# Eric-qi/NeuroQuant

Measured on AMD Instinct MI355X. Metric: calibration iters/sec (HNeRV Bunny 1280x640, 21k iters) + final PSNR vs ref, higher is better.
Workload: dtype f32 operands split into bf16 hi+lo, 3 BF16 MFMAs per product, fp32 accumulate (bf16x3); fp32 MFMA on small layers; 1 GPU; HNeRV Bunny_1280x640_3M, channel_wise, bits 6 5 4 5 5 6 6, phase-2 (AdaRound) iteration; per_gpu_batch=2, global_batch=2, frames=132, parallelism=dp1

## Files before the change

include/nq_hip.h:

```cpp
#ifndef NQ_HIP_H
#define NQ_HIP_H

#include <stdint.h>

#ifdef __cplusplus
extern "C" {
#endif

typedef void* nq_stream_t;

#define NQ_API __attribute__((visibility("default")))

#define NQ_OK 0
#define NQ_ERR_INVALID (-1)
#define NQ_ERR_UNSUPPORTED (-2)
#define NQ_ERR_LAUNCH (-3)

NQ_API int nq_abi_version(void);
NQ_API const char* nq_error_string(int code);


NQ_API int nq_scale_init_max(const float* x, int64_t rows, int64_t row_len, int n_levels, float* delta, float* zp,
                      nq_stream_t stream);

NQ_API int nq_uaq_forward(const float* x, const float* delta, const float* zp, float* y, int64_t rows, int64_t row_len,
                   int per_row, int n_levels, nq_stream_t stream);

NQ_API int nq_uaq_backward(const float* x, const float* gy, const float* delta, const float* zp, float* ddelta, float* dx,
                    int64_t rows, int64_t row_len, int per_row, int n_levels, nq_stream_t stream);

NQ_API int nq_adaround_init(const float* x, const float* delta_in, const float* zp_in, float* delta_out, float* zp_out,
                     float* alpha, int64_t rows, int64_t row_len, int per_row, nq_stream_t stream);

NQ_API int nq_adaround_forward(const float* x, const float* alpha, const float* delta, const float* zp, float* y, float* xq,
                        int64_t rows, int64_t row_len, int per_row, int n_levels, int soft, nq_stream_t stream);

NQ_API int nq_adaround_backward(const float* x, const float* gy, const float* alpha, const float* delta, const float* zp,
                         float* dalpha, int64_t rows, int64_t row_len, int per_row, int n_levels, float reg_weight,
                         float reg_b, nq_stream_t stream);

NQ_API int64_t nq_reduce_ws_floats(int64_t n);
NQ_API int nq_round_loss(const float* alpha, int64_t n, float b, float weight, float* ws, float* out, int accumulate,
                  nq_stream_t stream);

NQ_API int nq_round_loss_backward(const float* alpha, int64_t n, float b, float weight, const float* gscale, float* dalpha,
                           int accumulate, nq_stream_t stream);

NQ_API int nq_adam_step(float* p, const float* g, float* m, float* v, int64_t n, float step_size, float beta1, float beta2,
                 float eps, float bc2_sqrt, nq_stream_t stream);

typedef struct nq_ada_seg {
  const float* x;
  const float* gy;
  const float* alpha;
  const float* delta;
  const float* zp;
  float* out;
  int64_t rows, row_len;
  int per_row, n_levels, soft;
  float reg_weight;
} nq_ada_seg;
typedef struct nq_adam_seg {
  float* p;
  const float* g;
  float* m;
  float* v;
  int64_t n;
} nq_adam_seg;
typedef struct nq_ada_adam_seg {
  const float* x;
  const float* gy;
  float* alpha;
  const float* delta;
  const float* zp;
  float* m;
  float* v;
  int64_t rows, row_len;
  int per_row, n_levels;
  float reg_weight;
} nq_ada_adam_seg;
NQ_API int nq_adaround_adam_multi(const nq_ada_adam_seg* segs, int nseg, float reg_b, float step_size, float beta1, float beta2, float eps,
                           float bc2_sqrt, const float* dyn, nq_stream_t stream);
NQ_API int nq_adaround_forward_multi(const nq_ada_seg* segs, int nseg, nq_stream_t stream);
NQ_API int nq_uaq_forward_multi(const nq_ada_seg* segs, int nseg, nq_stream_t stream);
NQ_API int nq_uaq_backward_multi(const nq_ada_seg* segs, int nseg, nq_stream_t stream);
NQ_API int nq_adaround_backward_multi(const nq_ada_seg* segs, int nseg, float reg_b, nq_stream_t stream);
NQ_API int nq_adam_step_multi(const nq_adam_seg* segs, int nseg, float step_size, float beta1, float beta2, float eps,
                       float bc2_sqrt, nq_stream_t stream);

NQ_API int nq_step_prologue(const int64_t* order, const float* scal, int* step, int64_t* cur_idx, float* cur_scal, int B, int nscal,
                     nq_stream_t stream);
NQ_API int nq_step_prologue_gather(const int64_t* order, const float* scal, int* step, int64_t* cur_idx, float* cur_scal, int B, int nscal,
                            const float* table, int64_t table_rows, int64_t row_len, float* out, nq_stream_t stream);
NQ_API int nq_adaround_backward_multi_dyn(const nq_ada_seg* segs, int nseg, const float* dyn, nq_stream_t stream);
NQ_API int nq_adam_step_multi_dyn(const nq_adam_seg* segs, int nseg, const float* dyn, float beta1, float beta2, float eps,
                           nq_stream_t stream);

NQ_API int nq_fwht(const float* x, float* y, int64_t outer, int n, int64_t inner, int n_in, int n_out, nq_stream_t stream);

typedef struct nq_fwht_seg {
  const float* x;
  float* y;
  int64_t outer, inner;
  int n, n_in, n_out;
} nq_fwht_seg;
NQ_API int nq_fwht_multi(const nq_fwht_seg* segs, int nseg, nq_stream_t stream);

typedef struct nq_fq_fwht_seg {
  const float* x;
  float* alpha;
  const float* delta;
  const float* zp;
  float* m;
  float* v;
  const float* gy;
  float* y;
  int64_t outer, inner;
  int n, c_in, per_row, n_levels, soft;
  float reg_weight;
} nq_fq_fwht_seg;
NQ_API int nq_adaround_fwht_multi(const nq_fq_fwht_seg* segs, int nseg, nq_stream_t stream);
NQ_API int nq_fwht_adaround_adam_multi(const nq_fq_fwht_seg* segs, int nseg, float reg_b, float step_size, float beta1, float beta2,
                                float eps, float bc2_sqrt, const float* dyn, nq_stream_t stream);


NQ_API int nq_weight_layouts(const float* w, float* wt_fwd, float* wt_bwd, int Cout, int Cin, int k, int krows_fwd,
                      int ld_fwd, int krows_bwd, int ld_bwd, nq_stream_t stream);

typedef struct nq_wl_seg {
  const float* w;
  float* wt_fwd;
  float* wt_bwd;
  int Cout, Cin, k, krows_fwd, ld_fwd, krows_bwd, ld_bwd;
} nq_wl_seg;
NQ_API int nq_weight_layouts_multi(const nq_wl_seg* segs, int nseg, nq_stream_t stream);

NQ_API int nq_conv_operand_dims(int Cin, int Cout, int k, int* krows, int* ld);

#define NQ_EPI_PLAIN 0
#define NQ_EPI_PS_GELU 1
#define NQ_EPI_TANH 2
#define NQ_EPI_PS 3
#define NQ_EPI_DGRAD_GELU 4
#define NQ_EPI_X_SPLIT 0x100
#define NQ_EPI_Y_SPLIT 0x200
NQ_API int nq_split_words(const float* x, float* y, int64_t n, nq_stream_t stream);
NQ_API int64_t nq_conv_forward_ws_floats(int B, int Cin, int H, int W, int Cout, int k);
NQ_API int nq_conv_split_out(int B, int Cin, int H, int W, int Cout, int k, int r, int epilogue, int in_gelu, int has_bias);
NQ_API int nq_conv_forward(const float* x, const float* wt, const float* bias, float* y, float* z, float* ws, int B, int Cin, int H,
                    int W, int Cout, int k, int krows, int ld, int r, int epilogue, int in_gelu, const float* zprev,
                    nq_stream_t stream);

NQ_API int nq_conv3_supported(int B, int Cin, int H, int W, int Cout, int k);
NQ_API int nq_conv3_split_io(int B, int Cin, int H, int W, int Cout, int k);
NQ_API int64_t nq_conv_forward3_ws_floats(int B, int Cin, int H, int W, int Cout, int k);
NQ_API int64_t nq_conv3_weight_bytes(int Cin, int Cout, int k);
NQ_API int nq_weight_layout3(const float* w, void* wt3, int Cin, int Cout, int k, int transposed, nq_stream_t stream);
typedef struct nq_wl3_seg {
  const float* w;
  void* wt3;
  int Cin, Cout, k, transposed;
} nq_wl3_seg;
NQ_API int nq_weight_layout3_multi(const nq_wl3_seg* segs, int nseg, nq_stream_t stream);
NQ_API int nq_weight_layouts_all(const nq_wl3_seg* segs3, int n3, const nq_wl_seg* segsf, int nf, nq_stream_t stream);
NQ_API int nq_conv_forward3(const float* x, const void* wt3, const float* bias, float* y, float* z, const float* zprev, float* ws, int B,
                     int Cin, int H, int W, int Cout, int k, int r, int epilogue, nq_stream_t stream);

NQ_API int nq_conv_wgrad3_supported(int B, int Cin, int H, int W, int Cout, int k);
NQ_API int64_t nq_conv_wgrad3_ws_floats(int B, int Cin, int H, int W, int Cout, int k);
NQ_API int nq_conv_wgrad3_plan(int B, int Cin, int H, int W, int Cout, int k, int* mi, int* ni, int* nsplit, int* pc);
NQ_API int nq_conv_wgrad3(const float* x, const float* dy, float* dw, float* db, float* ws, int B, int Cin, int H, int W, int Cout,
                   int k, nq_stream_t stream);
NQ_API int nq_conv_wgrad3_split_io(int B, int Cin, int H, int W, int Cout, int k);
NQ_API int nq_conv_wgrad3_fmt(const float* x, const float* dy, float* dw, float* db, float* ws, int B, int Cin, int H, int W, int Cout,
                       int k, int fmt, nq_stream_t stream);
NQ_API int nq_conv_wgrad3_swapped(const float* x, const float* dy, float* dw, float* ws, int B, int Cin, int H, int W, int Cout, int k,
                           nq_stream_t stream);

NQ_API int64_t nq_conv_wgrad_ws_floats(int B, int Cin, int H, int W, int Cout, int k);
NQ_API int nq_conv_wgrad(const float* x, const float* dy, float* dw, float* db, float* ws, int B, int Cin, int H, int W, int Cout,
                  int k, int x_gelu, nq_stream_t stream);

typedef struct nq_wgr_seg {
  const float* slab;
  const float* slab_db;
  float* dw;
  float* db;
  int Cout, N, co_pad, n_pad, nsplit;
  int swap_kk;
  int sg;
} nq_wgr_seg;
NQ_API int nq_conv_wgrad3_slabs(const float* x, const float* dy, float* dw, float* db, float* ws, int B, int Cin, int H, int W, int Cout,
                         int k, nq_wgr_seg* seg, nq_stream_t stream);
NQ_API int nq_conv_wgrad3_slabs_fmt(const float* x, const float* dy, float* dw, float* db, float* ws, int B, int Cin, int H, int W,
                             int Cout, int k, nq_wgr_seg* seg, int fmt, nq_stream_t stream);
NQ_API int nq_conv_wgrad3_swapped_slabs(const float* x, const float* dy, float* dw, float* ws, int B, int Cin, int H, int W, int Cout,
                                 int k, nq_wgr_seg* seg, nq_stream_t stream);
NQ_API int nq_conv_wgrad_slabs(const float* x, const float* dy, float* dw, float* db, float* ws, int B, int Cin, int H, int W, int Cout,
                        int k, int x_gelu, nq_wgr_seg* seg, nq_stream_t stream);
NQ_API int nq_wgrad_reduce_multi(const nq_wgr_seg* segs, int nseg, nq_stream_t stream);

NQ_API int nq_ps_gelu_backward(const float* da, const float* z, float* dconv, int B, int C, int H, int W, int r,
                        nq_stream_t stream);

NQ_API int nq_tanh_out_backward(const float* dimg, const float* img, float* dconv, int64_t n, nq_stream_t stream);

NQ_API int nq_l2_loss(const float* pred, const float* tgt, float* loss, float* dpred, float* ws, int64_t n, int64_t mean_count,
               float gscale, nq_stream_t stream);

NQ_API int nq_channel_sum(const float* x, float* out, float* ws, int B, int C, int64_t HW, nq_stream_t stream);

NQ_API int nq_l2_loss_tanh_head(const float* pred, const float* tgt, const uint8_t* cache_u8, const int64_t* idx, float* loss,
                         float* dconv, float* db, float* ws, int B, int C, int64_t HW, int64_t mean_count, float gscale,
                         nq_stream_t stream);

NQ_API int64_t nq_head_forward_loss_ws_floats(int B, int H, int W);
NQ_API int nq_head_forward_loss(const float* x, const float* wt, int ld, const float* bias, float* y, const float* tgt,
                         const uint8_t* cache_u8, const int64_t* idx, float* loss, float* dconv, float* db, float* ws, int B,
                         int Cin, int H, int W, int64_t mean_count, float gscale, nq_stream_t stream);

NQ_API int nq_frame_sse(const float* out, const float* gt, float* sse, int64_t frames, int64_t frame_len, nq_stream_t stream);

NQ_API int64_t nq_ms_ssim_ws_floats(int64_t frames, int C, int H, int W);
NQ_API int nq_ms_ssim(const float* out, const float* gt, float* msssim, float* ws, int64_t frames, int C, int H, int W,
               nq_stream_t stream);

NQ_API int nq_gather_frames_u8(const uint8_t* src, const int64_t* idx, float* dst, int64_t n, int64_t frame_len,
                        nq_stream_t stream);

NQ_API int nq_act_dd(const float* x, const float* g, const float* g2, float* y, int64_t n, int mode, nq_stream_t stream);
NQ_API int nq_pixel_shuffle(const float* x, float* y, int B, int C, int H, int W, int r, int inverse, nq_stream_t stream);
NQ_API int nq_bias_add(const float* x, const float* bias, float* y, int B, int C, int64_t HW, nq_stream_t stream);

#ifdef __cplusplus
}
#endif
#endif
```

neuroquant_amd/_lib.py:

```python
import ctypes
import os
from ctypes import c_char_p, c_float, c_int, c_int64, c_void_p, POINTER, Structure

_HERE = os.path.dirname(os.path.abspath(__file__))
LIB_PATH = os.environ.get("NQ_LIB") or os.path.join(_HERE, "libnqhip.so")

NQ_OK = 0
ABI_VERSION = 5
EPI_PLAIN, EPI_PS_GELU, EPI_TANH, EPI_PS, EPI_DGRAD_GELU = 0, 1, 2, 3, 4


class NQLibraryError(RuntimeError):
    pass


class AdaSeg(Structure):
    _fields_ = [("x", c_void_p), ("gy", c_void_p), ("alpha", c_void_p), ("delta", c_void_p), ("zp", c_void_p),
                ("out", c_void_p), ("rows", c_int64), ("row_len", c_int64), ("per_row", c_int), ("n_levels", c_int),
                ("soft", c_int), ("reg_weight", c_float)]


class WL3Seg(Structure):
    _fields_ = [("w", c_void_p), ("wt3", c_void_p), ("Cin", c_int), ("Cout", c_int), ("k", c_int), ("transposed", c_int)]


class WLSeg(Structure):
    _fields_ = [("w", c_void_p), ("wt_fwd", c_void_p), ("wt_bwd", c_void_p), ("Cout", c_int), ("Cin", c_int), ("k", c_int),
                ("krows_fwd", c_int), ("ld_fwd", c_int), ("krows_bwd", c_int), ("ld_bwd", c_int)]


class FwhtSeg(Structure):
    _fields_ = [("x", c_void_p), ("y", c_void_p), ("outer", c_int64), ("inner", c_int64), ("n", c_int), ("n_in", c_int),
                ("n_out", c_int)]


class AdaAdamSeg(Structure):
    _fields_ = [("x", c_void_p), ("gy", c_void_p), ("alpha", c_void_p), ("delta", c_void_p), ("zp", c_void_p), ("m", c_void_p),
                ("v", c_void_p), ("rows", c_int64), ("row_len", c_int64), ("per_row", c_int), ("n_levels", c_int),
                ("reg_weight", c_float)]


class WgrSeg(Structure):
    _fields_ = [("slab", c_void_p), ("slab_db", c_void_p), ("dw", c_void_p), ("db", c_void_p), ("Cout", c_int), ("N", c_int),
                ("co_pad", c_int), ("n_pad", c_int), ("nsplit", c_int), ("swap_kk", c_int), ("sg", c_int)]


class FqFwhtSeg(Structure):
    _fields_ = [("x", c_void_p), ("alpha", c_void_p), ("delta", c_void_p), ("zp", c_void_p), ("m", c_void_p), ("v", c_void_p),
                ("gy", c_void_p), ("y", c_void_p), ("outer", c_int64), ("inner", c_int64), ("n", c_int), ("c_in", c_int),
                ("per_row", c_int), ("n_levels", c_int), ("soft", c_int), ("reg_weight", c_float)]


class AdamSeg(Structure):
    _fields_ = [("p", c_void_p), ("g", c_void_p), ("m", c_void_p), ("v", c_void_p), ("n", c_int64)]


def _load():
    if not os.path.exists(LIB_PATH):
        raise NQLibraryError(
            f"{LIB_PATH} not found: build it with `python -c 'import __graft_entry__ as g; g.build()'` "
            "(or `make -C neuroquant_amd/csrc`).  neuroquant_amd has no CPU/eager fallback.")
    import torch
    lib = ctypes.CDLL(LIB_PATH)
    P, I, L, F = c_void_p, c_int, c_int64, c_float

    def sig(name, res, *args):
        fn = getattr(lib, name)
        fn.restype = res
        fn.argtypes = list(args)

    sig("nq_abi_version", I)
    got = lib.nq_abi_version()
    if got != ABI_VERSION:
        raise NQLibraryError(f"{LIB_PATH} has ABI version {got}, this package binds version {ABI_VERSION}: rebuild it "
                             "(`make -C neuroquant_amd/csrc`)")
    sig("nq_error_string", c_char_p, I)
    sig("nq_scale_init_max", I, P, L, L, I, P, P, P)
    sig("nq_uaq_forward", I, P, P, P, P, L, L, I, I, P)
    sig("nq_uaq_backward", I, P, P, P, P, P, P, L, L, I, I, P)
    sig("nq_adaround_init", I, P, P, P, P, P, P, L, L, I, P)
    sig("nq_adaround_forward", I, P, P, P, P, P, P, L, L, I, I, I, P)
    sig("nq_adaround_backward", I, P, P, P, P, P, P, L, L, I, I, F, F, P)
    sig("nq_adaround_adam_multi", I, POINTER(AdaAdamSeg), I, F, F, F, F, F, F, P, P)
    sig("nq_adaround_forward_multi", I, POINTER(AdaSeg), I, P)
    sig("nq_uaq_forward_multi", I, POINTER(AdaSeg), I, P)
    sig("nq_uaq_backward_multi", I, POINTER(AdaSeg), I, P)
    sig("nq_adaround_backward_multi", I, POINTER(AdaSeg), I, F, P)
    sig("nq_adam_step_multi", I, POINTER(AdamSeg), I, F, F, F, F, F, P)
    sig("nq_step_prologue", I, P, P, P, P, P, I, I, P)
    sig("nq_step_prologue_gather", I, P, P, P, P, P, I, I, P, L, L, P, P)
    sig("nq_adaround_backward_multi_dyn", I, POINTER(AdaSeg), I, P, P)
    sig("nq_adam_step_multi_dyn", I, POINTER(AdamSeg), I, P, F, F, F, P)
    sig("nq_reduce_ws_floats", L, L)
    sig("nq_round_loss", I, P, L, F, F, P, P, I, P)
    sig("nq_round_loss_backward", I, P, L, F, F, P, P, I, P)
    sig("nq_adam_step", I, P, P, P, P, L, F, F, F, F, F, P)
    sig("nq_fwht", I, P, P, L, I, L, I, I, P)
    sig("nq_fwht_multi", I, POINTER(FwhtSeg), I, P)
    sig("nq_weight_layouts", I, P, P, P, I, I, I, I, I, I, I, P)
    sig("nq_conv_operand_dims", I, I, I, I, POINTER(c_int), POINTER(c_int))
    sig("nq_conv_forward_ws_floats", L, I, I, I, I, I, I)
    sig("nq_conv_forward", I, P, P, P, P, P, P, I, I, I, I, I, I, I, I, I, I, I, P, P)
    sig("nq_conv3_supported", I, I, I, I, I, I, I)
    sig("nq_conv3_split_io", I, I, I, I, I, I, I)
    sig("nq_conv_split_out", I, I, I, I, I, I, I, I, I, I, I)
    sig("nq_split_words", I, P, P, L, P)
    sig("nq_conv_wgrad3_split_io", I, I, I, I, I, I, I)
    sig("nq_conv_wgrad3_fmt", I, P, P, P, P, P, I, I, I, I, I, I, I, P)
    sig("nq_conv_wgrad3_slabs_fmt", I, P, P, P, P, P, I, I, I, I, I, I, POINTER(WgrSeg), I, P)
    sig("nq_conv3_weight_bytes", L, I, I, I)
    sig("nq_weight_layout3", I, P, P, I, I, I, I, P)
    sig("nq_weight_layout3_multi", I, POINTER(WL3Seg), I, P)
    sig("nq_weight_layouts_multi", I, POINTER(WLSeg), I, P)
    sig("nq_weight_layouts_all", I, POINTER(WL3Seg), I, POINTER(WLSeg), I, P)
    sig("nq_conv_forward3_ws_floats", L, I, I, I, I, I, I)
    sig("nq_conv_forward3", I, P, P, P, P, P, P, P, I, I, I, I, I, I, I, I, P)
    sig("nq_conv_wgrad3_supported", I, I, I, I, I, I, I)
    sig("nq_conv_wgrad3_ws_floats", L, I, I, I, I, I, I)
    sig("nq_conv_wgrad3_plan", I, I, I, I, I, I, I, POINTER(c_int), POINTER(c_int), POINTER(c_int), POINTER(c_int))
    sig("nq_conv_wgrad3", I, P, P, P, P, P, I, I, I, I, I, I, P)
    sig("nq_conv_wgrad3_swapped", I, P, P, P, P, I, I, I, I, I, I, P)
    sig("nq_conv_wgrad3_slabs", I, P, P, P, P, P, I, I, I, I, I, I, POINTER(WgrSeg), P)
    sig("nq_conv_wgrad3_swapped_slabs", I, P, P, P, P, I, I, I, I, I, I, POINTER(WgrSeg), P)
    sig("nq_conv_wgrad_slabs", I, P, P, P, P, P, I, I, I, I, I, I, I, POINTER(WgrSeg), P)
    sig("nq_wgrad_reduce_multi", I, POINTER(WgrSeg), I, P)
    sig("nq_conv_wgrad_ws_floats", L, I, I, I, I, I, I)
    sig("nq_conv_wgrad", I, P, P, P, P, P, I, I, I, I, I, I, I, P)
    sig("nq_ps_gelu_backward", I, P, P, P, I, I, I, I, I, P)
    sig("nq_tanh_out_backward", I, P, P, P, L, P)
    sig("nq_l2_loss", I, P, P, P, P, P, L, L, F, P)
    sig("nq_channel_sum", I, P, P, P, I, I, L, P)
    sig("nq_l2_loss_tanh_head", I, P, P, P, P, P, P, P, P, I, I, L, L, F, P)
    sig("nq_frame_sse", I, P, P, P, L, L, P)
    sig("nq_ms_ssim_ws_floats", L, L, I, I, I)
    sig("nq_ms_ssim", I, P, P, P, P, L, I, I, I, P)
    sig("nq_gather_frames_u8", I, P, P, P, L, L, P)
    sig("nq_adaround_fwht_multi", I, POINTER(FqFwhtSeg), I, P)
    sig("nq_fwht_adaround_adam_multi", I, POINTER(FqFwhtSeg), I, F, F, F, F, F, F, P, P)
    sig("nq_head_forward_loss_ws_floats", L, I, I, I)
    sig("nq_head_forward_loss", I, P, P, I, P, P, P, P, P, P, P, P, P, I, I, I, I, L, F, P)
    sig("nq_act_dd", I, P, P, P, P, L, I, P)
    sig("nq_pixel_shuffle", I, P, P, I, I, I, I, I, I, P)
    sig("nq_bias_add", I, P, P, P, I, I, L, P)
    return lib


EXPORTS = (
    "nq_abi_version", "nq_error_string", "nq_scale_init_max", "nq_uaq_forward", "nq_uaq_backward",
    "nq_adaround_init", "nq_adaround_forward", "nq_adaround_backward", "nq_reduce_ws_floats", "nq_round_loss", "nq_round_loss_backward",
    "nq_adam_step", "nq_adaround_adam_multi", "nq_adaround_forward_multi", "nq_uaq_forward_multi", "nq_uaq_backward_multi", "nq_adaround_backward_multi", "nq_adam_step_multi", "nq_step_prologue", "nq_step_prologue_gather", "nq_adaround_backward_multi_dyn", "nq_adam_step_multi_dyn", "nq_fwht", "nq_fwht_multi", "nq_weight_layouts", "nq_conv_operand_dims", "nq_conv_forward_ws_floats", "nq_conv_forward",
    "nq_conv3_supported", "nq_conv3_weight_bytes", "nq_weight_layout3", "nq_weight_layout3_multi", "nq_weight_layouts_multi", "nq_conv_forward3_ws_floats", "nq_conv_forward3",
    "nq_conv_wgrad3_supported", "nq_conv_wgrad3_ws_floats", "nq_conv_wgrad3_plan", "nq_conv_wgrad3", "nq_conv_wgrad3_swapped",
    "nq_conv_wgrad3_slabs", "nq_conv_wgrad3_swapped_slabs", "nq_conv_wgrad_slabs", "nq_wgrad_reduce_multi",
    "nq_conv_wgrad_ws_floats", "nq_conv_wgrad", "nq_ps_gelu_backward", "nq_tanh_out_backward", "nq_l2_loss",
    "nq_channel_sum", "nq_l2_loss_tanh_head", "nq_frame_sse", "nq_ms_ssim_ws_floats", "nq_ms_ssim", "nq_gather_frames_u8",
    "nq_act_dd", "nq_pixel_shuffle", "nq_bias_add", "nq_conv3_split_io", "nq_conv_split_out", "nq_split_words",
    "nq_conv_wgrad3_split_io", "nq_conv_wgrad3_fmt", "nq_conv_wgrad3_slabs_fmt", "nq_head_forward_loss_ws_floats", "nq_head_forward_loss",
    "nq_adaround_fwht_multi", "nq_fwht_adaround_adam_multi", "nq_weight_layouts_all",
)

_lib = None


def lib():
    global _lib
    if _lib is None:
        _lib = _load()
    return _lib


def check(rc, what=""):
    if rc != NQ_OK:
        msg = lib().nq_error_string(rc).decode()
        raise NQLibraryError(f"libnqhip {what}: {msg} ({rc})")
```

neuroquant_amd/csrc/conv3.hip:

```cpp
#include <cstdlib>
#include "nq_common.h"
#include "conv3_layout.h"

extern "C" {
int nq_conv_igemm3_k3(const float*, const void*, const float*, float*, float*, const float*, int, int, int, int, int, int, int,
                      int, int, int, float*, hipStream_t);
int nq_conv_igemm3_k5(const float*, const void*, const float*, float*, float*, const float*, int, int, int, int, int, int, int,
                      int, int, int, float*, hipStream_t);
int nq_conv_splitk_finish(const float*, const float*, float*, float*, const float*, int, int, int, int, int, int, int, hipStream_t);
int nq_conv3_nst_k3();
int nq_conv3_nst_k5();
int nq_conv3_nst8_k3();
int nq_conv3_nst8_k5();
int nq_conv3_nstk_k3(int);
int nq_conv3_nstk_k5(int);
int nq_conv_flat3_plan(int, int, int, int, int, int, int*, int*, int*, int*);
int nq_conv_flat3(const float*, const void*, const float*, float*, float*, const float*, float*, int, int, int, int, int, int, int, int,
                  int, int, int, int, hipStream_t);
int nq_conv_wgrad_flat3_ok(int, int, int, int, int, int);
int nq_conv_wgrad_flat3(const float*, const float*, float*, float*, int, int, int, int, int, int, hipStream_t);
int nq_conv_wgrad3_k3(const float*, const float*, float*, float*, int, int, int, int, int, int, int, int, int, int, int, int, hipStream_t);
int nq_conv_wgrad3_k5(const float*, const float*, float*, float*, int, int, int, int, int, int, int, int, int, int, int, int, hipStream_t);
}

namespace {

constexpr int CC = 16;

inline int pick_mi3(int Cout) {
  if (Cout <= 16) return 1;
  if (Cout <= 32) return 2;
  int best = 3, best_pad = 1 << 30;
  for (int mi = 5; mi >= 3; --mi) {
    int mt = 16 * mi, pad = (Cout + mt - 1) / mt * mt;
    if (pad < best_pad) {
      best_pad = pad;
      best = mi;
    }
  }
  if (Cout > 256 && (Cout + 63) / 64 * 64 <= best_pad + best_pad * 6 / 100) return 4;
  return best;
}
inline int nst_of(int k) { return k == 5 ? nq_conv3_nst_k5() : nq_conv3_nst_k3(); }
inline int nstk_of(int k, int kind) { return k == 5 ? nq_conv3_nstk_k5(kind) : nq_conv3_nstk_k3(kind); }
inline int tail_kind_of(int Cin, int mi) {
  const int r = Cin - CC * ((Cin + CC - 1) / CC - 1);
  return r <= 4 ? 1 : (r <= 8 ? 2 : (r <= 12 ? 3 : 0));
}
inline int64_t total_steps3(int Cin, int k, int mi) {
  const int nchunk = (Cin + CC - 1) / CC;
  return (int64_t)(nchunk - 1) * nst_of(k) + nstk_of(k, tail_kind_of(Cin, mi));
}

struct WL3 {
  const float* w;
  uint4* out;
  int Cin, Cout, KK, NST, NSTT, nchunk, tail, co_tiles, MT, transposed;
  int co16;
  int64_t slots;
};

constexpr int WL3_KKMAX = 25;
template <int KK>
__device__ __forceinline__ void wl3_tile(const WL3& p, int c, int g16, float* __restrict__ T ) {
  constexpr int RS = 16 * KK + 1;
  const int tid = threadIdx.x;
  const int nfull = p.nchunk - (p.tail ? 1 : 0);
  const int kind = (c == nfull) ? p.tail : 0;
  const int nst = kind ? p.NSTT : p.NST;
  const int64_t gs0 = (int64_t)c * p.NST;
  const int Ra = p.transposed ? p.Cin : p.Cout;
  const int Cb = p.transposed ? p.Cout : p.Cin;
  const int a0 = p.transposed ? c * 16 : g16 * 16, b0 = p.transposed ? g16 * 16 : c * 16;
  {
    float v[KK];
#pragma unroll
    for (int j = 0; j < KK; ++j) {
      const int e = tid + j * 256;
      const int a = e / (16 * KK), rem = e - a * (16 * KK);
      const int bb = rem / KK;
      const bool ok = a0 + a < Ra && b0 + bb < Cb;
      const float t = p.w[ok ? ((int64_t)(a0 + a) * Cb + b0) * KK + rem : 0];
      v[j] = ok ? t : 0.f;
    }
#pragma unroll
    for (int j = 0; j < KK; ++j) {
      const int e = tid + j * 256;
      const int a = e / (16 * KK), rem = e - a * (16 * KK);
      T[a * RS + rem] = v[j];
    }
  }
  __syncthreads();
  const int MT = p.MT;
  const int64_t plane_stride = (int64_t)p.co_tiles * 4 * MT;
  for (int sl = tid; sl < nst * 4 * 16; sl += 256) {
    const int col = sl & 15, kq = (sl >> 4) & 3, st = sl >> 6;
    const int co = g16 * 16 + col;
    if (co >= p.co_tiles * MT) continue;
    unsigned hi[4], lo[4];
#pragma unroll
    for (int j = 0; j < 4; ++j) {
      float v[2];
#pragma unroll
      for (int t = 0; t < 2; ++t) {
        int ch, tap;
        wl3_elem(kind, KK, st, kq, 2 * j + t, ch, tap);
        float x = 0.f;
        if (tap < KK) x = p.transposed ? T[ch * RS + col * KK + (KK - 1 - tap)] : T[col * RS + ch * KK + tap];
        v[t] = x;
      }
      __bf16 h0 = (__bf16)v[0], h1 = (__bf16)v[1];
      __bf16 l0 = (__bf16)(v[0] - (float)h0), l1 = (__bf16)(v[1] - (float)h1);
      hi[j] = (unsigned)__builtin_bit_cast(unsigned short, h0) | ((unsigned)__builtin_bit_cast(unsigned short, h1) << 16);
      lo[j] = (unsigned)__builtin_bit_cast(unsigned short, l0) | ((unsigned)__builtin_bit_cast(unsigned short, l1) << 16);
    }
    const int tile = co / MT, co_l = co - tile * MT;
    const int64_t base = (gs0 + st) * 2 * plane_stride + (int64_t)tile * 4 * MT + kq * MT + co_l;
    p.out[base] = make_uint4(hi[0], hi[1], hi[2], hi[3]);
    p.out[base + plane_stride] = make_uint4(lo[0], lo[1], lo[2], lo[3]);
  }
}

__global__ __launch_bounds__(256) void weight_layout3_kernel(WL3 p) {
  __shared__ float T[16 * (16 * WL3_KKMAX + 1)];
  if (p.KK == 25) wl3_tile<25>(p, (int)blockIdx.x / p.co16, (int)blockIdx.x % p.co16, T);
  else wl3_tile<9>(p, (int)blockIdx.x / p.co16, (int)blockIdx.x % p.co16, T);
}

constexpr int WL3_MAXSEG = 16;
struct WL3Multi {
  WL3 s[WL3_MAXSEG];
  int blk0[WL3_MAXSEG + 1];
  int nseg;
};
__global__ __launch_bounds__(256) void weight_layout3_multi_kernel(WL3Multi t) {
  __shared__ float T[16 * (16 * WL3_KKMAX + 1)];
  int k = 0;
  while (k + 1 < t.nseg && (int)blockIdx.x >= t.blk0[k + 1]) ++k;
  const int blk = (int)blockIdx.x - t.blk0[k];
  if (t.s[k].KK == 25) wl3_tile<25>(t.s[k], blk / t.s[k].co16, blk % t.s[k].co16, T);
  else wl3_tile<9>(t.s[k], blk / t.s[k].co16, blk % t.s[k].co16, T);
}

struct WLF {
  const float* w;
  float* wt;
  int Cout, Cin, KK, krows, ld, bwd;
};
struct WLAll {
  WL3 s3[WL3_MAXSEG];
  int blk3[WL3_MAXSEG + 1];
  int n3;
  WLF sf[WL3_MAXSEG];
  int blkf[WL3_MAXSEG + 1];
  int nf;
};
__global__ __launch_bounds__(256) void weight_layouts_all_kernel(WLAll t) {
  __shared__ float T[16 * (16 * WL3_KKMAX + 1)];
  const int nb3 = t.blk3[t.n3];
  if ((int)blockIdx.x < nb3) {
    int k = 0;
    while (k + 1 < t.n3 && (int)blockIdx.x >= t.blk3[k + 1]) ++k;
    const int blk = (int)blockIdx.x - t.blk3[k];
    if (t.s3[k].KK == 25) wl3_tile<25>(t.s3[k], blk / t.s3[k].co16, blk % t.s3[k].co16, T);
    else wl3_tile<9>(t.s3[k], blk / t.s3[k].co16, blk % t.s3[k].co16, T);
    return;
  }
  const int bf = (int)blockIdx.x - nb3;
  int k = 0;
  while (k + 1 < t.nf && bf >= t.blkf[k + 1]) ++k;
  const WLF& g = t.sf[k];
  const int64_t i = (int64_t)(bf - t.blkf[k]) * 256 + threadIdx.x;
  if (i >= (int64_t)g.krows * g.ld) return;
  const int row = (int)(i / g.ld), col = (int)(i - (int64_t)row * g.ld);
  float v = 0.f;
  if (g.bwd) {
    const int co = row / g.KK, tap = row - co * g.KK;
    if (co < g.Cout && col < g.Cin) v = g.w[((int64_t)co * g.Cin + col) * g.KK + (g.KK - 1 - tap)];
  } else {
    if (col < g.Cout && row < g.Cin * g.KK) v = g.w[(int64_t)col * (g.Cin * g.KK) + row];
  }
  g.wt[i] = v;
}

struct Fwd3Plan {
  int mi, nsplit, per;
  int64_t wgs;
};
inline Fwd3Plan plan_fwd3(int B, int Cin, int H, int W, int Cout) {
  Fwd3Plan p;
  p.mi = pick_mi3(Cout);
  p.wgs = (int64_t)((W + 31) / 32) * ((H + 7) / 8) * ((Cout + 16 * p.mi - 1) / (16 * p.mi)) * B;
  const int nchunk = (Cin + CC - 1) / CC;
  p.nsplit = 1;
  p.per = nchunk;
  static const int min_chunks = [] { const char* e = getenv("NQ_SPLITK_MIN_CHUNKS"); return e ? atoi(e) : 5; }();
  if (p.wgs < 256 && nchunk >= min_chunks) {
    int want = (int)(512 / p.wgs);
    if (want > nchunk) want = nchunk;
    p.per = (nchunk + want - 1) / want;
    p.nsplit = (nchunk + p.per - 1) / p.per;
  }
  return p;
}

inline bool use_flat3(int B, int Cin, int H, int W, int Cout, int k, int* fns) {
  int ns = 1;
  if (!nq_conv_flat3_plan(B, Cin, H, W, Cout, k, nullptr, nullptr, &ns, nullptr)) return false;
  if (fns) *fns = ns;
  if (ns == 1) return true;
  const Fwd3Plan p = plan_fwd3(B, Cin, H, W, Cout);
  return p.wgs * p.nsplit < 128;
}

struct Wg3Plan {
  int mi, ni, co_pad, n_pad, nsplit, pc;
};
inline bool wgrad3_ss1() {
  const char* e = std::getenv("NQ_WGRAD3_SS");
  return e && e[0] == '1';
}
inline bool wgrad3_pc_enabled() {
  const char* e = std::getenv("NQ_WGRAD3_PC");
  return !(e && e[0] == '0');
}
inline Wg3Plan plan_wgrad3(int B, int Cin, int H, int W, int Cout, int k) {
  Wg3Plan p;
  p.mi = pick_mi3(Cout);
  const int N = Cin * k * k;
  if (N <= 64) {
    p.ni = 1;
  } else {
    int best = 6, best_pad = 1 << 30;
    for (int ni = 5; ni <= (p.mi <= 4 ? 7 : 6); ++ni) {
      const int nt = 64 * ni, pad = (N + nt - 1) / nt * nt;
      if (pad <= best_pad) {
        best_pad = pad;
        best = ni;
      }
    }
    p.ni = best;
  }
  int mt = 16 * p.mi, nt = 64 * p.ni;
  p.co_pad = (Cout + mt - 1) / mt * mt;
  p.n_pad = (N + nt - 1) / nt * nt;
  int tiles = (p.co_pad / mt) * (p.n_pad / nt);
  if (tiles > 256 && p.mi < 5 && p.ni >= 5 && p.ni <= 6 ) {
    const int co5 = (Cout + 79) / 80 * 80, tiles5 = (co5 / 80) * (p.n_pad / nt);
    if (tiles5 <= 256 && co5 * 100 <= p.co_pad * 105) {
      p.mi = 5;
      mt = 80;
      p.co_pad = co5;
      tiles = tiles5;
    }
  }
  const int nseg = ((W + 31) / 32) * H * B;
  int ns = 512 / tiles;
  if (ns > nseg) ns = nseg;
  if (ns < 1) ns = 1;
  p.nsplit = ns;
  p.pc = 0;
  const bool pc_ok = wgrad3_pc_enabled() && (int64_t)B * Cin * H * W * 4 < (1ll << 31) && (int64_t)B * Cout * H * W * 4 < (1ll << 31);
  if (pc_ok && p.ni >= 5 && p.mi >= 3 && tiles <= 256) {
    int sy = 1;
    int ns_pc = 256 / tiles;
    const int segs_x = (W + 31) / 32;
    static const int minseg = [] { const char* e = std::getenv("NQ_WGRAD3_MINSEG"); return e ? atoi(e) : 6; }();
    if (!wgrad3_ss1() && ns_pc >= 1) {
      const bool sy4_fits = !(k == 3 && p.mi == 5 && p.ni == 6);
      if (sy4_fits && H % 4 == 0 && segs_x * (H / 4) * B / ns_pc >= minseg) sy = 4;
      else if (H % 2 == 0 && segs_x * (H / 2) * B / ns_pc >= minseg) sy = 2;
    }
    const int nseg_pc = segs_x * (H / sy) * B;
    const int need = minseg < 16 ? minseg : 16;
    static const int shrink = [] { const char* e = std::getenv("NQ_WGRAD3_SHRINK"); return e ? atoi(e) : 1; }();
    if (shrink && ns_pc >= 1 && nseg_pc / ns_pc < need && (nseg_pc / need) * tiles >= 192) ns_pc = nseg_pc / need;
    if (ns_pc >= 1 && nseg_pc / ns_pc >= need) {
      p.pc = sy == 1 ? 1 : 10 + sy;
      p.nsplit = ns_pc;
    }
  }
  if (pc_ok && p.ni == 1 && p.mi >= 2 && p.mi <= 5 && tiles == 1 && W % 128 == 0) {
    const int nseg_pc = (W / 128) * H * B;
    if (nseg_pc / 256 >= 8) {
      p.pc = 4;
      static const int hs = [] { const char* e = std::getenv("NQ_WGRAD3_HEAD_SPLITS"); return e ? atoi(e) : 512; }();
      p.nsplit = (p.mi <= 3 && nseg_pc / hs >= 8) ? hs : 256;
    }
  }
  return p;
}

template <int SG>
__global__ __launch_bounds__(256) void wgrad3_reduce_kernel(const float* __restrict__ slab, const float* __restrict__ slab_db,
                                                            float* __restrict__ dw, float* __restrict__ db, int Cout, int N,
                                                            int co_pad, int n_pad, int nsplit, int swap_kk) {
  constexpr int OG = 256 / SG;
  __shared__ float part[SG][OG];
  const int o = threadIdx.x % OG, g = threadIdx.x / OG;
  const int64_t i = (int64_t)blockIdx.x * OG + o;
  const int64_t total = (int64_t)Cout * N;
  float s = 0.f;
  if (i < total) {
    const int co = (int)(i / N), n = (int)(i - (int64_t)co * N);
    const float* p = slab + (int64_t)co * n_pad + n;
    const int64_t stride = (int64_t)co_pad * n_pad;
#pragma unroll 4
    for (int k = g; k < nsplit; k += SG) s += p[k * stride];
  } else if (db && i < total + Cout) {
    const int co = (int)(i - total);
#pragma unroll 4
    for (int k = g; k < nsplit; k += SG) s += slab_db[(int64_t)k * co_pad + co];
  }
  part[g][o] = s;
  __syncthreads();
  if (g == 0) {
    float t = part[0][o];
#pragma unroll
    for (int j = 1; j < SG; ++j) t += part[j][o];
    if (i < total) {
      if (swap_kk > 0) {
        const int co = (int)(i / N), n = (int)(i - (int64_t)co * N);
        const int ci = n / swap_kk, tap = n - ci * swap_kk;
        dw[((int64_t)ci * Cout + co) * swap_kk + (swap_kk - 1 - tap)] = t;
      } else {
        dw[i] = t;
      }
    } else if (db && i < total + Cout) {
      db[(int)(i - total)] = t;
    }
  }
}

constexpr int WGR_MAXSEG = 16;
struct WGRMulti {
  nq_wgr_seg s[WGR_MAXSEG];
  int blk0[WGR_MAXSEG + 1];
  int nseg;
};
__global__ __launch_bounds__(256) void wgrad_reduce_multi_kernel(WGRMulti t) {
  __shared__ float4 part[256];
  int k = 0;
  while (k + 1 < t.nseg && (int)blockIdx.x >= t.blk0[k + 1]) ++k;
  const nq_wgr_seg& q = t.s[k];
  const int SG = q.sg, OG = 256 / SG;
  const int o = threadIdx.x % OG, g = threadIdx.x / OG;
  const int N = q.N, Cout = q.Cout, nsplit = q.nsplit;
  const int NQ = (N + 3) >> 2;
  const int64_t i = (int64_t)((int)blockIdx.x - t.blk0[k]) * OG + o;
  const int64_t total = (int64_t)Cout * NQ;
  float4 s = make_float4(0.f, 0.f, 0.f, 0.f);
  int co = 0, n = 0;
  if (i < total) {
    co = (int)(i / NQ);
    n = 4 * (int)(i - (int64_t)co * NQ);
    const float* p = q.slab + (int64_t)co * q.n_pad + n;
    const int64_t stride = (int64_t)q.co_pad * q.n_pad;
#pragma unroll 8
    for (int j = g; j < nsplit; j += SG) {
      const float4 v = *reinterpret_cast<const float4*>(p + j * stride);
      s.x += v.x; s.y += v.y; s.z += v.z; s.w += v.w;
    }
  } else if (q.db && i < total + Cout) {
    const int cb = (int)(i - total);
#pragma unroll 8
    for (int j = g; j < nsplit; j += SG) s.x += q.slab_db[(int64_t)j * q.co_pad + cb];
  }
  if (SG > 1) {
    part[g * OG + o] = s;
    __syncthreads();
    if (g != 0) return;
    s = part[o];
    for (int j = 1; j < SG; ++j) {
      const float4 v = part[j * OG + o];
      s.x += v.x; s.y += v.y; s.z += v.z; s.w += v.w;
    }
  }
  if (i < total) {
    const float sv[4] = {s.x, s.y, s.z, s.w};
    if (q.swap_kk > 0) {
#pragma unroll
      for (int e = 0; e < 4; ++e) {
        if (n + e >= N) break;
        const int ci = (n + e) / q.swap_kk, tap = (n + e) - ci * q.swap_kk;
        q.dw[((int64_t)ci * Cout + co) * q.swap_kk + (q.swap_kk - 1 - tap)] = sv[e];
      }
    } else if ((N & 3) == 0) {
      *reinterpret_cast<float4*>(q.dw + (int64_t)co * N + n) = s;
    } else {
#pragma unroll
      for (int e = 0; e < 4; ++e)
        if (n + e < N) q.dw[(int64_t)co * N + n + e] = sv[e];
    }
  } else if (q.db && i < total + Cout) {
    q.db[(int)(i - total)] = s.x;
  }
}

}

extern "C" {

int nq_conv3_supported(int B, int Cin, int H, int W, int Cout, int k) {
  if (!(k == 3 || k == 5) || B <= 0 || Cin <= 0 || Cout <= 4 || Cin <= 4) return 0;
  if ((int64_t)B * Cin * H * W * 4 >= 0xFFFFFF00ll) return 0;
  if (use_flat3(B, Cin, H, W, Cout, k, nullptr) && (int64_t)Cin * k * k * Cout >= 65536) return 1;
  const Fwd3Plan p = plan_fwd3(B, Cin, H, W, Cout);
  return p.wgs * p.nsplit >= 128;
}

int64_t nq_conv_forward3_ws_floats(int B, int Cin, int H, int W, int Cout, int k) {
  if (!(k == 3 || k == 5) || B <= 0 || Cin <= 0 || H <= 0 || W <= 0 || Cout <= 0) return 0;
  int fns = 1;
  if (use_flat3(B, Cin, H, W, Cout, k, &fns)) return fns > 1 ? (int64_t)fns * B * Cout * H * W : 0;
  const Fwd3Plan p = plan_fwd3(B, Cin, H, W, Cout);
  return p.nsplit > 1 ? (int64_t)p.nsplit * B * Cout * H * W : 0;
}

int64_t nq_conv3_weight_bytes(int Cin, int Cout, int k) {
  if (!(k == 3 || k == 5)) return 0;
  const int mi = pick_mi3(Cout), mt = 16 * mi;
  const int64_t co_tiles = (Cout + mt - 1) / mt, nchunk = (Cin + CC - 1) / CC;
  (void)nchunk;
  return total_steps3(Cin, k, mi) * 2 * co_tiles * 4 * mt * 16;
}

static bool wl3_fill(WL3& p, const float* w, void* wt3, int Cin, int Cout, int k, int transposed) {
  if (!w || !wt3 || !(k == 3 || k == 5) || Cin <= 0 || Cout <= 0) return false;
  const int mi = pick_mi3(Cout);
  p.w = w; p.out = reinterpret_cast<uint4*>(wt3);
  p.Cin = Cin; p.Cout = Cout; p.KK = k * k; p.NST = nst_of(k); p.tail = tail_kind_of(Cin, mi); p.NSTT = nstk_of(k, p.tail);
  p.MT = 16 * mi; p.co_tiles = (Cout + p.MT - 1) / p.MT; p.nchunk = (Cin + CC - 1) / CC; p.transposed = transposed;
  p.slots = total_steps3(Cin, k, mi) * p.co_tiles * 4 * p.MT;
  p.co16 = (p.co_tiles * p.MT + 15) / 16;
  return true;
}

int nq_weight_layout3(const float* w, void* wt3, int Cin, int Cout, int k, int transposed, nq_stream_t stream) {
  WL3 p;
  if (!wl3_fill(p, w, wt3, Cin, Cout, k, transposed)) return NQ_ERR_INVALID;
  hipLaunchKernelGGL(weight_layout3_kernel, dim3((unsigned)(p.nchunk * p.co16)), dim3(256), 0, nq_s(stream), p);
  return nq_launch_status();
}

int nq_weight_layout3_multi(const nq_wl3_seg* segs, int nseg, nq_stream_t stream) {
  if (!segs || nseg <= 0) return NQ_ERR_INVALID;
  for (int base = 0; base < nseg; base += WL3_MAXSEG) {
    WL3Multi t;
    t.nseg = (nseg - base < WL3_MAXSEG) ? nseg - base : WL3_MAXSEG;
    int blocks = 0;
    for (int i = 0; i < t.nseg; ++i) {
      const nq_wl3_seg& h = segs[base + i];
      if (!wl3_fill(t.s[i], h.w, h.wt3, h.Cin, h.Cout, h.k, h.transposed)) return NQ_ERR_INVALID;
      t.blk0[i] = blocks;
      blocks += t.s[i].nchunk * t.s[i].co16;
    }
    t.blk0[t.nseg] = blocks;
    hipLaunchKernelGGL(weight_layout3_multi_kernel, dim3((unsigned)blocks), dim3(256), 0, nq_s(stream), t);
  }
  return nq_launch_status();
}

int nq_weight_layouts_all(const nq_wl3_seg* segs3, int n3, const nq_wl_seg* segsf, int nf, nq_stream_t stream) {
  if ((n3 > 0 && !segs3) || (nf > 0 && !segsf) || n3 < 0 || nf < 0 || n3 + nf == 0) return NQ_ERR_INVALID;
  int nfo = 0;
  for (int i = 0; i < nf; ++i) nfo += (segsf[i].wt_fwd ? 1 : 0) + (segsf[i].wt_bwd ? 1 : 0);
  if (n3 > WL3_MAXSEG || nfo > WL3_MAXSEG || n3 == 0 || nfo == 0) {
    if (n3 > 0)
      if (int rc = nq_weight_layout3_multi(segs3, n3, stream)) return rc;
    if (nf > 0) return nq_weight_layouts_multi(segsf, nf, stream);
    return NQ_OK;
  }
  WLAll t;
  t.n3 = n3;
  int blocks = 0;
  for (int i = 0; i < n3; ++i) {
    const nq_wl3_seg& h = segs3[i];
    if (!wl3_fill(t.s3[i], h.w, h.wt3, h.Cin, h.Cout, h.k, h.transposed)) return NQ_ERR_INVALID;
    t.blk3[i] = blocks;
    blocks += t.s3[i].nchunk * t.s3[i].co16;
  }
  t.blk3[n3] = blocks;
  t.nf = 0;
  int bf = 0;
  for (int i = 0; i < nf; ++i) {
    const nq_wl_seg& h = segsf[i];
    if (!h.w || h.Cout <= 0 || h.Cin <= 0 || h.k <= 0) return NQ_ERR_INVALID;
    const int KK = h.k * h.k;
    for (int bwd = 0; bwd < 2; ++bwd) {
      float* wt = bwd ? h.wt_bwd : h.wt_fwd;
      if (!wt) continue;
      const int krows = bwd ? h.krows_bwd : h.krows_fwd, ld = bwd ? h.ld_bwd : h.ld_fwd;
      if (bwd ? (krows < h.Cout * KK || ld < h.Cin) : (krows < h.Cin * KK || ld < h.Cout)) return NQ_ERR_INVALID;
      t.sf[t.nf] = WLF{h.w, wt, h.Cout, h.Cin, KK, krows, ld, bwd};
      t.blkf[t.nf] = bf;
      bf += (int)(((int64_t)krows * ld + 255) / 256);
      ++t.nf;
    }
  }
  t.blkf[t.nf] = bf;
  hipLaunchKernelGGL(weight_layouts_all_kernel, dim3((unsigned)(blocks + bf)), dim3(256), 0, nq_s(stream), t);
  return nq_launch_status();
}

int nq_conv3_split_io(int B, int Cin, int H, int W, int Cout, int k) {
  if (!nq_conv3_supported(B, Cin, H, W, Cout, k)) return 0;
  {
    int fns = 1;
    if (use_flat3(B, Cin, H, W, Cout, k, &fns)) return fns == 1 ? NQ_EPI_Y_SPLIT : 0;
  }
  const Fwd3Plan p = plan_fwd3(B, Cin, H, W, Cout);
  return (p.mi >= 2 ? NQ_EPI_X_SPLIT : 0) | (p.nsplit == 1 ? NQ_EPI_Y_SPLIT : 0);
}

int nq_conv_forward3(const float* x, const void* wt3, const float* bias, float* y, float* z, const float* zprev, float* ws, int B,
                     int Cin, int H, int W, int Cout, int k, int r, int epilogue, nq_stream_t stream) {
  if (!x || !wt3 || (!y && epilogue != NQ_EPI_PS) || B <= 0 || Cin <= 0 || H <= 0 || W <= 0 || Cout <= 0) return NQ_ERR_INVALID;
  if (!(k == 3 || k == 5)) return NQ_ERR_UNSUPPORTED;
  const int fmt = epilogue & (NQ_EPI_X_SPLIT | NQ_EPI_Y_SPLIT);
  epilogue &= ~(NQ_EPI_X_SPLIT | NQ_EPI_Y_SPLIT);
  if (fmt & ~nq_conv3_split_io(B, Cin, H, W, Cout, k)) return NQ_ERR_UNSUPPORTED;
  if (epilogue < 0 || epilogue > NQ_EPI_DGRAD_GELU) return NQ_ERR_INVALID;
  if ((epilogue == NQ_EPI_PS_GELU || epilogue == NQ_EPI_PS) && (!z || r <= 0 || Cout % (r * r) != 0)) return NQ_ERR_INVALID;
  if (epilogue == NQ_EPI_DGRAD_GELU && (!zprev || r <= 0 || H % r != 0 || W % r != 0)) return NQ_ERR_INVALID;
  if (B > 65535) return NQ_ERR_UNSUPPORTED;
  hipStream_t st = nq_s(stream);
  {
    int fns = 1;
    if (use_flat3(B, Cin, H, W, Cout, k, &fns)) {
      if (fns > 1 && !ws) return NQ_ERR_INVALID;
      const int mi = pick_mi3(Cout), kind = tail_kind_of(Cin, mi);
      int rc = nq_conv_flat3(x, wt3, bias, y, z, zprev, ws, B, Cin, H, W, Cout, k, r, epilogue | fmt, 16 * mi, kind, nst_of(k),
                             nstk_of(k, kind), st);
      if (rc != NQ_OK || fns == 1) return rc;
      return nq_conv_splitk_finish(ws, bias, y, z, zprev, B, H, W, Cout, r, epilogue, fns, st);
    }
  }
  const Fwd3Plan p = plan_fwd3(B, Cin, H, W, Cout);
  if (p.nsplit > 1 && !ws) return NQ_ERR_INVALID;
  int rc = (k == 3) ? nq_conv_igemm3_k3(x, wt3, bias, y, z, zprev, B, Cin, H, W, Cout, r, epilogue | fmt, p.mi, p.nsplit, p.per, ws, st)
                    : nq_conv_igemm3_k5(x, wt3, bias, y, z, zprev, B, Cin, H, W, Cout, r, epilogue | fmt, p.mi, p.nsplit, p.per, ws, st);
  if (rc != NQ_OK || p.nsplit == 1) return rc;
  return nq_conv_splitk_finish(ws, bias, y, z, zprev, B, H, W, Cout, r, epilogue, p.nsplit, st);
}

int nq_conv_wgrad3_supported(int B, int Cin, int H, int W, int Cout, int k) {
  if (!(k == 3 || k == 5) || B <= 0 || Cin <= 0 || Cout <= 4) return 0;
  if (nq_conv_wgrad_flat3_ok(B, Cin, H, W, Cout, k)) return 1;
  return (int64_t)((W + 31) / 32) * H * B >= 128;
}

int nq_conv_wgrad3_plan(int B, int Cin, int H, int W, int Cout, int k, int* mi, int* ni, int* nsplit, int* pc) {
  if (!(k == 3 || k == 5) || B <= 0 || Cin <= 0 || H <= 0 || W <= 0 || Cout <= 0 || !mi || !ni || !nsplit || !pc) return NQ_ERR_INVALID;
  const Wg3Plan p = plan_wgrad3(B, Cin, H, W, Cout, k);
  *mi = p.mi; *ni = p.ni; *nsplit = p.nsplit; *pc = p.pc;
  return NQ_OK;
}

int64_t nq_conv_wgrad3_ws_floats(int B, int Cin, int H, int W, int Cout, int k) {
  if (!(k == 3 || k == 5) || B <= 0 || Cin <= 0 || H <= 0 || W <= 0 || Cout <= 0) return 0;
  if (nq_conv_wgrad_flat3_ok(B, Cin, H, W, Cout, k)) return 4;
  Wg3Plan p = plan_wgrad3(B, Cin, H, W, Cout, k);
  return (int64_t)p.nsplit * p.co_pad * ((int64_t)p.n_pad + 1);
}

static int conv_wgrad3_impl(const float* x, const float* dy, float* dw, float* db, float* ws, int B, int Cin, int H, int W,
                            int Cout, int k, int swap_kk, nq_wgr_seg* seg, nq_stream_t stream, int fmt = 0);

int nq_conv_wgrad3(const float* x, const float* dy, float* dw, float* db, float* ws, int B, int Cin, int H, int W, int Cout,
                   int k, nq_stream_t stream) {
  return conv_wgrad3_impl(x, dy, dw, db, ws, B, Cin, H, W, Cout, k, 0, nullptr, stream);
}

int nq_conv_wgrad3_split_io(int B, int Cin, int H, int W, int Cout, int k) {
  if (!nq_conv_wgrad3_supported(B, Cin, H, W, Cout, k) || nq_conv_wgrad_flat3_ok(B, Cin, H, W, Cout, k)) return 0;
  const Wg3Plan p = plan_wgrad3(B, Cin, H, W, Cout, k);
  return (p.pc == 1 || p.pc == 12 || p.pc == 14) ? 3 : 0;
}
int nq_conv_wgrad3_fmt(const float* x, const float* dy, float* dw, float* db, float* ws, int B, int Cin, int H, int W, int Cout,
                       int k, int fmt, nq_stream_t stream) {
  if (fmt & ~nq_conv_wgrad3_split_io(B, Cin, H, W, Cout, k)) return NQ_ERR_UNSUPPORTED;
  return conv_wgrad3_impl(x, dy, dw, db, ws, B, Cin, H, W, Cout, k, 0, nullptr, stream, fmt);
}
int nq_conv_wgrad3_slabs_fmt(const float* x, const float* dy, float* dw, float* db, float* ws, int B, int Cin, int H, int W,
                             int Cout, int k, nq_wgr_seg* seg, int fmt, nq_stream_t stream) {
  if (!seg) return NQ_ERR_INVALID;
  if (fmt & ~nq_conv_wgrad3_split_io(B, Cin, H, W, Cout, k)) return NQ_ERR_UNSUPPORTED;
  return conv_wgrad3_impl(x, dy, dw, db, ws, B, Cin, H, W, Cout, k, 0, seg, stream, fmt);
}

int nq_conv_wgrad3_swapped(const float* x, const float* dy, float* dw, float* ws, int B, int Cin, int H, int W, int Cout, int k,
                           nq_stream_t stream) {
  return conv_wgrad3_impl(dy, x, dw, nullptr, ws, B, Cout, H, W, Cin, k, k * k, nullptr, stream);
}

int nq_conv_wgrad3_slabs(const float* x, const float* dy, float* dw, float* db, float* ws, int B, int Cin, int H, int W, int Cout,
                         int k, nq_wgr_seg* seg, nq_stream_t stream) {
  if (!seg) return NQ_ERR_INVALID;
  return conv_wgrad3_impl(x, dy, dw, db, ws, B, Cin, H, W, Cout, k, 0, seg, stream);
}

int nq_conv_wgrad3_swapped_slabs(const float* x, const float* dy, float* dw, float* ws, int B, int Cin, int H, int W, int Cout,
                                 int k, nq_wgr_seg* seg, nq_stream_t stream) {
  if (!seg) return NQ_ERR_INVALID;
  return conv_wgrad3_impl(dy, x, dw, nullptr, ws, B, Cout, H, W, Cin, k, k * k, seg, stream);
}

int nq_wgrad_reduce_multi(const nq_wgr_seg* segs, int nseg, nq_stream_t stream) {
  if (!segs || nseg < 0) return NQ_ERR_INVALID;
  WGRMulti t;
  t.nseg = 0;
  int blocks = 0;
  auto flush = [&]() {
    if (t.nseg == 0) return;
    t.blk0[t.nseg] = blocks;
    hipLaunchKernelGGL(wgrad_reduce_multi_kernel, dim3((unsigned)blocks), dim3(256), 0, nq_s(stream), t);
    t.nseg = 0;
    blocks = 0;
  };
  for (int i = 0; i < nseg; ++i) {
    const nq_wgr_seg& h = segs[i];
    if (h.nsplit == 0) continue;
    if (!h.slab || !h.dw || h.Cout <= 0 || h.N <= 0 || h.nsplit < 0 || !(h.sg == 1 || h.sg == 4 || h.sg == 16) ||
        (h.db && !h.slab_db))
      return NQ_ERR_INVALID;
    if (t.nseg == WGR_MAXSEG) flush();
    t.s[t.nseg] = h;
    t.blk0[t.nseg] = blocks;
    const int og = 256 / h.sg;
    blocks += (int)(((int64_t)h.Cout * ((h.N + 3) / 4) + h.Cout + og - 1) / og);
    ++t.nseg;
  }
  flush();
  return nq_launch_status();
}

static int conv_wgrad3_impl(const float* x, const float* dy, float* dw, float* db, float* ws, int B, int Cin, int H, int W,
                            int Cout, int k, int swap_kk, nq_wgr_seg* seg, nq_stream_t stream, int fmt) {
  if (!x || !dy || !dw || !ws || B <= 0 || Cin <= 0 || H <= 0 || W <= 0 || Cout <= 0) return NQ_ERR_INVALID;
  if (!(k == 3 || k == 5)) return NQ_ERR_UNSUPPORTED;
  if ((int64_t)Cout * H * W >= (1ll << 31) || (int64_t)Cin * H * W >= (1ll << 31)) return NQ_ERR_UNSUPPORTED;
  if (swap_kk == 0 && nq_conv_wgrad_flat3_ok(B, Cin, H, W, Cout, k)) {
    if (fmt) return NQ_ERR_UNSUPPORTED;
    if (seg) *seg = nq_wgr_seg{nullptr, nullptr, dw, db, Cout, Cin * k * k, 0, 0, 0, 0, 1};
    return nq_conv_wgrad_flat3(x, dy, dw, db, B, Cin, H, W, Cout, k, nq_s(stream));
  }
  if (swap_kk != 0 && nq_conv_wgrad_flat3_ok(B, Cin, H, W, Cout, k)) return NQ_ERR_UNSUPPORTED;
  Wg3Plan p = plan_wgrad3(B, Cin, H, W, Cout, k);
  float* slab = ws;
  float* slab_db = ws + (int64_t)p.nsplit * p.co_pad * p.n_pad;
  hipStream_t st = nq_s(stream);
  int rc = (k == 3) ? nq_conv_wgrad3_k3(x, dy, slab, slab_db, B, Cin, H, W, Cout, p.co_pad, p.n_pad, p.nsplit, p.mi, p.ni, p.pc, fmt, st)
                    : nq_conv_wgrad3_k5(x, dy, slab, slab_db, B, Cin, H, W, Cout, p.co_pad, p.n_pad, p.nsplit, p.mi, p.ni, p.pc, fmt, st);
  if (rc != NQ_OK) return rc;
  const int N = Cin * k * k;
  int64_t total = (int64_t)Cout * N + Cout;
  if (seg) {
    *seg = nq_wgr_seg{slab, db ? slab_db : nullptr, dw, db, Cout, N, p.co_pad, p.n_pad, p.nsplit, swap_kk,
                      (total < 65536 && p.nsplit >= 16) ? 16 : 4};
    return NQ_OK;
  }
  if (total < 65536 && p.nsplit >= 16) {
    hipLaunchKernelGGL(wgrad3_reduce_kernel<16>, dim3((unsigned)((total + 15) / 16)), dim3(256), 0, st, slab, slab_db, dw, db,
                       Cout, N, p.co_pad, p.n_pad, p.nsplit, swap_kk);
  } else {
    hipLaunchKernelGGL(wgrad3_reduce_kernel<4>, dim3((unsigned)((total + 63) / 64)), dim3(256), 0, st, slab, slab_db, dw, db,
                       Cout, N, p.co_pad, p.n_pad, p.nsplit, swap_kk);
  }
  return nq_launch_status();
}

}
```

neuroquant_amd/csrc/quant.hip:

```cpp
#include "nq_common.h"
#include "quant_elem.h"

namespace {

constexpr int TPB = 256;
constexpr int EPT = 4;

__global__ __launch_bounds__(TPB) void scale_init_kernel(const float* __restrict__ x, int64_t row_len, int n_levels,
                                                         float* __restrict__ delta, float* __restrict__ zp) {
  __shared__ float smin[4], smax[4];
  const float* xr = x + (int64_t)blockIdx.x * row_len;
  float mn = 0.f, mx = 0.f;
  for (int64_t i = threadIdx.x; i < row_len; i += TPB) {
    float v = xr[i];
    mn = fminf(mn, v);
    mx = fmaxf(mx, v);
  }
  mn = nq_wave_min(mn);
  mx = nq_wave_max(mx);
  if ((threadIdx.x & 63) == 0) {
    smin[threadIdx.x >> 6] = mn;
    smax[threadIdx.x >> 6] = mx;
  }
  __syncthreads();
// ... 83 lines not shown
                                                           const float* __restrict__ delta,
                                                           const float* __restrict__ zp, float* __restrict__ y,
                                                           float* __restrict__ xq_out, int64_t row_len, int per_row,
                                                           float qmax, int soft, unsigned bpr) {
  const int64_t row = blockIdx.x / bpr;
  const float d = per_row ? delta[row] : delta[0];
  const float z = per_row ? zp[row] : zp[0];
  const int64_t base = row * row_len;
  int64_t i = (int64_t)(blockIdx.x - row * bpr) * (TPB * EPT) + threadIdx.x;
#pragma unroll
  for (int e = 0; e < EPT; ++e, i += TPB) {
    if (i < row_len) {
      float xq;
      y[base + i] = ada_fwd_elem(x[base + i], alpha[base + i], d, z, qmax, soft, xq);
      if (xq_out) xq_out[base + i] = xq;
    }
  }
}

__global__ __launch_bounds__(TPB) void adaround_bwd_kernel(const float* __restrict__ x, const float* __restrict__ gy,
                                                           const float* __restrict__ alpha,
                                                           const float* __restrict__ delta,
                                                           const float* __restrict__ zp, float* __restrict__ dalpha,
                                                           int64_t row_len, int per_row, float qmax, float reg_weight,
                                                           float reg_b, unsigned bpr) {
  const int64_t row = blockIdx.x / bpr;
  const float d = per_row ? delta[row] : delta[0];
  const float z = per_row ? zp[row] : zp[0];
  const int64_t base = row * row_len;
  int64_t i = (int64_t)(blockIdx.x - row * bpr) * (TPB * EPT) + threadIdx.x;
#pragma unroll
  for (int e = 0; e < EPT; ++e, i += TPB) {
    if (i < row_len) {
      float g = ada_bwd_elem(x[base + i], gy[base + i], alpha[base + i], d, z, qmax, reg_weight, reg_b);
      dalpha[base + i] = g;
    }
  }
}

constexpr int RED_CHUNK = NQ_RED_CHUNK;

__global__ __launch_bounds__(TPB) void round_loss_stage1(const float* __restrict__ alpha, int64_t n, float b,
                                                         float* __restrict__ ws) {
  __shared__ float red[16];
  int64_t i0 = (int64_t)blockIdx.x * RED_CHUNK;
  float acc = 0.f;
  for (int k = 0; k < 16; ++k) {
    int64_t i = i0 + k * TPB + threadIdx.x;
    if (i < n) {
      float h = fminf(fmaxf(soft_target_lin(alpha[i]), 0.f), 1.f);
      acc += 1.f - powf(fabsf(h - 0.5f) * 2.f, b);
    }
  }
  float s = nq_block_sum(acc, red);
  if (threadIdx.x == 0) ws[blockIdx.x] = s;
}

__global__ __launch_bounds__(TPB) void round_loss_bwd_kernel(const float* __restrict__ alpha, int64_t n, float b,
                                                             float weight, const float* __restrict__ gscale,
                                                             float* __restrict__ dalpha, int accumulate) {
  int64_t i = (int64_t)blockIdx.x * TPB + threadIdx.x;
  if (i >= n) return;
  float s = nq_sigmoid(alpha[i]);
  float lin = s * (NQ_ZETA - NQ_GAMMA) + NQ_GAMMA;
  float h = fminf(fmaxf(lin, 0.f), 1.f);
  float hp = (lin >= 0.f && lin <= 1.f) ? (NQ_ZETA - NQ_GAMMA) * (s * (1.f - s)) : 0.f;
  float c = h - 0.5f;
  float sg = (c > 0.f) ? 1.f : ((c < 0.f) ? -1.f : 0.f);
  float g = -(weight * (gscale ? gscale[0] : 1.f)) * (b * powf(fabsf(c) * 2.f, b - 1.f)) * 2.f * sg * hp;
  dalpha[i] = accumulate ? dalpha[i] + g : g;
}

__device__ __forceinline__ void adam_elem(float* __restrict__ p, const float* __restrict__ g, float* __restrict__ m,
                                          float* __restrict__ v, int64_t i, float step_size, float beta1, float beta2,
                                          float eps, float bc2_sqrt) {
  float gi = g[i];
  float mi = m[i];
  mi = mi + (1.f - beta1) * (gi - mi);
  float vi = v[i] * beta2 + (1.f - beta2) * (gi * gi);
  m[i] = mi;
  v[i] = vi;
  float denom = sqrtf(vi) / bc2_sqrt + eps;
  p[i] = p[i] - step_size * (mi / denom);
}

__global__ __launch_bounds__(TPB) void adam_kernel(float* __restrict__ p, const float* __restrict__ g,
                                                   float* __restrict__ m, float* __restrict__ v, int64_t n,
                                                   float step_size, float beta1, float beta2, float eps,
                                                   float bc2_sqrt) {
  int64_t i = (int64_t)blockIdx.x * TPB + threadIdx.x;
  if (i >= n) return;
  adam_elem(p, g, m, v, i, step_size, beta1, beta2, eps, bc2_sqrt);
}


constexpr int MAXSEG = 16;
struct AdaSegD {
  const float* x;
  const float* gy;
  const float* alpha;
  const float* delta;
  const float* zp;
  float* out;
  int64_t n;
  int row_len, per_row, soft;
  float qmax, reg_weight;
  int vec;
};
struct AdaMulti {
  AdaSegD s[MAXSEG];
  int blk0[MAXSEG + 1];
  int nseg;
  float reg_b;
  const float* dyn;
};
struct AdamSegD {
  float* p;
  const float* g;
  float* m;
  float* v;
  int64_t n;
  int vec;
};
struct AdamMulti {
  AdamSegD s[MAXSEG];
  int blk0[MAXSEG + 1];
  int nseg;
};

template <class T>
__device__ __forceinline__ int find_seg(const T& t, int blk) {
  int k = 0;
  while (k + 1 < t.nseg && blk >= t.blk0[k + 1]) ++k;
  return k;
}

template <bool BWD>
__global__ __launch_bounds__(TPB) void adaround_multi_kernel(AdaMulti t) {
  const int k = find_seg(t, blockIdx.x);
  const AdaSegD& sg = t.s[k];
  const int64_t i0 = (int64_t)(blockIdx.x - t.blk0[k]) * (TPB * EPT) + 4 * threadIdx.x;
  if (i0 >= sg.n) return;
  const bool vec = sg.vec && (i0 + 3 < sg.n);
  float xv[4], av[4], gv[4] = {0.f, 0.f, 0.f, 0.f}, ov[4];
  if (vec) {
    const float4 x4 = *reinterpret_cast<const float4*>(sg.x + i0), a4 = *reinterpret_cast<const float4*>(sg.alpha + i0);
    xv[0] = x4.x; xv[1] = x4.y; xv[2] = x4.z; xv[3] = x4.w;
    av[0] = a4.x; av[1] = a4.y; av[2] = a4.z; av[3] = a4.w;
    if (BWD) {
      const float4 g4 = *reinterpret_cast<const float4*>(sg.gy + i0);
      gv[0] = g4.x; gv[1] = g4.y; gv[2] = g4.z; gv[3] = g4.w;
    }
  } else {
#pragma unroll
    for (int j = 0; j < 4; ++j) {
      const bool in = i0 + j < sg.n;
      xv[j] = in ? sg.x[i0 + j] : 0.f;
      av[j] = in ? sg.alpha[i0 + j] : 0.f;
      if (BWD) gv[j] = in ? sg.gy[i0 + j] : 0.f;
    }
  }
  const int64_t row0 = sg.per_row ? i0 / sg.row_len : 0;
  const int rem0 = sg.per_row ? (int)(i0 - row0 * sg.row_len) : 0;
  const float rb = (BWD && t.dyn) ? t.dyn[0] : t.reg_b;
  const float rw = (BWD && t.dyn) ? sg.reg_weight * t.dyn[1] : sg.reg_weight;
#pragma unroll
  for (int j = 0; j < 4; ++j) {
    int64_t row = 0;
    if (sg.per_row) row = (sg.row_len >= 4) ? row0 + ((rem0 + j >= sg.row_len) ? 1 : 0) : (i0 + j) / sg.row_len;
    if (i0 + j >= sg.n) row = 0;
    const float d = sg.delta[row], z = sg.zp[row];
    if (BWD) {
      ov[j] = ada_bwd_elem(xv[j], gv[j], av[j], d, z, sg.qmax, rw, rb);
    } else {
      float xq;
      ov[j] = ada_fwd_elem(xv[j], av[j], d, z, sg.qmax, sg.soft, xq);
    }
  }
  if (vec) {
    *reinterpret_cast<float4*>(sg.out + i0) = make_float4(ov[0], ov[1], ov[2], ov[3]);
  } else {
#pragma unroll
    for (int j = 0; j < 4; ++j)
      if (i0 + j < sg.n) sg.out[i0 + j] = ov[j];
  }
}

__global__ __launch_bounds__(TPB) void adam_multi_kernel(AdamMulti t, float step_size, float beta1, float beta2, float eps,
                                                         float bc2_sqrt, const float* __restrict__ dyn) {
  if (dyn) {
    step_size = dyn[2];
    bc2_sqrt = dyn[3];
  }
  const int k = find_seg(t, blockIdx.x);
  const AdamSegD& sg = t.s[k];
  const int64_t i0 = (int64_t)(blockIdx.x - t.blk0[k]) * (TPB * EPT) + 4 * threadIdx.x;
  if (i0 >= sg.n) return;
  if (sg.vec && i0 + 3 < sg.n) {
    const float4 g4 = *reinterpret_cast<const float4*>(sg.g + i0);
    float4 m4 = *reinterpret_cast<const float4*>(sg.m + i0), v4 = *reinterpret_cast<const float4*>(sg.v + i0);
    float4 p4 = *reinterpret_cast<const float4*>(sg.p + i0);
    const float g[4] = {g4.x, g4.y, g4.z, g4.w};
    float m[4] = {m4.x, m4.y, m4.z, m4.w}, v[4] = {v4.x, v4.y, v4.z, v4.w}, p[4] = {p4.x, p4.y, p4.z, p4.w};
#pragma unroll
    for (int j = 0; j < 4; ++j) {
      m[j] = m[j] + (1.f - beta1) * (g[j] - m[j]);
      v[j] = v[j] * beta2 + (1.f - beta2) * (g[j] * g[j]);
      const float denom = sqrtf(v[j]) / bc2_sqrt + eps;
      p[j] = p[j] - step_size * (m[j] / denom);
    }
    *reinterpret_cast<float4*>(sg.m + i0) = make_float4(m[0], m[1], m[2], m[3]);
    *reinterpret_cast<float4*>(sg.v + i0) = make_float4(v[0], v[1], v[2], v[3]);
    *reinterpret_cast<float4*>(sg.p + i0) = make_float4(p[0], p[1], p[2], p[3]);
  } else {
#pragma unroll
    for (int j = 0; j < 4; ++j)
      if (i0 + j < sg.n) adam_elem(sg.p, sg.g, sg.m, sg.v, i0 + j, step_size, beta1, beta2, eps, bc2_sqrt);
  }
}

struct AdaAdamSegD {
  const float* x;
  const float* gy;
  float* alpha;
  const float* delta;
  const float* zp;
  float* m;
  float* v;
  int64_t n;
  int row_len, per_row;
  float qmax, reg_weight;
  int vec;
};
struct AdaAdamMulti {
  AdaAdamSegD s[MAXSEG];
  int blk0[MAXSEG + 1];
  int nseg;
};
__global__ __launch_bounds__(TPB) void adaround_adam_multi_kernel(AdaAdamMulti t, float reg_b, float step_size, float beta1,
                                                                  float beta2, float eps, float bc2_sqrt,
                                                                  const float* __restrict__ dyn) {
  float gate = 1.f;
  if (dyn) {
    reg_b = dyn[0];
    gate = dyn[1];
    step_size = dyn[2];
    bc2_sqrt = dyn[3];
  }
  const int k = find_seg(t, blockIdx.x);
  const AdaAdamSegD& sg = t.s[k];
  const int64_t i0 = (int64_t)(blockIdx.x - t.blk0[k]) * (TPB * EPT) + 4 * threadIdx.x;
  if (i0 >= sg.n) return;
  const bool vec = sg.vec && (i0 + 3 < sg.n);
  float xv[4], av[4], gv[4], mv[4], vv[4];
  if (vec) {
    const float4 x4 = *reinterpret_cast<const float4*>(sg.x + i0), a4 = *reinterpret_cast<const float4*>(sg.alpha + i0);
    const float4 g4 = *reinterpret_cast<const float4*>(sg.gy + i0);
    const float4 m4 = *reinterpret_cast<const float4*>(sg.m + i0), v4 = *reinterpret_cast<const float4*>(sg.v + i0);
    xv[0] = x4.x; xv[1] = x4.y; xv[2] = x4.z; xv[3] = x4.w;
    av[0] = a4.x; av[1] = a4.y; av[2] = a4.z; av[3] = a4.w;
    gv[0] = g4.x; gv[1] = g4.y; gv[2] = g4.z; gv[3] = g4.w;
    mv[0] = m4.x; mv[1] = m4.y; mv[2] = m4.z; mv[3] = m4.w;
    vv[0] = v4.x; vv[1] = v4.y; vv[2] = v4.z; vv[3] = v4.w;
  } else {
#pragma unroll
    for (int j = 0; j < 4; ++j) {
      const bool in = i0 + j < sg.n;
      xv[j] = in ? sg.x[i0 + j] : 0.f;
      av[j] = in ? sg.alpha[i0 + j] : 0.f;
      gv[j] = in ? sg.gy[i0 + j] : 0.f;
      mv[j] = in ? sg.m[i0 + j] : 0.f;
      vv[j] = in ? sg.v[i0 + j] : 0.f;
    }
  }
  const int64_t row0 = sg.per_row ? i0 / sg.row_len : 0;
  const int rem0 = sg.per_row ? (int)(i0 - row0 * sg.row_len) : 0;
  const float rw = dyn ? sg.reg_weight * gate : sg.reg_weight;
#pragma unroll
  for (int j = 0; j < 4; ++j) {
    int64_t row = 0;
    if (sg.per_row) row = (sg.row_len >= 4) ? row0 + ((rem0 + j >= sg.row_len) ? 1 : 0) : (i0 + j) / sg.row_len;
    if (i0 + j >= sg.n) row = 0;
    const float g = ada_bwd_elem(xv[j], gv[j], av[j], sg.delta[row], sg.zp[row], sg.qmax, rw, reg_b);
    mv[j] = mv[j] + (1.f - beta1) * (g - mv[j]);
    vv[j] = vv[j] * beta2 + (1.f - beta2) * (g * g);
    const float denom = sqrtf(vv[j]) / bc2_sqrt + eps;
    av[j] = av[j] - step_size * (mv[j] / denom);
  }
  if (vec) {
    *reinterpret_cast<float4*>(sg.m + i0) = make_float4(mv[0], mv[1], mv[2], mv[3]);
    *reinterpret_cast<float4*>(sg.v + i0) = make_float4(vv[0], vv[1], vv[2], vv[3]);
    *reinterpret_cast<float4*>(sg.alpha + i0) = make_float4(av[0], av[1], av[2], av[3]);
  } else {
#pragma unroll
    for (int j = 0; j < 4; ++j)
      if (i0 + j < sg.n) {
        sg.m[i0 + j] = mv[j];
        sg.v[i0 + j] = vv[j];
        sg.alpha[i0 + j] = av[j];
      }
  }
}

struct UaqSegD {
  const float* x;
  const float* gy;
  const float* delta;
  const float* zp;
  float* out;
  int64_t n;
  int64_t rows;
  int row_len, per_row;
  float qmax;
};
struct UaqMulti {
  UaqSegD s[MAXSEG];
  int blk0[MAXSEG + 1];
  int nseg;
};
__global__ __launch_bounds__(TPB) void uaq_fwd_multi_kernel(UaqMulti t) {
  const int k = find_seg(t, blockIdx.x);
  const UaqSegD& sg = t.s[k];
  int64_t i = (int64_t)(blockIdx.x - t.blk0[k]) * (TPB * EPT) + threadIdx.x;
#pragma unroll
  for (int e = 0; e < EPT; ++e, i += TPB) {
    if (i < sg.n) {
      const int64_t row = sg.per_row ? i / sg.row_len : 0;
      const float d = sg.delta[row], z = sg.zp[row];
      float xi = rintf(sg.x[i] / d) + z;
      float xq = fminf(fmaxf(xi, 0.f), sg.qmax);
      sg.out[i] = (xq - z) * d;
    }
  }
}
__global__ __launch_bounds__(TPB) void uaq_bwd_multi_kernel(UaqMulti t) {
  __shared__ float red[16];
  const int k = find_seg(t, blockIdx.x);
  const UaqSegD& sg = t.s[k];
  const int64_t row = blockIdx.x - t.blk0[k];
  const float d = sg.delta[row], z = sg.zp[row];
  const int64_t base = row * sg.row_len;
  float acc = 0.f;
  for (int64_t i = threadIdx.x; i < sg.row_len; i += TPB) {
    float u = sg.x[base + i] / d;
    float xi = rintf(u) + z;
    float xq = fminf(fmaxf(xi, 0.f), sg.qmax);
    float inside = (xi >= 0.f && xi <= sg.qmax) ? 1.f : 0.f;
    acc += sg.gy[base + i] * ((xq - z) - inside * u);
  }
  float s = nq_block_sum(acc, red);
  if (threadIdx.x == 0) sg.out[row] = s;
}

inline unsigned blocks_per_row(int64_t row_len) { return (unsigned)((row_len + TPB * EPT - 1) / (TPB * EPT)); }
inline dim3 row_grid(int64_t rows, int64_t row_len) { return dim3((unsigned)(rows * blocks_per_row(row_len)), 1, 1); }
inline bool bad_rows(int64_t rows, int64_t row_len) {
  return rows <= 0 || row_len <= 0 || rows * (int64_t)blocks_per_row(row_len) > 0x7fffffffLL;
}

}

extern "C" {

int nq_abi_version(void) { return 5; }

const char* nq_error_string(int code) {
  switch (code) {
    case NQ_OK: return "ok";
    case NQ_ERR_INVALID: return "invalid argument";
    case NQ_ERR_UNSUPPORTED: return "unsupported shape";
    case NQ_ERR_LAUNCH: return "HIP launch error";
    default: return "unknown error";
  }
}

int nq_scale_init_max(const float* x, int64_t rows, int64_t row_len, int n_levels, float* delta, float* zp,
                      nq_stream_t stream) {
  if (!x || !delta || !zp || rows <= 0 || row_len <= 0 || n_levels < 2) return NQ_ERR_INVALID;
  hipLaunchKernelGGL(scale_init_kernel, dim3((unsigned)rows), dim3(TPB), 0, nq_s(stream), x, row_len, n_levels, delta,
                     zp);
  return nq_launch_status();
}

int nq_uaq_forward(const float* x, const float* delta, const float* zp, float* y, int64_t rows, int64_t row_len,
                   int per_row, int n_levels, nq_stream_t stream) {
  if (!x || !delta || !zp || !y || bad_rows(rows, row_len)) return NQ_ERR_INVALID;
  hipLaunchKernelGGL(uaq_fwd_kernel, row_grid(rows, row_len), dim3(TPB), 0, nq_s(stream), x, delta, zp, y, row_len,
                     per_row, (float)(n_levels - 1), blocks_per_row(row_len));
  return nq_launch_status();
}

int nq_uaq_backward(const float* x, const float* gy, const float* delta, const float* zp, float* ddelta, float* dx,
                    int64_t rows, int64_t row_len, int per_row, int n_levels, nq_stream_t stream) {
  if (!x || !gy || !delta || !zp || !ddelta || rows <= 0 || row_len <= 0) return NQ_ERR_INVALID;
  int64_t r = per_row ? rows : 1, len = per_row ? row_len : rows * row_len;
  hipLaunchKernelGGL(uaq_bwd_kernel, dim3((unsigned)r), dim3(TPB), 0, nq_s(stream), x, gy, delta, zp, ddelta, dx, len,
                     per_row, (float)(n_levels - 1));
  return nq_launch_status();
}

static int uaq_multi(const nq_ada_seg* segs, int nseg, bool bwd, nq_stream_t stream) {
  if (!segs || nseg <= 0) return NQ_ERR_INVALID;
  for (int base = 0; base < nseg; base += MAXSEG) {
    UaqMulti t;
    t.nseg = (nseg - base < MAXSEG) ? nseg - base : MAXSEG;
    int64_t blocks = 0;
    for (int k = 0; k < t.nseg; ++k) {
      const nq_ada_seg& h = segs[base + k];
      if (!h.x || !h.delta || !h.zp || !h.out || (bwd && !h.gy) || h.rows <= 0 || h.row_len <= 0) return NQ_ERR_INVALID;
      UaqSegD& d = t.s[k];
      d.x = h.x; d.gy = h.gy; d.delta = h.delta; d.zp = h.zp; d.out = h.out;
      d.n = h.rows * h.row_len;
      d.rows = h.per_row ? h.rows : 1;
      const int64_t rl = h.per_row ? h.row_len : h.rows * h.row_len;
      if (rl > 0x7fffffffLL) return NQ_ERR_INVALID;
      d.row_len = (int)rl; d.per_row = h.per_row; d.qmax = (float)(h.n_levels - 1);
      t.blk0[k] = (int)blocks;
      blocks += bwd ? d.rows : (d.n + TPB * EPT - 1) / (TPB * EPT);
      if (blocks > 0x7fffffffLL) return NQ_ERR_INVALID;
    }
    t.blk0[t.nseg] = (int)blocks;
    if (bwd)
      hipLaunchKernelGGL(uaq_bwd_multi_kernel, dim3((unsigned)blocks), dim3(TPB), 0, nq_s(stream), t);
    else
      hipLaunchKernelGGL(uaq_fwd_multi_kernel, dim3((unsigned)blocks), dim3(TPB), 0, nq_s(stream), t);
  }
  return nq_launch_status();
}

int nq_uaq_forward_multi(const nq_ada_seg* segs, int nseg, nq_stream_t stream) { return uaq_multi(segs, nseg, false, stream); }
int nq_uaq_backward_multi(const nq_ada_seg* segs, int nseg, nq_stream_t stream) { return uaq_multi(segs, nseg, true, stream); }

int nq_adaround_init(const float* x, const float* delta_in, const float* zp_in, float* delta_out, float* zp_out,
                     float* alpha, int64_t rows, int64_t row_len, int per_row, nq_stream_t stream) {
  if (!x || !delta_in || !zp_in || !delta_out || !zp_out || !alpha || bad_rows(rows, row_len)) return NQ_ERR_INVALID;
  int64_t ns = per_row ? rows : 1;
  hipLaunchKernelGGL(adaround_scale_kernel, dim3((unsigned)((ns + 255) / 256)), dim3(256), 0, nq_s(stream), delta_in,
                     zp_in, delta_out, zp_out, ns);
  hipLaunchKernelGGL(adaround_alpha_init_kernel, row_grid(rows, row_len), dim3(TPB), 0, nq_s(stream), x, delta_out,
                     alpha, row_len, per_row, blocks_per_row(row_len));
  return nq_launch_status();
}

int nq_adaround_forward(const float* x, const float* alpha, const float* delta, const float* zp, float* y, float* xq,
                        int64_t rows, int64_t row_len, int per_row, int n_levels, int soft, nq_stream_t stream) {
  if (!x || !alpha || !delta || !zp || !y || bad_rows(rows, row_len)) return NQ_ERR_INVALID;
  hipLaunchKernelGGL(adaround_fwd_kernel, row_grid(rows, row_len), dim3(TPB), 0, nq_s(stream), x, alpha, delta, zp, y,
                     xq, row_len, per_row, (float)(n_levels - 1), soft, blocks_per_row(row_len));
  return nq_launch_status();
}

int nq_adaround_backward(const float* x, const float* gy, const float* alpha, const float* delta, const float* zp,
                         float* dalpha, int64_t rows, int64_t row_len, int per_row, int n_levels, float reg_weight,
                         float reg_b, nq_stream_t stream) {
  if (!x || !gy || !alpha || !delta || !zp || !dalpha || bad_rows(rows, row_len)) return NQ_ERR_INVALID;
  hipLaunchKernelGGL(adaround_bwd_kernel, row_grid(rows, row_len), dim3(TPB), 0, nq_s(stream), x, gy, alpha, delta, zp,
                     dalpha, row_len, per_row, (float)(n_levels - 1), reg_weight, reg_b, blocks_per_row(row_len));
  return nq_launch_status();
}

int64_t nq_reduce_ws_floats(int64_t n) { return n <= 0 ? 1 : (n + RED_CHUNK - 1) / RED_CHUNK; }

int nq_round_loss(const float* alpha, int64_t n, float b, float weight, float* ws, float* out, int accumulate,
                  nq_stream_t stream) {
  if (!alpha || !ws || !out || n <= 0) return NQ_ERR_INVALID;
  int64_t parts = nq_reduce_ws_floats(n);
  hipLaunchKernelGGL(round_loss_stage1, dim3((unsigned)parts), dim3(TPB), 0, nq_s(stream), alpha, n, b, ws);
  hipLaunchKernelGGL(nq_sum_stage2, dim3(1), dim3(TPB), 0, nq_s(stream), ws, parts, weight, out, accumulate);
  return nq_launch_status();
}

int nq_round_loss_backward(const float* alpha, int64_t n, float b, float weight, const float* gscale, float* dalpha,
                           int accumulate, nq_stream_t stream) {
  if (!alpha || !dalpha || n <= 0) return NQ_ERR_INVALID;
  hipLaunchKernelGGL(round_loss_bwd_kernel, dim3((unsigned)((n + TPB - 1) / TPB)), dim3(TPB), 0, nq_s(stream), alpha, n,
                     b, weight, gscale, dalpha, accumulate);
  return nq_launch_status();
}

int nq_adam_step(float* p, const float* g, float* m, float* v, int64_t n, float step_size, float beta1, float beta2,
                 float eps, float bc2_sqrt, nq_stream_t stream) {
  if (!p || !g || !m || !v || n <= 0) return NQ_ERR_INVALID;
  hipLaunchKernelGGL(adam_kernel, dim3((unsigned)((n + TPB - 1) / TPB)), dim3(TPB), 0, nq_s(stream), p, g, m, v, n,
                     step_size, beta1, beta2, eps, bc2_sqrt);
  return nq_launch_status();
}

__global__ __launch_bounds__(256) void step_prologue_kernel(const int64_t* __restrict__ order, const float* __restrict__ scal,
                                                            int* __restrict__ step, int64_t* __restrict__ cur_idx,
                                                            float* __restrict__ cur_scal, int B, int nscal) {
  const int s = *step;
  const int t = threadIdx.x;
  int64_t vi = 0;
  float vs = 0.f;
  if (t < B) vi = order[(int64_t)s * B + t];
  if (t < nscal) vs = scal[(int64_t)s * nscal + t];
  __syncthreads();
  if (t < B) cur_idx[t] = vi;
  if (t < nscal) cur_scal[t] = vs;
  if (t == 0) *step = s + 1;
}

__global__ __launch_bounds__(256) void step_prologue_gather_kernel(const int64_t* __restrict__ order, const float* __restrict__ scal,
                                                                   int* __restrict__ step, int64_t* __restrict__ cur_idx,
                                                                   float* __restrict__ cur_scal, int B, int nscal,
                                                                   const float* __restrict__ table, int64_t table_rows,
                                                                   int64_t row_len, float* __restrict__ out) {
  __shared__ int last;
  const int s = __hip_atomic_load(step, __ATOMIC_RELAXED, __HIP_MEMORY_SCOPE_AGENT);
  const int t = threadIdx.x;
  if (blockIdx.x == 0) {
    if (t < B) cur_idx[t] = order[(int64_t)s * B + t];
    if (t < nscal) cur_scal[t] = scal[(int64_t)s * nscal + t];
  } else {
    const int64_t per = ((int64_t)B * row_len + (gridDim.x - 2)) / (gridDim.x - 1);
    const int64_t lo = (int64_t)(blockIdx.x - 1) * per, hi = min(lo + per, (int64_t)B * row_len);
    for (int64_t e = lo + t; e < hi; e += 256) {
      const int64_t f = e / row_len, j = e - f * row_len;
      int64_t idx = order[(int64_t)s * B + f];
      idx = idx < 0 ? 0 : (idx >= table_rows ? table_rows - 1 : idx);
      out[e] = table[idx * row_len + j];
    }
  }
  __syncthreads();
  if (t == 0) last = (atomicAdd(step + 1, 1) == (int)gridDim.x - 1);
  __syncthreads();
  if (last && t == 0) {
    step[1] = 0;
    __hip_atomic_store(step, s + 1, __ATOMIC_RELAXED, __HIP_MEMORY_SCOPE_AGENT);
  }
}

static int ada_multi(const nq_ada_seg* segs, int nseg, float reg_b, const float* dyn, bool bwd, nq_stream_t stream) {
  if (!segs || nseg <= 0) return NQ_ERR_INVALID;
  for (int base = 0; base < nseg; base += MAXSEG) {
    AdaMulti t;
    t.nseg = (nseg - base < MAXSEG) ? nseg - base : MAXSEG;
    t.reg_b = reg_b;
    t.dyn = dyn;
    int blocks = 0;
    for (int k = 0; k < t.nseg; ++k) {
      const nq_ada_seg& h = segs[base + k];
      if (!h.x || !h.alpha || !h.delta || !h.zp || !h.out || (bwd && !h.gy) || h.rows <= 0 || h.row_len <= 0 ||
          h.row_len > 0x7fffffffLL)
        return NQ_ERR_INVALID;
      AdaSegD& d = t.s[k];
      d.x = h.x; d.gy = h.gy; d.alpha = h.alpha; d.delta = h.delta; d.zp = h.zp; d.out = h.out;
      d.n = h.rows * h.row_len; d.row_len = (int)h.row_len; d.per_row = h.per_row; d.soft = h.soft;
      d.qmax = (float)(h.n_levels - 1); d.reg_weight = h.reg_weight;
      d.vec = (((uintptr_t)h.x | (uintptr_t)h.alpha | (uintptr_t)h.out | (uintptr_t)(bwd ? h.gy : h.x)) & 15) == 0;
      t.blk0[k] = blocks;
      blocks += (int)((d.n + TPB * EPT - 1) / (TPB * EPT));
    }
    t.blk0[t.nseg] = blocks;
    if (bwd)
      hipLaunchKernelGGL(adaround_multi_kernel<true>, dim3((unsigned)blocks), dim3(TPB), 0, nq_s(stream), t);
    else
      hipLaunchKernelGGL(adaround_multi_kernel<false>, dim3((unsigned)blocks), dim3(TPB), 0, nq_s(stream), t);
  }
  return nq_launch_status();
}

int nq_adaround_forward_multi(const nq_ada_seg* segs, int nseg, nq_stream_t stream) {
  return ada_multi(segs, nseg, 0.f, nullptr, false, stream);
}

int nq_adaround_backward_multi(const nq_ada_seg* segs, int nseg, float reg_b, nq_stream_t stream) {
  return ada_multi(segs, nseg, reg_b, nullptr, true, stream);
}

int nq_adaround_backward_multi_dyn(const nq_ada_seg* segs, int nseg, const float* dyn, nq_stream_t stream) {
  if (!dyn) return NQ_ERR_INVALID;
  return ada_multi(segs, nseg, 0.f, dyn, true, stream);
}

int nq_step_prologue(const int64_t* order, const float* scal, int* step, int64_t* cur_idx, float* cur_scal, int B, int nscal,
                     nq_stream_t stream) {
  if (!order || !scal || !step || !cur_idx || !cur_scal || B <= 0 || B > 256 || nscal <= 0 || nscal > 256) return NQ_ERR_INVALID;
  hipLaunchKernelGGL(step_prologue_kernel, dim3(1), dim3(256), 0, nq_s(stream), order, scal, step, cur_idx, cur_scal, B, nscal);
  return nq_launch_status();
}

int nq_step_prologue_gather(const int64_t* order, const float* scal, int* step, int64_t* cur_idx, float* cur_scal, int B, int nscal,
                            const float* table, int64_t table_rows, int64_t row_len, float* out, nq_stream_t stream) {
  if (!order || !scal || !step || !cur_idx || !cur_scal || B <= 0 || B > 256 || nscal <= 0 || nscal > 256 || !table || !out ||
      table_rows <= 0 || row_len <= 0)
    return NQ_ERR_INVALID;
  const int64_t total = (int64_t)B * row_len;
  int gb = (int)((total + 4095) / 4096);
  if (gb < 1) gb = 1;
  if (gb > 64) gb = 64;
  hipLaunchKernelGGL(step_prologue_gather_kernel, dim3(1 + gb), dim3(256), 0, nq_s(stream), order, scal, step, cur_idx, cur_scal, B,
                     nscal, table, table_rows, row_len, out);
  return nq_launch_status();
}

static int adam_multi(const nq_adam_seg* segs, int nseg, float step_size, float beta1, float beta2, float eps, float bc2_sqrt,
                      const float* dyn, nq_stream_t stream);

int nq_adaround_adam_multi(const nq_ada_adam_seg* segs, int nseg, float reg_b, float step_size, float beta1, float beta2, float eps,
                           float bc2_sqrt, const float* dyn, nq_stream_t stream) {
  if (!segs || nseg <= 0) return NQ_ERR_INVALID;
  for (int base = 0; base < nseg; base += MAXSEG) {
    AdaAdamMulti t;
    t.nseg = (nseg - base < MAXSEG) ? nseg - base : MAXSEG;
    int blocks = 0;
    for (int k = 0; k < t.nseg; ++k) {
      const nq_ada_adam_seg& h = segs[base + k];
      if (!h.x || !h.gy || !h.alpha || !h.delta || !h.zp || !h.m || !h.v || h.rows <= 0 || h.row_len <= 0 ||
          h.row_len > 0x7fffffffLL)
        return NQ_ERR_INVALID;
      AdaAdamSegD& d = t.s[k];
      d.x = h.x; d.gy = h.gy; d.alpha = h.alpha; d.delta = h.delta; d.zp = h.zp; d.m = h.m; d.v = h.v;
      d.n = h.rows * h.row_len; d.row_len = (int)h.row_len; d.per_row = h.per_row;
      d.qmax = (float)(h.n_levels - 1); d.reg_weight = h.reg_weight;
      d.vec = (((uintptr_t)h.x | (uintptr_t)h.gy | (uintptr_t)h.alpha | (uintptr_t)h.m | (uintptr_t)h.v) & 15) == 0;
      t.blk0[k] = blocks;
      blocks += (int)((d.n + TPB * EPT - 1) / (TPB * EPT));
    }
    t.blk0[t.nseg] = blocks;
    hipLaunchKernelGGL(adaround_adam_multi_kernel, dim3((unsigned)blocks), dim3(TPB), 0, nq_s(stream), t, reg_b, step_size,
                       beta1, beta2, eps, bc2_sqrt, dyn);
  }
  return nq_launch_status();
}

int nq_adam_step_multi(const nq_adam_seg* segs, int nseg, float step_size, float beta1, float beta2, float eps,
                       float bc2_sqrt, nq_stream_t stream) {
  return adam_multi(segs, nseg, step_size, beta1, beta2, eps, bc2_sqrt, nullptr, stream);
}

int nq_adam_step_multi_dyn(const nq_adam_seg* segs, int nseg, const float* dyn, float beta1, float beta2, float eps,
                           nq_stream_t stream) {
  if (!dyn) return NQ_ERR_INVALID;
  return adam_multi(segs, nseg, 0.f, beta1, beta2, eps, 1.f, dyn, stream);
}

static int adam_multi(const nq_adam_seg* segs, int nseg, float step_size, float beta1, float beta2, float eps, float bc2_sqrt,
                      const float* dyn, nq_stream_t stream) {
  if (!segs || nseg <= 0) return NQ_ERR_INVALID;
  for (int base = 0; base < nseg; base += MAXSEG) {
    AdamMulti t;
    t.nseg = (nseg - base < MAXSEG) ? nseg - base : MAXSEG;
    int blocks = 0;
    for (int k = 0; k < t.nseg; ++k) {
      const nq_adam_seg& h = segs[base + k];
      if (!h.p || !h.g || !h.m || !h.v || h.n <= 0) return NQ_ERR_INVALID;
      t.s[k].p = h.p; t.s[k].g = h.g; t.s[k].m = h.m; t.s[k].v = h.v; t.s[k].n = h.n;
      t.s[k].vec = (((uintptr_t)h.p | (uintptr_t)h.g | (uintptr_t)h.m | (uintptr_t)h.v) & 15) == 0;
      t.blk0[k] = blocks;
      blocks += (int)((h.n + TPB * EPT - 1) / (TPB * EPT));
    }
    t.blk0[t.nseg] = blocks;
    hipLaunchKernelGGL(adam_multi_kernel, dim3((unsigned)blocks), dim3(TPB), 0, nq_s(stream), t, step_size, beta1, beta2,
                       eps, bc2_sqrt, dyn);
  }
  return nq_launch_status();
}

}
```

neuroquant_amd/ops.py:

```python
import contextlib
import ctypes
import functools
import math
import os
import threading

import torch
from torch.autograd import Function

from . import _lib as L

_QCACHE = {}


def _q(name, *args):
    key = (name, args, os.environ.get("NQ_WGRAD3_PC"), os.environ.get("NQ_WGRAD3_SS"))
    v = _QCACHE.get(key)
    if v is None:
        v = _QCACHE[key] = getattr(L.lib(), name)(*args)
    return v

EPI_PLAIN, EPI_PS_GELU, EPI_TANH, EPI_PS, EPI_DGRAD_GELU = (L.EPI_PLAIN, L.EPI_PS_GELU, L.EPI_TANH, L.EPI_PS,
                                                                L.EPI_DGRAD_GELU)
EPI_X_SPLIT, EPI_Y_SPLIT = 0x100, 0x200


def _stream():
    return torch.cuda.current_stream().cuda_stream


_PROF = None
_PROF_ON = True


def profile_start():
    global _PROF, _PROF_ON
    _PROF, _PROF_ON = {}, True


def profile_sample(on: bool):
    global _PROF_ON
    _PROF_ON = bool(on)


def profile_stop():
    global _PROF
    prof, _PROF = _PROF, None
    torch.cuda.synchronize()
    return {k: (len(v), sum(s.elapsed_time(e) for s, e in v)) for k, v in (prof or {}).items()}


def profiling_active():
    return _PROF is not None and _PROF_ON


def _timed(key, fn):
    if _PROF is None or not _PROF_ON:
        return fn()
    s, e = torch.cuda.Event(enable_timing=True), torch.cuda.Event(enable_timing=True)
    s.record()
    out = fn()
    e.record()
    _PROF.setdefault(key, []).append((s, e))
    return out


def _dev(t: torch.Tensor, name="tensor") -> torch.Tensor:
    if not isinstance(t, torch.Tensor) or not t.is_cuda:
        raise RuntimeError(f"neuroquant_amd: {name} must live on the GPU (no CPU fallback exists)")
    if t.dtype != torch.float32:
        raise RuntimeError(f"neuroquant_amd: {name} must be float32, got {t.dtype}")
    return t if t.is_contiguous() else t.contiguous()


def _p(t):
    return None if t is None else ctypes.c_void_p(t.data_ptr())


def _rows(x: torch.Tensor, scale: torch.Tensor):
    if scale.numel() > 1:
        rows = x.shape[0]
        if scale.numel() != rows:
            raise RuntimeError("delta/zero_point must hold one value per output channel or a single value")
        return rows, x.numel() // rows, 1
    return 1, x.numel(), 0


def scale_init_max(x: torch.Tensor, n_levels: int, channel_wise: bool):
    x = _dev(x.detach(), "x")
    if channel_wise:
        if x.dim() == 4:
            rows, shape = x.shape[0], (-1, 1, 1, 1)
        elif x.dim() == 1:
            rows, shape = 1, (-1,)
        else:
            raise ValueError
    else:
        rows, shape = 1, ()
    delta = torch.empty(rows, device=x.device, dtype=torch.float32)
    zp = torch.empty_like(delta)
    L.check(L.lib().nq_scale_init_max(_p(x), rows, x.numel() // rows, n_levels, _p(delta), _p(zp), _stream()), "scale_init")
    return delta.view(shape), zp.view(shape)


def uaq_forward(x, delta, zp, n_levels, out=None):
    x, delta, zp = _dev(x), _dev(delta), _dev(zp)
    rows, rl, per_row = _rows(x, delta)
    y = torch.empty_like(x) if out is None else out
    L.check(L.lib().nq_uaq_forward(_p(x), _p(delta), _p(zp), _p(y), rows, rl, per_row, n_levels, _stream()), "uaq_forward")
    return y


def uaq_backward(x, gy, delta, zp, n_levels, want_dx=False):
    x, gy, delta, zp = _dev(x), _dev(gy), _dev(delta), _dev(zp)
    rows, rl, per_row = _rows(x, delta)
    dd = torch.empty_like(delta)
    dx = torch.empty_like(x) if want_dx else None
    L.check(L.lib().nq_uaq_backward(_p(x), _p(gy), _p(delta), _p(zp), _p(dd), _p(dx), rows, rl, per_row, n_levels, _stream()),
            "uaq_backward")
    return (dd, dx) if want_dx else dd


def adaround_init(x, delta_uaq, zp_uaq):
    x, d0, z0 = _dev(x.detach()), _dev(delta_uaq.detach()), _dev(zp_uaq.detach())
    rows, rl, per_row = _rows(x, d0)
    d, z, a = torch.empty_like(d0), torch.empty_like(z0), torch.empty_like(x)
    L.check(L.lib().nq_adaround_init(_p(x), _p(d0), _p(z0), _p(d), _p(z), _p(a), rows, rl, per_row, _stream()),
            "adaround_init")
    return d, z, a


def adaround_forward(x, alpha, delta, zp, n_levels, soft, want_xq=False, out=None):
    x, alpha, delta, zp = _dev(x), _dev(alpha), _dev(delta), _dev(zp)
    rows, rl, per_row = _rows(x, delta)
    y = torch.empty_like(x) if out is None else out
    xq = torch.empty_like(x) if want_xq else None
    L.check(L.lib().nq_adaround_forward(_p(x), _p(alpha), _p(delta), _p(zp), _p(y), _p(xq), rows, rl, per_row, n_levels,
                                        1 if soft else 0, _stream()), "adaround_forward")
    return (y, xq) if want_xq else y


def adaround_backward(x, gy, alpha, delta, zp, n_levels, reg_weight=0.0, reg_b=0.0, out=None):
    x, gy, alpha, delta, zp = _dev(x), _dev(gy), _dev(alpha), _dev(delta), _dev(zp)
    rows, rl, per_row = _rows(x, delta)
    da = torch.empty_like(alpha) if out is None else out
    L.check(L.lib().nq_adaround_backward(_p(x), _p(gy), _p(alpha), _p(delta), _p(zp), _p(da), rows, rl, per_row, n_levels,
                                         float(reg_weight), float(reg_b), _stream()), "adaround_backward")
    return da


def round_loss(alpha, b, weight, out=None, accumulate=False):
    alpha = _dev(alpha)
    n = alpha.numel()
    ws = torch.empty(_q("nq_reduce_ws_floats", n), device=alpha.device, dtype=torch.float32)
    if out is None:
        out = torch.zeros((), device=alpha.device, dtype=torch.float32)
    L.check(L.lib().nq_round_loss(_p(alpha), n, float(b), float(weight), _p(ws), _p(out), 1 if accumulate else 0, _stream()),
            "round_loss")
    return out


def adam_step(p, g, m, v, lr, step, beta1=0.9, beta2=0.999, eps=1e-8):
    bc1 = 1 - beta1 ** step
    bc2 = 1 - beta2 ** step
    L.check(L.lib().nq_adam_step(_p(p), _p(_dev(g)), _p(m), _p(v), p.numel(), lr / bc1, beta1, beta2, eps, bc2 ** 0.5,
                                 _stream()), "adam_step")


def _ada_segs(items, out_like=None, opt=None, absent=()):
    segs = ((L.AdaSeg if opt is None else L.AdaAdamSeg) * len(items))()
    outs, keep = [], []
    for i, (sg, (x, gy, alpha, delta, zp, n_levels, reg_weight, soft)) in enumerate(zip(segs, items)):
        t = {"x": x, "gy": gy, "alpha": alpha, "delta": delta, "zp": zp}
        t = {name: None if name in absent else _dev(a, name) for name, a in t.items()}
        for name, a in t.items():
            setattr(sg, name, _p(a))
        sg.rows, sg.row_len, sg.per_row = _rows(t["x"], t["delta"])
        sg.n_levels, sg.reg_weight = n_levels, float(reg_weight)
        if opt is None:
            outs.append(torch.empty_like(t[out_like]))
            sg.out, sg.soft = _p(outs[-1]), int(bool(soft))
        else:
            sg.m, sg.v = _p(opt.m[i]), _p(opt.v[i])
        keep.append(t)
    return segs, outs, keep


def adaround_forward_multi(items):
    segs, outs, keep = _ada_segs([(x, None, alpha, delta, zp, n_levels, 0.0, soft)
                                  for x, alpha, delta, zp, n_levels, soft in items], "x", absent=("gy",))
    L.check(L.lib().nq_adaround_forward_multi(segs, len(items), _stream()), "adaround_forward_multi")
    return outs


def uaq_forward_multi(items):
    segs, outs, keep = _ada_segs([(x, None, None, delta, zp, n_levels, 0.0, 0) for x, delta, zp, n_levels in items], "x",
                                 absent=("gy", "alpha"))
    L.check(L.lib().nq_uaq_forward_multi(segs, len(items), _stream()), "uaq_forward_multi")
    return outs


def uaq_backward_multi(items):
    segs, outs, keep = _ada_segs([(x, gy, None, delta, zp, n_levels, 0.0, 0) for x, gy, delta, zp, n_levels in items], "delta",
                                 absent=("alpha",))
    L.check(L.lib().nq_uaq_backward_multi(segs, len(items), _stream()), "uaq_backward_multi")
    return outs


def step_prologue(order_tab, scal_tab, step_ctr, cur_idx, cur_scal):
    L.check(L.lib().nq_step_prologue(_p(order_tab), _p(scal_tab), _p(step_ctr), _p(cur_idx), _p(cur_scal), cur_idx.numel(),
                                     cur_scal.numel(), _stream()), "step_prologue")


def step_prologue_gather(order_tab, scal_tab, step_ctr, cur_idx, cur_scal, table, out):
    table = _dev(table)
    if step_ctr.numel() < 2 or out.shape[0] != cur_idx.numel() or out[0].numel() != table[0].numel() or not out.is_contiguous():
        raise RuntimeError("step_prologue_gather: step_ctr needs two ints, out must be (B,) + table.shape[1:], contiguous")
    L.check(L.lib().nq_step_prologue_gather(_p(order_tab), _p(scal_tab), _p(step_ctr), _p(cur_idx), _p(cur_scal), cur_idx.numel(),
                                            cur_scal.numel(), _p(table), table.shape[0], table[0].numel(), _p(out), _stream()),
            "step_prologue_gather")


def adaround_backward_multi(items, reg_b=0.0, dyn=None):
    segs, outs, keep = _ada_segs([tuple(it) + (1,) for it in items], "alpha")
    if dyn is not None:
        L.check(L.lib().nq_adaround_backward_multi_dyn(segs, len(items), _p(dyn), _stream()), "adaround_backward_multi_dyn")
    else:
        L.check(L.lib().nq_adaround_backward_multi(segs, len(items), float(reg_b), _stream()), "adaround_backward_multi")
    return outs


def adaround_adam_multi(items, opt, reg_b=0.0, dyn=None, beta1=0.9, beta2=0.999, eps=1e-8):
    assert len(items) == len(opt.params)
    opt.t += 1
    segs, _, keep = _ada_segs([tuple(it) + (1,) for it in items], opt=opt)
    if any(t["alpha"].data_ptr() != p.data_ptr() for t, p in zip(keep, opt.params)):
        raise RuntimeError("adaround_adam_multi: items must be in the optimiser's parameter order")
    step_size, bc2_sqrt = opt.scalars(opt.t, beta1, beta2)
    L.check(L.lib().nq_adaround_adam_multi(segs, len(items), float(reg_b), step_size, beta1, beta2, eps, bc2_sqrt, _p(dyn),
                                           _stream()), "adaround_adam_multi")


class FusedAdam:

    def __init__(self, params, lr):
        self.params = [p for p in params]
        self.lr = lr
        self.t = 0
        self.m = [torch.zeros_like(p) for p in self.params]
        self.v = [torch.zeros_like(p) for p in self.params]

    def zero_grad(self):
        for p in self.params:
            p.grad = None

    def scalars(self, t, beta1=0.9, beta2=0.999):
        return self.lr / (1 - beta1 ** t), (1 - beta2 ** t) ** 0.5

    def step(self, grads=None, beta1=0.9, beta2=0.999, eps=1e-8, dyn=None):
        self.t += 1
        todo = [(p, (p.grad if grads is None else grads[i]), self.m[i], self.v[i]) for i, p in enumerate(self.params)]
        todo = [t for t in todo if t[1] is not None]
        if not todo:
            return
        segs = (L.AdamSeg * len(todo))()
        keep = []
        for sg, (p, g, m, v) in zip(segs, todo):
            g = _dev(g).contiguous()
            keep.append(g)
            sg.p, sg.g, sg.m, sg.v, sg.n = _p(p.data), _p(g), _p(m), _p(v), p.numel()
        if dyn is not None:
            L.check(L.lib().nq_adam_step_multi_dyn(segs, len(todo), _p(dyn), beta1, beta2, eps, _stream()), "adam_step_multi_dyn")
            return
        bc1, bc2 = 1 - beta1 ** self.t, 1 - beta2 ** self.t
        L.check(L.lib().nq_adam_step_multi(segs, len(todo), self.lr / bc1, beta1, beta2, eps, bc2 ** 0.5, _stream()),
                "adam_step_multi")


class _UAQFn(Function):
    @staticmethod
    def forward(ctx, x, delta, zp, n_levels):
        ctx.save_for_backward(x, delta, zp)
        ctx.n_levels = n_levels
        return uaq_forward(x, delta, zp, n_levels)

    @staticmethod
    def backward(ctx, gy):
        x, delta, zp = ctx.saved_tensors
        if ctx.needs_input_grad[0]:
            dd, dx = uaq_backward(x, gy, delta, zp, ctx.n_levels, want_dx=True)
            return dx, dd.view_as(delta), None, None
        return None, uaq_backward(x, gy, delta, zp, ctx.n_levels).view_as(delta), None, None


class _AdaRoundFn(Function):
    @staticmethod
    def forward(ctx, x, alpha, delta, zp, n_levels, soft):
        y, xq = adaround_forward(x, alpha, delta, zp, n_levels, soft, want_xq=True)
        ctx.save_for_backward(x, alpha, delta, zp)
        ctx.n_levels, ctx.soft = n_levels, soft
        ctx.mark_non_differentiable(xq)
        return y, xq

    @staticmethod
    def backward(ctx, gy, _gxq):
        x, alpha, delta, zp = ctx.saved_tensors
        if ctx.needs_input_grad[2] and os.environ.get("NQ_STRICT_GRADS"):
            raise NotImplementedError("d(delta) of the AdaRound fake-quant is not built (never stepped by the reference)")
        da = adaround_backward(x, gy, alpha, delta, zp, ctx.n_levels) if ctx.soft else None
        return None, da, None, None, None, None


class _RoundLossFn(Function):
    @staticmethod
    def forward(ctx, alpha, b, weight):
        ctx.save_for_backward(alpha)
        ctx.b, ctx.weight = float(b), float(weight)
        return round_loss(alpha, b, weight)

    @staticmethod
    def backward(ctx, g):
        (alpha,) = ctx.saved_tensors
        da = torch.empty_like(alpha)
        L.check(L.lib().nq_round_loss_backward(_p(alpha), alpha.numel(), ctx.b, ctx.weight, _p(_dev(g)), _p(da), 0, _stream()),
                "round_loss_backward")
        return da, None, None


def uaq_fake_quant(x, delta, zp, n_levels):
    return _UAQFn.apply(x, delta, zp, n_levels)


def adaround_fake_quant(x, alpha, delta, zp, n_levels, soft):
    return _AdaRoundFn.apply(x, alpha, delta, zp, n_levels, soft)


def round_regulariser(alpha, b, weight):
    return _RoundLossFn.apply(alpha, b, weight)


def next_pow2(n: int) -> int:
    return 1 if n == 0 else 2 ** math.ceil(math.log2(n))


def fwht_channels(w: torch.Tensor, n: int, n_out: int) -> torch.Tensor:
    w = _dev(w)
    co, c, kh, kw = w.shape
    y = torch.empty((co, n_out, kh, kw), device=w.device, dtype=torch.float32)
    L.check(L.lib().nq_fwht(_p(w), _p(y), co, n, kh * kw, c, n_out, _stream()), "fwht")
    return y


def fwht_channels_multi(items):
    segs = (L.FwhtSeg * len(items))()
    outs = []
    for sg, (w, n, n_out) in zip(segs, items):
        w = _dev(w)
        co, c, kh, kw = w.shape
        y = torch.empty((co, n_out, kh, kw), device=w.device, dtype=torch.float32)
        sg.x, sg.y, sg.outer, sg.inner, sg.n, sg.n_in, sg.n_out = _p(w), _p(y), co, kh * kw, n, c, n_out
        outs.append(y)
    if items:
        L.check(L.lib().nq_fwht_multi(segs, len(items), _stream()), "fwht_multi")
    return outs


def _fq_fwht_segs(items, bwd):
    segs = (L.FqFwhtSeg * len(items))()
    outs, keep = [], []
    for sg, (x, alpha, delta, zp, n_levels, soft, n, c_in, reg_weight, gy, m, v) in zip(segs, items):
        x, alpha, delta, zp = _dev(x), _dev(alpha), _dev(delta), _dev(zp)
        sg.x, sg.alpha, sg.delta, sg.zp = _p(x), _p(alpha), _p(delta), _p(zp)
        sg.n_levels, sg.soft, sg.reg_weight = n_levels, int(bool(soft)), float(reg_weight)
        if n:
            co, npad, kh, kw = x.shape
            if npad != n or delta.numel() not in (1, co):
                raise RuntimeError("fused fake-quant + FWHT: x must be (C_out, n, kh, kw) with per-channel or scalar delta")
            sg.outer, sg.inner, sg.n, sg.c_in, sg.per_row = co, kh * kw, n, c_in, int(delta.numel() > 1)
            spatial = (co, c_in, kh, kw)
        else:
            if delta.numel() != 1:
                raise RuntimeError("fused fake-quant + FWHT: a plain tensor takes one scalar delta / zero point")
            sg.outer, sg.inner, sg.n, sg.c_in, sg.per_row = x.numel(), 1, 0, 0, 0
            spatial = tuple(x.shape)
        if bwd:
            gy = _dev(gy)
            if tuple(gy.shape) != spatial:
                raise RuntimeError(f"fused FWHT + d(alpha) + Adam: gradient shape {tuple(gy.shape)} != {spatial}")
            sg.gy, sg.m, sg.v = _p(gy), _p(m), _p(v)
            keep.append((x, gy))
        else:
            y = torch.empty(spatial, device=x.device, dtype=torch.float32)
            sg.y = _p(y)
            outs.append(y)
            keep.append(x)
    return segs, outs, keep


def adaround_fwht_multi(items):
    segs, outs, keep = _fq_fwht_segs([it + (0.0, None, None, None) for it in items], bwd=False)
    L.check(L.lib().nq_adaround_fwht_multi(segs, len(items), _stream()), "adaround_fwht_multi")
    return outs


def fwht_adaround_adam_multi(items, opt, reg_b=0.0, dyn=None, beta1=0.9, beta2=0.999, eps=1e-8):
    assert len(items) == len(opt.params)
    opt.t += 1
    full = []
    for i, (x, gy, alpha, delta, zp, n_levels, reg_weight, n, c_in) in enumerate(items):
        if alpha.data_ptr() != opt.params[i].data_ptr():
            raise RuntimeError("fwht_adaround_adam_multi: items must be in the optimiser's parameter order")
        full.append((x, alpha, delta, zp, n_levels, True, n, c_in, reg_weight, gy, opt.m[i], opt.v[i]))
    segs, _, keep = _fq_fwht_segs(full, bwd=True)
    step_size, bc2_sqrt = opt.scalars(opt.t, beta1, beta2)
    L.check(L.lib().nq_fwht_adaround_adam_multi(segs, len(items), float(reg_b), step_size, beta1, beta2, eps, bc2_sqrt, _p(dyn),
                                                _stream()), "fwht_adaround_adam_multi")


def fq_fwht_fusable(n, inner):
    return n * inner <= 8192 and n <= 1024


class _HadamardFn(Function):
    @staticmethod
    def forward(ctx, w, n, n_out):
        ctx.n, ctx.c_in = n, w.shape[1]
        return fwht_channels(w, n, n_out)

    @staticmethod
    def backward(ctx, g):
        return fwht_channels(g, ctx.n, ctx.c_in), None, None


def hadamard_along_channel_weight(x: torch.Tensor, n_out=None) -> torch.Tensor:
    n = next_pow2(x.shape[1])
    if n != x.shape[1] and n_out is None:
        raise ValueError("channel count must be a power of two (pad first, quant_layer.py:45-49)")
    return _HadamardFn.apply(x, n, x.shape[1] if n_out is None else n_out)


def hadamard_weight_of(w: torch.Tensor) -> torch.Tensor:
    n = next_pow2(w.shape[1])
    return fwht_channels(w.detach(), n, n)


@functools.lru_cache(maxsize=None)
def conv_operand_dims(cin, cout, k):
    kr, ld = ctypes.c_int(0), ctypes.c_int(0)
    L.check(L.lib().nq_conv_operand_dims(cin, cout, k, ctypes.byref(kr), ctypes.byref(ld)), "conv_operand_dims")
    return kr.value, ld.value


def _wl_segs(items):
    segs = (L.WLSeg * len(items))()
    outs, keep = [], []
    for sg, (w, need_fwd, need_bwd) in zip(segs, items):
        w = _dev(w)
        cout, cin, k, _ = w.shape
        wt = wb = None
        kf = lf = kb = lb = 0
        if need_fwd:
            kf, lf = conv_operand_dims(cin, cout, k)
            wt = torch.empty(kf * lf, device=w.device, dtype=torch.float32)
        if need_bwd:
            kb, lb = conv_operand_dims(cout, cin, k)
            wb = torch.empty(kb * lb, device=w.device, dtype=torch.float32)
        sg.w, sg.wt_fwd, sg.wt_bwd, sg.Cout, sg.Cin, sg.k = _p(w), _p(wt), _p(wb), cout, cin, k
        sg.krows_fwd, sg.ld_fwd, sg.krows_bwd, sg.ld_bwd = kf, lf, kb, lb
        outs.append((wt, (kf, lf), wb, (kb, lb)))
        keep.append(w)
    return segs, outs, keep


def _wl3_segs(items):
    segs = (L.WL3Seg * len(items))()
    outs, keep = [], []
    for sg, (w, transposed) in zip(segs, items):
        w = _dev(w)
        cw_out, cw_in, k, _ = w.shape
        cin, cout = (cw_out, cw_in) if transposed else (cw_in, cw_out)
        outs.append(torch.empty(_q("nq_conv3_weight_bytes", cin, cout, k), device=w.device, dtype=torch.uint8))
        sg.w, sg.wt3, sg.Cin, sg.Cout, sg.k, sg.transposed = _p(w), _p(outs[-1]), cin, cout, k, int(bool(transposed))
        keep.append(w)
    return segs, outs, keep


def weight_layouts(w, need_bwd):
    (sg,), (out,), (w,) = _wl_segs([(w, True, need_bwd)])
    L.check(L.lib().nq_weight_layouts(_p(w), _p(out[0]), _p(out[2]), sg.Cout, sg.Cin, sg.k, sg.krows_fwd, sg.ld_fwd, sg.krows_bwd,
                                      sg.ld_bwd, _stream()), "weight_layouts")
    return out


def weight_layouts_multi(items):
    segs, outs, keep = _wl_segs(items)
    if items:
        L.check(L.lib().nq_weight_layouts_multi(segs, len(items), _stream()), "weight_layouts_multi")
    return outs


def weight_layouts_all(items3, items_f):
    if not items3 or not items_f or os.environ.get("NQ_LAYOUTS_ALL", "1") == "0":
        return weight_layout3_multi(items3), weight_layouts_multi(items_f)
    segs3, outs3, keep3 = _wl3_segs(items3)
    segsf, outsf, keepf = _wl_segs(items_f)
    L.check(L.lib().nq_weight_layouts_all(segs3, len(items3), segsf, len(items_f), _stream()), "weight_layouts_all")
    return outs3, outsf


def _conv_outputs(x, cout, epilogue, r):
    B, _, H, W = x.shape
    y = z = None
    if epilogue in (EPI_PS_GELU, EPI_PS):
        z = torch.empty((B, cout // (r * r), H * r, W * r), device=x.device, dtype=torch.float32)
        if epilogue == EPI_PS_GELU:
            y = torch.empty_like(z)
    elif epilogue == EPI_DGRAD_GELU:
        y = torch.empty((B, cout * r * r, H // r, W // r), device=x.device, dtype=torch.float32)
    else:
        y = torch.empty((B, cout, H, W), device=x.device, dtype=torch.float32)
    return y, z


def conv_forward_raw(x, wt, dims, bias, cout, k, epilogue, r, zprev=None, fmt=0):
    B, cin, H, W = x.shape
    y, z = _conv_outputs(x, cout, epilogue, r)
    nws = _q("nq_conv_forward_ws_floats", B, cin, H, W, cout, k)
    ws = torch.empty(nws, device=x.device, dtype=torch.float32) if nws else None
    _timed(("conv_igemm", k, cin, cout, H, W, B, epilogue),
           lambda: L.check(L.lib().nq_conv_forward(_p(x), _p(wt), _p(bias), _p(y), _p(z), _p(ws), B, cin, H, W, cout, k,
                                                   dims[0], dims[1], r, epilogue | fmt, 0, _p(zprev), _stream()), "conv_forward"))
    return y, z


def conv3_supported(B, cin, H, W, cout, k):
    return bool(_q("nq_conv3_supported", B, cin, H, W, cout, k))


def conv3_split_io(B, cin, H, W, cout, k):
    return int(_q("nq_conv3_split_io", B, cin, H, W, cout, k))


def conv_wgrad3_split_io(B, cin, H, W, cout, k):
    return int(_q("nq_conv_wgrad3_split_io", B, cin, H, W, cout, k))


def conv_split_out(B, cin, H, W, cout, k, r, epilogue, has_bias=False):
    return bool(_q("nq_conv_split_out", B, cin, H, W, cout, k, r, epilogue, 0, 1 if has_bias else 0))


def split_words(x):
    x = _dev(x).contiguous()
    y = torch.empty_like(x)
    L.check(L.lib().nq_split_words(_p(x), _p(y), x.numel(), _stream()), "split_words")
    return y


def weight_layout3(w, transposed=False):
    (sg,), (buf,), (w,) = _wl3_segs([(w, transposed)])
    L.check(L.lib().nq_weight_layout3(_p(w), _p(buf), sg.Cin, sg.Cout, sg.k, sg.transposed, _stream()), "weight_layout3")
    return buf


def weight_layout3_multi(items):
    segs, outs, keep = _wl3_segs(items)
    if items:
        L.check(L.lib().nq_weight_layout3_multi(segs, len(items), _stream()), "weight_layout3_multi")
    return outs


def conv3_forward_raw(x, wt3, bias, cout, k, epilogue, r, zprev=None, fmt=0):
    B, cin, H, W = x.shape
    y, z = _conv_outputs(x, cout, epilogue, r)
    nws = _q("nq_conv_forward3_ws_floats", B, cin, H, W, cout, k)
    ws = torch.empty(nws, device=x.device, dtype=torch.float32) if nws else None
    _timed(("conv_igemm3", k, cin, cout, H, W, B, epilogue),
           lambda: L.check(L.lib().nq_conv_forward3(_p(x), _p(wt3), _p(bias), _p(y), _p(z), _p(zprev), _p(ws), B, cin, H, W,
                                                    cout, k, r, epilogue | fmt, _stream()), "conv_forward3"))
    return y, z


def conv_wgrad3_supported(B, cin, H, W, cout, k):
    return bool(_q("nq_conv_wgrad3_supported", B, cin, H, W, cout, k))


class PendingReductions:

    def __init__(self):
        self.segs, self.keep = [], []

    def add(self, seg, *tensors):
        self.segs.append(seg)
        self.keep.append(tensors)

    def flush(self):
        if self.segs:
            arr = (L.WgrSeg * len(self.segs))(*self.segs)
            L.check(L.lib().nq_wgrad_reduce_multi(arr, len(self.segs), _stream()), "wgrad_reduce_multi")
        self.segs, self.keep = [], []


def conv_wgrad3_raw(x, dy, cout, k, want_db, out=None, defer=None, fmt=0):
    B, cin, H, W = x.shape
    ws = torch.empty(_q("nq_conv_wgrad3_ws_floats", B, cin, H, W, cout, k), device=x.device, dtype=torch.float32)
    dw = torch.empty((cout, cin, k, k), device=x.device, dtype=torch.float32) if out is None else out[0]
    db = (torch.empty(cout, device=x.device, dtype=torch.float32) if out is None else out[1]) if want_db else None
    if defer is not None:
        seg = L.WgrSeg()
        _timed(("conv_wgrad3", k, cin, cout, H, W, B, 0),
               lambda: L.check(L.lib().nq_conv_wgrad3_slabs_fmt(_p(x), _p(dy), _p(dw), _p(db), _p(ws), B, cin, H, W, cout, k,
                                                                ctypes.byref(seg), fmt, _stream()), "conv_wgrad3_slabs"))
        defer.add(seg, ws, dw, db)
        return dw, db
    _timed(("conv_wgrad3", k, cin, cout, H, W, B, 0),
           lambda: L.check(L.lib().nq_conv_wgrad3_fmt(_p(x), _p(dy), _p(dw), _p(db), _p(ws), B, cin, H, W, cout, k, fmt,
                                                      _stream()), "conv_wgrad3"))
    return dw, db


def channel_sum(x):
    x = _dev(x)
    B, C = x.shape[0], x.shape[1]
    out = torch.empty(C, device=x.device, dtype=torch.float32)
    ws = torch.empty(512 * C, device=x.device, dtype=torch.float32)
    L.check(L.lib().nq_channel_sum(_p(x), _p(out), _p(ws), B, C, x.numel() // (B * C), _stream()), "channel_sum")
    return out


def conv_wgrad_swapped3_supported(B, cin, H, W, cout, k):
    return (cout <= 4 and cin > 4 and cout * k * k <= 64 and conv_wgrad3_supported(B, cout, H, W, cin, k)
            and _q("nq_conv_wgrad3_ws_floats", B, cout, H, W, cin, k) > 4)


def conv_wgrad_swapped3(x, dy, cout, k, want_db, out=None, defer=None):
    B, cin, H, W = x.shape
    ws = torch.empty(_q("nq_conv_wgrad3_ws_floats", B, cout, H, W, cin, k), device=x.device, dtype=torch.float32)
    dw = torch.empty((cout, cin, k, k), device=x.device, dtype=torch.float32) if out is None else out[0]
    if defer is not None:
        seg = L.WgrSeg()
        _timed(("conv_wgrad3", k, cout, cin, H, W, B, 0),
               lambda: L.check(L.lib().nq_conv_wgrad3_swapped_slabs(_p(x), _p(dy), _p(dw), _p(ws), B, cin, H, W, cout, k,
                                                                    ctypes.byref(seg), _stream()), "conv_wgrad3_swapped_slabs"))
        defer.add(seg, ws, dw)
    else:
        _timed(("conv_wgrad3", k, cout, cin, H, W, B, 0),
               lambda: L.check(L.lib().nq_conv_wgrad3_swapped(_p(x), _p(dy), _p(dw), _p(ws), B, cin, H, W, cout, k, _stream()),
                               "conv_wgrad3_swapped"))
    db = None
    if want_db:
        db = channel_sum(dy)
        if out is not None:
            out[1].copy_(db)
            db = out[1]
    return dw, db


def conv_wgrad_raw(x, dy, cout, k, want_db, out=None, defer=None):
    B, cin, H, W = x.shape
    ws = torch.empty(_q("nq_conv_wgrad_ws_floats", B, cin, H, W, cout, k), device=x.device, dtype=torch.float32)
    dw = torch.empty((cout, cin, k, k), device=x.device, dtype=torch.float32) if out is None else out[0]
    db = (torch.empty(cout, device=x.device, dtype=torch.float32) if out is None else out[1]) if want_db else None
    if defer is not None:
        seg = L.WgrSeg()
        _timed(("conv_wgrad", k, cin, cout, H, W, B, 0),
               lambda: L.check(L.lib().nq_conv_wgrad_slabs(_p(x), _p(dy), _p(dw), _p(db), _p(ws), B, cin, H, W, cout, k,
                                                           0, ctypes.byref(seg), _stream()), "conv_wgrad_slabs"))
        defer.add(seg, ws, dw, db)
        return dw, db
    _timed(("conv_wgrad", k, cin, cout, H, W, B, 0),
           lambda: L.check(L.lib().nq_conv_wgrad(_p(x), _p(dy), _p(dw), _p(db), _p(ws), B, cin, H, W, cout, k,
                                                 0, _stream()), "conv_wgrad"))
    return dw, db


class _ConvFn(Function):

    @staticmethod
    def forward(ctx, x, w, b, epilogue, r):
        x, w = _dev(x, "x"), _dev(w, "weight")
        b = _dev(b, "bias") if b is not None else None
        cout, cin, k, k2 = w.shape
        if k != k2 or x.shape[1] != cin:
            raise ValueError(f"conv shape mismatch: x {tuple(x.shape)} w {tuple(w.shape)}")
        need_dx = ctx.needs_input_grad[0]
        wt, dims, wb, dims_b = weight_layouts(w, need_dx)
        y, z = conv_forward_raw(x, wt, dims, b, cout, k, epilogue, r)
        ctx.save_for_backward(x, wb, z if epilogue == EPI_PS_GELU else (y if epilogue == EPI_TANH else None))
        ctx.meta = (cout, cin, k, epilogue, r, dims_b, b is not None)
        return y

    @staticmethod
    def backward(ctx, gy):
        x, wb, aux = ctx.saved_tensors
        cout, cin, k, epilogue, r, dims_b, has_b = ctx.meta
        B, _, H, W = x.shape
        gy = _dev(gy, "grad")
        if epilogue == EPI_PS_GELU:
            dconv = torch.empty((B, cout, H, W), device=x.device, dtype=torch.float32)
            L.check(L.lib().nq_ps_gelu_backward(_p(gy), _p(aux), _p(dconv), B, cout // (r * r), H, W, r, _stream()),
                    "ps_gelu_backward")
        elif epilogue == EPI_TANH:
            dconv = torch.empty_like(gy)
            L.check(L.lib().nq_tanh_out_backward(_p(gy), _p(aux), _p(dconv), gy.numel(), _stream()), "tanh_backward")
        else:
            dconv = gy
        dx = dw = db = None
        if ctx.needs_input_grad[0]:
            dx, _ = conv_forward_raw(dconv, wb, dims_b, None, cin, k, EPI_PLAIN, 1)
        if ctx.needs_input_grad[1] or (has_b and ctx.needs_input_grad[2]):
            dw, db = conv_wgrad_raw(x, dconv, cout, k, has_b)
        return dx, dw, db, None, None


_PRECISION = None


def set_conv_precision(precision):
    global _PRECISION
    if precision not in (None, "fp32", "bf16x3"):
        raise ValueError(f"unknown conv precision {precision!r}")
    _PRECISION = precision


def get_conv_precision():
    return _PRECISION or os.environ.get("NQ_CONV_PRECISION", "bf16x3")


def _use3(precision):
    return (precision or get_conv_precision()) == "bf16x3"


def _conv_plain(x, w, precision=None):
    cout, cin, k, _ = w.shape
    B, _, H, W = x.shape
    if _use3(precision) and conv3_supported(B, cin, H, W, cout, k):
        return conv3_forward_raw(x, weight_layout3(w), None, cout, k, EPI_PLAIN, 1)[0]
    wt, dims, _, _ = weight_layouts(w, need_bwd=False)
    return conv_forward_raw(x, wt, dims, None, cout, k, EPI_PLAIN, 1)[0]


def _dgrad_plain(gy, w, precision=None):
    cout, cin, k, _ = w.shape
    B, _, H, W = gy.shape
    if _use3(precision) and conv3_supported(B, cout, H, W, cin, k):
        return conv3_forward_raw(gy, weight_layout3(w, transposed=True), None, cin, k, EPI_PLAIN, 1)[0]
    _, _, wb, dims_b = weight_layouts(w, need_bwd=True)
    return conv_forward_raw(gy, wb, dims_b, None, cin, k, EPI_PLAIN, 1)[0]


def _wgrad_plain(x, gy, k, precision=None):
    B, cin, H, W = x.shape
    cout = gy.shape[1]
    if _use3(precision) and conv_wgrad3_supported(B, cin, H, W, cout, k):
        return conv_wgrad3_raw(x, gy, cout, k, False)[0]
    if _use3(precision) and conv_wgrad_swapped3_supported(B, cin, H, W, cout, k):
        return conv_wgrad_swapped3(x, gy, cout, k, False)[0]
    return conv_wgrad_raw(x, gy, cout, k, False)[0]


class _ConvF(Function):
    @staticmethod
    def forward(ctx, x, w):
        x, w = _dev(x, "x").contiguous(), _dev(w, "weight").contiguous()
        ctx.save_for_backward(x, w)
        return _conv_plain(x, w)

    @staticmethod
    def backward(ctx, gy):
        x, w = ctx.saved_tensors
        gy = gy.contiguous()
        return (_ConvD.apply(gy, w) if ctx.needs_input_grad[0] else None,
                _ConvWg.apply(x, gy, w.shape[-1]) if ctx.needs_input_grad[1] else None)


class _ConvD(Function):
    @staticmethod
    def forward(ctx, gy, w):
        gy, w = _dev(gy, "gy").contiguous(), _dev(w, "weight").contiguous()
        ctx.save_for_backward(gy, w)
        return _dgrad_plain(gy, w)

    @staticmethod
    def backward(ctx, g):
        gy, w = ctx.saved_tensors
        g = g.contiguous()
        return (_ConvF.apply(g, w) if ctx.needs_input_grad[0] else None,
                _ConvWg.apply(g, gy, w.shape[-1]) if ctx.needs_input_grad[1] else None)


class _ConvWg(Function):
    @staticmethod
    def forward(ctx, x, gy, k):
        x, gy = _dev(x, "x").contiguous(), _dev(gy, "gy").contiguous()
        ctx.save_for_backward(x, gy)
        return _wgrad_plain(x, gy, k)

    @staticmethod
    def backward(ctx, G):
        x, gy = ctx.saved_tensors
        G = G.contiguous()
        return (_ConvD.apply(gy, G) if ctx.needs_input_grad[0] else None,
                _ConvF.apply(x, G) if ctx.needs_input_grad[1] else None, None)


_ACT_BASE = {"gelu": 0, "tanh": 3}


def act_dd_raw(x, kind, order, g=None, g2=None):
    x = _dev(x, "x")
    g = _dev(g, "g") if g is not None else None
    g2 = _dev(g2, "g2") if g2 is not None else None
    y = torch.empty_like(x)
    L.check(L.lib().nq_act_dd(_p(x), _p(g), _p(g2), _p(y), x.numel(), _ACT_BASE[kind] + order, _stream()), "act_dd")
    return y


class _ActDD(Function):

    @staticmethod
    def forward(ctx, x, g, kind, order):
        ctx.save_for_backward(x, g)
        ctx.kind, ctx.order = kind, order
        return act_dd_raw(x, kind, order, g)

    @staticmethod
    def backward(ctx, gy):
        x, g = ctx.saved_tensors
        gy = gy.contiguous()
        dx = dg = None
        if ctx.needs_input_grad[0]:
            if ctx.order >= 2:
                raise NotImplementedError("third derivative of the activation is not built (Hessian-vector products need two)")
            dx = _ActDD2.apply(x, gy, g, ctx.kind, ctx.order + 1)
        if g is not None and ctx.needs_input_grad[1]:
            dg = _ActDD.apply(x, gy, ctx.kind, ctx.order)
        return dx, dg, None, None


class _ActDD2(Function):

    @staticmethod
    def forward(ctx, x, g, h, kind, order):
        ctx.save_for_backward(x, g, h)
        ctx.kind, ctx.order = kind, order
        return act_dd_raw(x, kind, order, g, h)

    @staticmethod
    def backward(ctx, gy):
        x, g, h = ctx.saved_tensors
        gy = gy.contiguous()
        dx = dg = dh = None
        if ctx.needs_input_grad[0]:
            if ctx.order >= 2 or h is not None:
                raise NotImplementedError("third derivative of the activation is not built (Hessian-vector products need two)")
            dx = _ActDD2.apply(x, gy, g, ctx.kind, ctx.order + 1)
        if ctx.needs_input_grad[1]:
            dg = _ActDD2.apply(x, gy, h, ctx.kind, ctx.order) if h is not None else _ActDD.apply(x, gy, ctx.kind, ctx.order)
        if h is not None and ctx.needs_input_grad[2]:
            dh = _ActDD2.apply(x, gy, g, ctx.kind, ctx.order)
        return dx, dg, dh, None, None


def gelu_dd(x):
    return _ActDD.apply(x.contiguous(), None, "gelu", 0)


def tanh_out_dd(x):
    return _ActDD.apply(x.contiguous(), None, "tanh", 0)


def pixel_shuffle_raw(x, r, inverse=False):
    x = _dev(x, "x")
    B, Cx, Hx, Wx = x.shape
    if inverse:
        if Hx % r or Wx % r:
            raise ValueError("pixel_unshuffle: spatial size not divisible by r")
        C, H, W = Cx, Hx // r, Wx // r
        y = torch.empty((B, C * r * r, H, W), device=x.device, dtype=torch.float32)
    else:
        if Cx % (r * r):
            raise ValueError("pixel_shuffle: channels not divisible by r*r")
        C, H, W = Cx // (r * r), Hx, Wx
        y = torch.empty((B, C, H * r, W * r), device=x.device, dtype=torch.float32)
    L.check(L.lib().nq_pixel_shuffle(_p(x), _p(y), B, C, H, W, r, 1 if inverse else 0, _stream()), "pixel_shuffle")
    return y


class _PixelShuffleDD(Function):

    @staticmethod
    def forward(ctx, x, r, inverse):
        ctx.r, ctx.inverse = r, inverse
        return pixel_shuffle_raw(x.contiguous(), r, inverse)

    @staticmethod
    def backward(ctx, gy):
        return _PixelShuffleDD.apply(gy.contiguous(), ctx.r, not ctx.inverse), None, None


def pixel_shuffle_dd(x, r):
    return _PixelShuffleDD.apply(x, r, False)


class _BiasAddDD(Function):

    @staticmethod
    def forward(ctx, x, bias):
        x, bias = _dev(x, "x").contiguous(), _dev(bias, "bias").contiguous()
        y = torch.empty_like(x)
        B, C = x.shape[0], x.shape[1]
        L.check(L.lib().nq_bias_add(_p(x), _p(bias), _p(y), B, C, x.numel() // (B * C), _stream()), "bias_add")
        return y

    @staticmethod
    def backward(ctx, gy):
        gy = gy.contiguous()
        return (gy if ctx.needs_input_grad[0] else None), (_ChannelSumDD.apply(gy) if ctx.needs_input_grad[1] else None)


class _ChannelSumDD(Function):
    @staticmethod
    def forward(ctx, x):
        ctx.shape = tuple(x.shape)
        return channel_sum(x.contiguous())

    @staticmethod
    def backward(ctx, g):
        g = _dev(g, "g").contiguous()
        B, C = ctx.shape[0], ctx.shape[1]
        y = torch.empty(ctx.shape, device=g.device, dtype=torch.float32)
        L.check(L.lib().nq_bias_add(None, _p(g), _p(y), B, C, y.numel() // (B * C), _stream()), "bias_add")
        return y


def conv2d_dd(x, w, b=None):
    y = _ConvF.apply(x, w)
    return y if b is None else _BiasAddDD.apply(y, b)


def decoder_stack_dd(emb, spec, weights):
    x = emb
    for l, ((k, r, act), (W, b)) in enumerate(zip(spec.layers, weights)):
        x = conv2d_dd(x, W, b)
        if l == 0 and spec.fc_hw != (1, 1):
            x = _space_from_channels(x, *spec.fc_hw)
        if r > 1:
            x = pixel_shuffle_dd(x, r)
        if act:
            x = gelu_dd(x)
    return tanh_out_dd(x) if spec.tanh_out else x


def conv2d_fused(x, w, b, epilogue=EPI_PLAIN, r=1):
    if not torch.is_grad_enabled() or not (x.requires_grad or w.requires_grad or (b is not None and b.requires_grad)):
        x, w = _dev(x, "x"), _dev(w, "weight")
        b = _dev(b, "bias") if b is not None else None
        cout, cin, k, k2 = w.shape
        if k != k2 or x.shape[1] != cin:
            raise ValueError(f"conv shape mismatch: x {tuple(x.shape)} w {tuple(w.shape)}")
        B, _, H, W = x.shape
        if _use3(None) and conv3_supported(B, cin, H, W, cout, k):
            return conv3_forward_raw(x, weight_layout3(w), b, cout, k, epilogue, r)[0]
        wt, dims, _, _ = weight_layouts(w, False)
        return conv_forward_raw(x, wt, dims, b, cout, k, epilogue, r)[0]
    return _ConvFn.apply(x, w, b, epilogue, r)


class DecoderSpec:

    def __init__(self, layers, fc_hw=(1, 1), tanh_out=True, precision=None):
        self.layers = [tuple(l) for l in layers]
        self.fc_hw = tuple(fc_hw)
        self.tanh_out = tanh_out
        self.precision = precision or get_conv_precision()
        if self.precision not in ("fp32", "bf16x3"):
            raise ValueError(f"unknown conv precision {self.precision!r}")
        self.overlap_wgrad = os.environ.get("NQ_WGRAD_STREAM", "0") == "1"


def _space_from_channels(x, fh, fw):
    n, c, h, w = x.shape
    return x.view(n, -1, fh, fw, h, w).permute(0, 1, 4, 2, 5, 3).reshape(n, -1, fh * h, fw * w)


def _channels_from_space(g, fh, fw):
    n, c, hh, ww = g.shape
    return g.view(n, c, hh // fh, fh, ww // fw, fw).permute(0, 1, 3, 5, 2, 4).reshape(n, c * fh * fw, hh // fh, ww // fw)


_ARENA_TLS = threading.local()


def _arena_state():
    return getattr(_ARENA_TLS, "state", (None, False))


def set_grad_arena_hook(fn, two_phase=False):
    _ARENA_TLS.state = (fn, bool(two_phase) and fn is not None)


@contextlib.contextmanager
def grad_arena_hook(fn, two_phase=False):
    prev = _arena_state()
    set_grad_arena_hook(fn, two_phase)
    try:
        yield
    finally:
        _ARENA_TLS.state = prev


def arena_reduced(img):
    return bool(getattr(getattr(img, "grad_fn", None), "nq_arena_reduced", False))


_LOSS_TLS = threading.local()


@contextlib.contextmanager
def fused_head_loss(tgt=None, cache_u8=None, idx=None):
    prev = getattr(_LOSS_TLS, "req", None)
    _LOSS_TLS.req = None if os.environ.get("NQ_FUSED_HEAD_LOSS", "1") == "0" else (tgt, cache_u8, idx)
    try:
        yield
    finally:
        _LOSS_TLS.req = prev


def head_forward_loss_raw(x, wt, dims, bias, cout, k, tgt=None, cache_u8=None, idx=None):
    B, cin, H, W = x.shape
    if cout != 3 or k != 3 or (W & 3) or (dims[1] & 3) or os.environ.get("NQ_HEAD_FWD") == "1":
        return None
    if cache_u8 is not None:
        if not cache_u8.is_cuda or cache_u8.dtype != torch.uint8 or not cache_u8.is_contiguous() \
                or tuple(cache_u8.shape[1:]) != (cout, H, W) or idx is None or idx.numel() != B:
            return None
        idx = idx.to(device=x.device, dtype=torch.int64).contiguous()
        tgt = None
    elif tgt is not None:
        if not tgt.is_cuda or tgt.dtype != torch.float32 or tuple(tgt.shape) != (B, cout, H, W):
            return None
        tgt = tgt.contiguous()
    else:
        return None
    y = torch.empty((B, cout, H, W), device=x.device, dtype=torch.float32)
    dconv = torch.empty_like(y)
    loss = torch.empty((), device=x.device, dtype=torch.float32)
    db = torch.empty(cout, device=x.device, dtype=torch.float32)
    ws = torch.empty(_q("nq_head_forward_loss_ws_floats", B, H, W), device=x.device, dtype=torch.float32)
    rc = _timed(("conv_igemm", k, cin, cout, H, W, B, EPI_TANH),
                lambda: L.lib().nq_head_forward_loss(_p(x), _p(wt), dims[1], _p(bias), _p(y), _p(tgt), _p(cache_u8), _p(idx), _p(loss),
                                                     _p(dconv), _p(db), _p(ws), B, cin, H, W, B * H * W, 1.0, _stream()))
    if rc == -2:
        return None
    L.check(rc, "head_forward_loss")
    return y, loss, dconv, db


_SIDE_STREAMS = {}


def _side_stream(device):
    key = torch.device(device).index
    if key not in _SIDE_STREAMS:
        _SIDE_STREAMS[key] = torch.cuda.Stream(device=device)
    return _SIDE_STREAMS[key]


class LayerPlan:
    __slots__ = ("k", "r", "act", "cin", "cout", "has_bias", "H", "W", "epi", "fwd", "dgrad", "wgrad", "x_split", "g_split",
                 "fwd_fmt", "dgrad_epi", "dgrad_r", "dgrad_fmt", "wgrad_fmt")


def plan_decoder(spec, wshapes, has_bias, B, H, W, want_emb_grad):
    n = len(spec.layers)
    use3 = spec.precision == "bf16x3"
    plan = []
    fio, bio, wio = [0] * n, [0] * n, [0] * n
    for l, (k, r, act) in enumerate(spec.layers):
        p = LayerPlan()
        p.k, p.r, p.act, (p.cout, p.cin), p.has_bias, p.H, p.W = k, r, act, wshapes[l], bool(has_bias[l]), H, W
        cout, cin = p.cout, p.cin
        if l == n - 1:
            p.epi = EPI_TANH if spec.tanh_out else EPI_PLAIN
        else:
            p.epi = EPI_PS_GELU if act else EPI_PS if r > 1 else EPI_PLAIN
        p.fwd = "bf16x3" if use3 and conv3_supported(B, cin, H, W, cout, k) else "fp32"
        if l == 0:
            p.dgrad = "fp32" if want_emb_grad else None
        else:
            p.dgrad = "bf16x3" if use3 and conv3_supported(B, cout, H, W, cin, k) else "fp32"
        if use3 and conv_wgrad3_supported(B, cin, H, W, cout, k):
            p.wgrad = "bf16x3"
        elif use3 and conv_wgrad_swapped3_supported(B, cin, H, W, cout, k):
            p.wgrad = "swapped3"
        else:
            p.wgrad = "fp32"
        if p.fwd == "bf16x3":
            fio[l] = conv3_split_io(B, cin, H, W, cout, k)
        if p.dgrad == "bf16x3":
            bio[l] = conv3_split_io(B, cout, H, W, cin, k)
        if p.wgrad == "bf16x3":
            wio[l] = conv_wgrad3_split_io(B, cin, H, W, cout, k)
        below_act = l > 0 and spec.layers[l - 1][2]
        p.dgrad_epi, p.dgrad_r = (EPI_DGRAD_GELU, spec.layers[l - 1][1]) if below_act else (EPI_PLAIN, 1)
        if l == n - 1 and l > 0 and p.dgrad == "fp32" and below_act \
                and conv_split_out(B, cout, H, W, cin, k, p.dgrad_r, EPI_DGRAD_GELU):
            bio[l] = EPI_Y_SPLIT
        plan.append(p)
        if l == 0:
            H, W = H * spec.fc_hw[0], W * spec.fc_hw[1]
        H, W = H * r, W * r
    split_on = use3 and os.environ.get("NQ_SPLIT_IO", "1") != "0"
    for l, p in enumerate(plan):
        below_act = l > 0 and plan[l - 1].act
        p.x_split = bool(split_on and l >= 2 and below_act and (fio[l - 1] & EPI_Y_SPLIT) and (fio[l] & EPI_X_SPLIT)
                         and (wio[l] & 1))
        p.g_split = bool(split_on and 1 <= l < n - 1 and (bio[l + 1] & EPI_Y_SPLIT) and (bio[l] & EPI_X_SPLIT) and (wio[l] & 2)
                         and below_act and not (l == 1 and spec.fc_hw != (1, 1)))
    for l, p in enumerate(plan):
        p.fwd_fmt = (EPI_X_SPLIT if p.x_split else 0) | (EPI_Y_SPLIT if l + 1 < n and plan[l + 1].x_split else 0)
        p.dgrad_fmt = (EPI_X_SPLIT if p.g_split else 0) | (EPI_Y_SPLIT if l > 0 and plan[l - 1].g_split else 0)
        p.wgrad_fmt = (1 if p.x_split else 0) | (2 if p.g_split else 0)
    return plan


class _DecoderStackFn(Function):

    @staticmethod
    def forward(ctx, emb, spec, *wb):
        x = _dev(emb, "embedding")
        n = len(spec.layers)
        Ws = [_dev(w, "weight") for w in wb[0::2]]
        bs = [_dev(b, "bias") if b is not None else None for b in wb[1::2]]
        plan = plan_decoder(spec, [tuple(W.shape[:2]) for W in Ws], [b is not None for b in bs], x.shape[0], x.shape[2],
                            x.shape[3], ctx.needs_input_grad[0])
        keys3 = [(l, t) for l, p in enumerate(plan) for t, route in ((False, p.fwd), (True, p.dgrad)) if route == "bf16x3"]
        keys32 = [l for l, p in enumerate(plan) if "fp32" in (p.fwd, p.dgrad)]
        ops3, ops32 = weight_layouts_all([(Ws[l], t) for l, t in keys3],
                                         [(Ws[l], plan[l].fwd == "fp32", plan[l].dgrad == "fp32") for l in keys32])
        ops3, ops32 = dict(zip(keys3, ops3)), dict(zip(keys32, ops32))
        saved_in, saved_z = [], []
        ctx.wbk, ctx.dims_b, ctx.w3t = [None] * n, [None] * n, [None] * n
        zprev = None
        fused_loss = None
        for l, p in enumerate(plan):
            wt, dims, wbk, dims_b = ops32.get(l, (None,) * 4)
            if p.dgrad == "fp32":
                ctx.wbk[l], ctx.dims_b[l] = wbk, dims_b
            ctx.w3t[l] = ops3.get((l, True))
            if l == n - 1 and p.epi == EPI_TANH and p.fwd == "fp32" and getattr(_LOSS_TLS, "req", None) is not None:
                fused_loss = head_forward_loss_raw(x, wt, dims, bs[l], p.cout, p.k, *_LOSS_TLS.req)
            if fused_loss is not None:
                y, z = fused_loss[0], None
            elif p.fwd == "bf16x3":
                y, z = conv3_forward_raw(x, ops3[l, False], bs[l], p.cout, p.k, p.epi, p.r, fmt=p.fwd_fmt)
            else:
                y, z = conv_forward_raw(x, wt, dims, bs[l], p.cout, p.k, p.epi, p.r)
            saved_in.append(x)
            saved_z.append(zprev)
            x, zprev = (y, z) if p.epi == EPI_PS_GELU else (z, None) if p.epi == EPI_PS else (y, None)
            if l == 0 and spec.fc_hw != (1, 1):
                x = _space_from_channels(x, *spec.fc_hw).contiguous()
        ctx.spec, ctx.plan, ctx.n = spec, plan, n
        ctx.save_for_backward(x, *saved_in, *saved_z)
        ctx.nq_arena, ctx.nq_arena_reduced = _arena_state(), False
        ctx.nq_head = _HeadHandoff() if spec.tanh_out else None
        if fused_loss is not None:
            ctx.nq_head.loss, ctx.nq_head.dconv, ctx.nq_head.db = fused_loss[1], fused_loss[2], fused_loss[3]
            ctx.nq_head.version = fused_loss[2]._version
        return x

    @staticmethod
    def backward(ctx, g_img):
        hook = ctx.nq_arena[0]
        steps = _decoder_backward_steps(ctx, g_img)
        while True:
            try:
                part, last = next(steps)
            except StopIteration as done:
                return done.value
            if last is None:
                hook(part)
            else:
                hook(part, last)


def _decoder_backward_steps(ctx, g_img):
    spec, plan, n = ctx.spec, ctx.plan, ctx.n
    saved = ctx.saved_tensors
    img, xs, zs = saved[0], saved[1:1 + n], saved[1 + n:]
    d_emb = None
    g = _dev(g_img, "grad")
    head_db = None
    head = ctx.nq_head
    if head is not None and head.loss is not None:
        head.dconv = head.db = head.loss = None
    if head is not None and head.dconv is not None:
        if head.dconv.data_ptr() != g.data_ptr() or g.shape != head.dconv.shape:
            raise RuntimeError("neuroquant_amd: the gradient returned by ops.l2_loss_head_grad must be passed to "
                               "backward() as it is (it already contains the tanh backward of this decoder)")
        dconv = g
        head_db = head.db if g._version == head.version else None
        head.dconv = head.db = None
    elif spec.tanh_out:
        dconv = torch.empty_like(g)
        L.check(L.lib().nq_tanh_out_backward(_p(g), _p(img), _p(dconv), g.numel(), _stream()), "tanh_backward")
    else:
        dconv = g
    grads = [None] * (2 * n)
    main = torch.cuda.current_stream()
    side = _side_stream(g.device) if spec.overlap_wgrad else None
    keep = []

    arena = views = None
    arena_hook, arena_two_phase = ctx.nq_arena
    if arena_hook is not None:
        sizes = []
        for p in plan:
            sizes += [p.cout * p.cin * p.k * p.k, p.cout if p.has_bias else 0]
        arena = torch.empty(sum(sizes), device=g.device, dtype=torch.float32)
        views, off = [], 0
        for l, p in enumerate(plan):
            wv = arena[off:off + sizes[2 * l]].view(p.cout, p.cin, p.k, p.k)
            off += sizes[2 * l]
            bv = arena[off:off + sizes[2 * l + 1]] if sizes[2 * l + 1] else None
            off += sizes[2 * l + 1]
            views.append((wv, bv))

    pending = PendingReductions() if side is None and os.environ.get("NQ_DEFER_REDUCE", "1") != "0" else None

    def wgrad(l, dconv):
        p = plan[l]
        out = views[l] if views is not None else None
        if p.wgrad == "bf16x3":
            return conv_wgrad3_raw(xs[l], dconv, p.cout, p.k, p.has_bias, out=out, defer=pending, fmt=p.wgrad_fmt)
        if p.wgrad == "swapped3":
            if l == n - 1 and p.has_bias and head_db is not None:
                dw, _ = conv_wgrad_swapped3(xs[l], dconv, p.cout, p.k, False, out=out, defer=pending)
                if out is not None:
                    out[1].copy_(head_db)
                    return dw, out[1]
                return dw, head_db
            return conv_wgrad_swapped3(xs[l], dconv, p.cout, p.k, p.has_bias, out=out, defer=pending)
        return conv_wgrad_raw(xs[l], dconv, p.cout, p.k, p.has_bias, out=out, defer=pending)

    def dgrad(l, dconv):
        p = plan[l]
        if not plan[l - 1].act and plan[l - 1].r != 1:
            raise NotImplementedError("PixelShuffle without activation between decoder layers")
        zp = zs[l] if p.dgrad_epi == EPI_DGRAD_GELU else None
        if p.dgrad == "bf16x3":
            d, _ = conv3_forward_raw(dconv, ctx.w3t[l], None, p.cin, p.k, p.dgrad_epi, p.dgrad_r, zprev=zp, fmt=p.dgrad_fmt)
        else:
            d, _ = conv_forward_raw(dconv, ctx.wbk[l], ctx.dims_b[l], None, p.cin, p.k, p.dgrad_epi, p.dgrad_r, zprev=zp,
                                    fmt=p.dgrad_fmt)
        if not plan[l - 1].act and l == 1 and spec.fc_hw != (1, 1):
            d = _channels_from_space(d, *spec.fc_hw).contiguous()
        return d

    def emb_grad(dconv):
        return conv_forward_raw(dconv, ctx.wbk[0], ctx.dims_b[0], None, plan[0].cin, plan[0].k, EPI_PLAIN, 1)[0]

    if arena is not None and arena_two_phase and n > 1:
        dcs = [None] * n
        dcs[n - 1] = dconv
        for l in range(n - 1, 0, -1):
            dcs[l - 1] = dgrad(l, dcs[l])
        if plan[0].dgrad is not None:
            d_emb = emb_grad(dcs[0])
        flops = [p.cout * p.cin * p.k ** 2 * p.H * p.W for p in plan]
        split, late = n - 1, flops[n - 1]
        while split > 1 and late < 0.8 * sum(flops):
            split -= 1
            late += flops[split]
        for l in range(split):
            grads[2 * l], grads[2 * l + 1] = wgrad(l, dcs[l])
            dcs[l] = None
        off = sum(sizes[:2 * split])
        if pending is not None:
            pending.flush()
        yield arena[:off], False
        for l in range(split, n):
            grads[2 * l], grads[2 * l + 1] = wgrad(l, dcs[l])
            dcs[l] = None
        if pending is not None:
            pending.flush()
        yield arena[off:], True
        ctx.nq_arena_reduced = True
        return (d_emb, None) + tuple(grads)

    for l in range(n - 1, -1, -1):
        if side is not None:
            keep.append(dconv)
            side.wait_stream(main)
            with torch.cuda.stream(side):
                dw, db = wgrad(l, dconv)
            for t in (dw, db):
                if t is not None:
                    t.record_stream(main)
        else:
            dw, db = wgrad(l, dconv)
        grads[2 * l], grads[2 * l + 1] = dw, db
        if l == 0:
            if plan[0].dgrad is not None:
                d_emb = emb_grad(dconv)
            break
        dconv = dgrad(l, dconv)
    if side is not None:
        main.wait_stream(side)
        keep.clear()
    if pending is not None:
        pending.flush()
    if arena is not None:
        yield arena, None
        ctx.nq_arena_reduced = True
    return (d_emb, None) + tuple(grads)


class _ManualNode:

    def __init__(self, n_inputs, want_emb_grad=False):
        self.needs_input_grad = (bool(want_emb_grad), False) + (True,) * n_inputs
        self.saved_tensors = ()

    def save_for_backward(self, *tensors):
        self.saved_tensors = tensors


def decoder_forward_manual(emb, spec: DecoderSpec, weights, two_phase=True):
    flat = []
    for W, b in weights:
        flat += [W, b]
    node = _ManualNode(len(flat))
    with torch.no_grad():
        img = _DecoderStackFn.forward(node, emb, spec, *flat)
    node.nq_arena = ("manual", bool(two_phase))
    return img, node


def decoder_backward_steps(node, g_img):
    return _decoder_backward_steps(node, g_img)


def decoder_stack(emb, spec: DecoderSpec, weights):
    flat = []
    for W, b in weights:
        flat += [W, b]
    return _DecoderStackFn.apply(emb, spec, *flat)


class _L2LossFn(Function):

    @staticmethod
    def forward(ctx, pred, tgt):
        pred, tgt = _dev(pred, "pred"), _dev(tgt, "tgt")
        n = pred.numel()
        mean_count = n // pred.shape[1]
        loss = torch.empty((), device=pred.device, dtype=torch.float32)
        dpred = torch.empty_like(pred) if ctx.needs_input_grad[0] else None
        ws = torch.empty(_q("nq_reduce_ws_floats", n), device=pred.device, dtype=torch.float32)
        L.check(L.lib().nq_l2_loss(_p(pred), _p(tgt), _p(loss), _p(dpred), _p(ws), n, mean_count, 1.0, _stream()), "l2_loss")
        ctx.save_for_backward(dpred)
        return loss

    @staticmethod
    def backward(ctx, g):
        (dpred,) = ctx.saved_tensors
        return dpred * g, None


def l2_loss(pred, tgt):
    return _L2LossFn.apply(pred, tgt)


def l2_loss_and_grad(pred, tgt):
    pred_d, tgt = _dev(pred.detach(), "pred"), _dev(tgt, "tgt")
    n = pred_d.numel()
    loss = torch.empty((), device=pred_d.device, dtype=torch.float32)
    dpred = torch.empty_like(pred_d)
    ws = torch.empty(_q("nq_reduce_ws_floats", n), device=pred_d.device, dtype=torch.float32)
    L.check(L.lib().nq_l2_loss(_p(pred_d), _p(tgt), _p(loss), _p(dpred), _p(ws), n, n // pred_d.shape[1], 1.0, _stream()),
            "l2_loss")
    return loss, dpred


class _HeadHandoff:
    __slots__ = ("dconv", "db", "version", "loss")

    def __init__(self):
        self.dconv = self.db = self.version = self.loss = None


def l2_loss_tanh_head_raw(pred, tgt=None, cache_u8=None, idx=None):
    pred_d = _dev(pred.detach(), "pred")
    if pred_d.dim() != 4:
        return None
    B, C, H, W = pred_d.shape
    if (H * W) % 4096 != 0 or C > 1024:
        return None
    if cache_u8 is not None:
        if not cache_u8.is_cuda or cache_u8.dtype != torch.uint8 or not cache_u8.is_contiguous() \
                or tuple(cache_u8.shape[1:]) != (C, H, W) or idx.numel() != B:
            raise RuntimeError("frame cache must be a contiguous uint8 GPU tensor of the image's shape")
        idx = idx.to(device=pred_d.device, dtype=torch.int64).contiguous()
    else:
        tgt = _dev(tgt, "tgt")
    n = pred_d.numel()
    loss = torch.empty((), device=pred_d.device, dtype=torch.float32)
    dconv = torch.empty_like(pred_d)
    db = torch.empty(C, device=pred_d.device, dtype=torch.float32)
    ws = torch.empty(2 * _q("nq_reduce_ws_floats", n), device=pred_d.device, dtype=torch.float32)
    L.check(L.lib().nq_l2_loss_tanh_head(_p(pred_d), _p(tgt) if cache_u8 is None else None,
                                         _p(cache_u8) if cache_u8 is not None else None,
                                         _p(idx) if cache_u8 is not None else None, _p(loss), _p(dconv), _p(db), _p(ws),
                                         B, C, H * W, n // C, 1.0, _stream()), "l2_loss_tanh_head")
    return loss, dconv, db


def l2_loss_head_grad(pred, tgt=None, cache_u8=None, idx=None, node=None):
    head = getattr(node if node is not None else pred.grad_fn, "nq_head", None)
    if not isinstance(head, _HeadHandoff) or os.environ.get("NQ_FUSED_LOSS", "1") == "0":
        return None
    if head.loss is not None:
        loss, head.loss = head.loss, None
        return loss, head.dconv
    out = l2_loss_tanh_head_raw(pred, tgt, cache_u8, idx)
    if out is None:
        return None
    loss, head.dconv, head.db = out
    head.version = head.dconv._version
    return loss, head.dconv


def frame_psnr(out, gt):
    out, gt = _dev(out.detach()), _dev(gt.detach())
    frames = out.shape[0]
    flen = out.numel() // frames
    sse = torch.empty(frames, device=out.device, dtype=torch.float32)
    L.check(L.lib().nq_frame_sse(_p(out), _p(gt), _p(sse), frames, flen, _stream()), "frame_sse")
    return -10 * torch.log10(sse / flen + 1e-9)


def ms_ssim(out, gt):
    out, gt = _dev(out.detach(), "out"), _dev(gt.detach(), "gt")
    if out.dim() != 4 or out.shape != gt.shape:
        raise RuntimeError(f"neuroquant_amd: ms_ssim takes two (F, C, H, W) tensors of one shape, got {tuple(out.shape)} and "
                           f"{tuple(gt.shape)}")
    F_, C, H, W = out.shape
    if min(H, W) <= 160:
        raise ValueError(f"ms_ssim: the smaller side of the image must exceed (11 - 1) * 2**4 = 160, got {H} x {W}")
    res = torch.empty(F_, device=out.device, dtype=torch.float32)
    ws = torch.empty(_q("nq_ms_ssim_ws_floats", F_, C, H, W), device=out.device, dtype=torch.float32)
    L.check(L.lib().nq_ms_ssim(_p(out), _p(gt), _p(res), _p(ws), F_, C, H, W, _stream()), "ms_ssim")
    return res


def gather_frames_u8(frames_u8: torch.Tensor, idx: torch.Tensor) -> torch.Tensor:
    if not frames_u8.is_cuda or frames_u8.dtype != torch.uint8 or not frames_u8.is_contiguous():
        raise RuntimeError("frame cache must be a contiguous uint8 GPU tensor")
    idx = idx.to(device=frames_u8.device, dtype=torch.int64).contiguous()
    n = idx.numel()
    flen = frames_u8[0].numel()
    out = torch.empty((n,) + tuple(frames_u8.shape[1:]), device=frames_u8.device, dtype=torch.float32)
    L.check(L.lib().nq_gather_frames_u8(_p(frames_u8), _p(idx), _p(out), n, flen, _stream()), "gather_frames")
    return out
```

neuroquant_amd/quantization/calib_model.py:

```python
import contextlib
import logging
import os

import torch
import torch.nn as nn

from .. import ops
from ..utils import allreduce_mean_
from .data_utils import LinearTempDecay
from .quant_layer import QuantModule
from .quant_model import QuantModel
from .quantizer import AdaRoundQuantizer, lp_loss


def _quant_modules(module: nn.Module, out=None):
    out = [] if out is None else out
    for name, child in module.named_children():
        if 'encoder' in name:
            continue
        if isinstance(child, QuantModule):
            out.append(child)
        else:
            _quant_modules(child, out)
    return out


class LossFunction:

    def __init__(self, model: nn.Module, round_loss: str = 'relaxation', weight: float = 1., rec_loss: str = 'mse',
                 max_count: int = 2000, b_range: tuple = (10, 2), decay_start: float = 0.0, warmup: float = 0.0,
                 p: float = 2.):
        self.model = model
        self.round = round_loss
        self.weight = weight
        self.rec = rec_loss
        self.loss_start = max_count * warmup
        self.p = p
        self.temp_decay = LinearTempDecay(max_count, rel_start_decay=warmup + (1 - warmup) * decay_start,
                                          start_b=b_range[0], end_b=b_range[1])
        self.count = 0
        self.round_loss = 0

    def collect_round_loss(self, module, b):
        for m in _quant_modules(module):
            self.round_loss = self.round_loss + ops.round_regulariser(m.weight_quantizer.alpha, b, self.weight)

    def __call__(self, pred, tgt, grad=None):
        self.count += 1
        if self.rec != 'mse':
            raise NotImplementedError(f'rec_loss {self.rec!r}: the drivers hard-code opt_mode="mse"')
        rec_loss = lp_loss(pred, tgt, p=self.p)
        b = self.temp_decay(self.count)
        if self.count < self.loss_start or self.round == 'none':
            b = self.round_loss = 0
        elif self.round == 'relaxation':
            self.round_loss = 0
            self.collect_round_loss(self.model, b)
        else:
            raise NotImplementedError
        total_loss = self.round_loss + rec_loss
        if self.count % 500 == 0:
            logging.info('Total loss:\t{:.4f} (rec:{:.4f}, round:{:.4f})\tb={:.2f}\tcount={}'.format(
                float(total_loss), float(rec_loss), float(self.round_loss), b, self.count))
        return total_loss


class _Layer:

    def __init__(self, m: QuantModule, hadamard: bool):
        self.m = m
        self.hadamard = hadamard
        self.src = m.hadamard_weight if hadamard else m.weight.data
        self.n = self.src.shape[1]
        self.c_in = m.weight.shape[1]
        self.bias = m.bias.data
        self.W = self.b = None

    def forward_uaq(self):
        wq, bq = self.m.weight_quantizer, self.m.bias_quantizer
        Wq = ops.uaq_forward(self.src, wq.delta.data, wq.zero_point, wq.n_levels)
        self._finish(Wq, ops.uaq_forward(self.bias, bq.delta.data, bq.zero_point, bq.n_levels))

    def forward_ada(self):
        wq, bq = self.m.weight_quantizer, self.m.bias_quantizer
        Wq = ops.adaround_forward(self.src, wq.alpha.data, wq.delta.data, wq.zero_point, wq.n_levels, wq.soft_targets)
        self._finish(Wq, ops.adaround_forward(self.bias, bq.alpha.data, bq.delta.data, bq.zero_point, bq.n_levels,
                                              bq.soft_targets))

    def uaq_items(self):
        wq, bq = self.m.weight_quantizer, self.m.bias_quantizer
        return [(self.src, wq.delta.data, wq.zero_point, wq.n_levels), (self.bias, bq.delta.data, bq.zero_point, bq.n_levels)]

    def ada_items(self):
        wq, bq = self.m.weight_quantizer, self.m.bias_quantizer
        return [(self.src, wq.alpha.data, wq.delta.data, wq.zero_point, wq.n_levels, wq.soft_targets),
                (self.bias, bq.alpha.data, bq.delta.data, bq.zero_point, bq.n_levels, bq.soft_targets)]

    def _finish(self, Wq, b, transformed=False):
        self.W = (ops.fwht_channels(Wq, self.n, self.c_in) if self.hadamard and not transformed else Wq).requires_grad_(True)
        self.b = b.requires_grad_(True)
        self.m._wb_override = (self.W, self.b)

    def grads(self):
        gW = self.W.grad
        if self.hadamard:
            gW = ops.fwht_channels(gW, self.n, self.n)
        return gW, self.b.grad

    def release(self):
        self.m._wb_override = None
        self.W = self.b = None


_AVG_OK = {}


def _avg_unsupported(err):
    msg = str(err).lower()
    return "avg" in msg or "reduceop" in msg or "reduce op" in msg or "unsupported reduction" in msg


def _mean_all_reduce(t):
    import torch.distributed as dist
    be = dist.get_backend()
    if _AVG_OK.get(be, True):
        try:
            w = dist.all_reduce(t, op=dist.ReduceOp.AVG, async_op=True)
            _AVG_OK[be] = True
            return w.wait
        except (RuntimeError, ValueError, NotImplementedError) as err:
            if not _avg_unsupported(err):
                raise
            _AVG_OK[be] = False
    w = dist.all_reduce(t, op=dist.ReduceOp.SUM, async_op=True)
    scale = 1.0 / dist.get_world_size()

    def fin():
        w.wait()
        if scale != 1.0:
            t.mul_(scale)
    return fin


def model_reconstruction(model: QuantModel, cali_data: torch.Tensor, gt, arch: str = 'hnerv', batch_size: int = 8,
                         iters: int = 20000, weight: float = 0.01, opt_mode: str = 'mse', hadamard: bool = True,
                         b_range: tuple = (20, 2), warmup: float = 0.0, p: float = 2.0, lr: float = 0.0015,
                         recorder: list = None, max_steps: int = None, step_hook=None, probe=None):
    if arch not in ('hnerv', 'nerv'):
        raise ValueError
    if opt_mode != 'mse' or p != 2.0:
        raise NotImplementedError('only opt_mode="mse", p=2 is on the calibration path')
    model.set_quant_state(True)
    device = next(model.parameters()).device
    layers = [_Layer(m, hadamard) for m in _quant_modules(model)]
    for L in layers:
        if not L.m.weight_quantizer.inited:
            L.m.weight_quantizer(L.src)
        if not L.m.bias_quantizer.inited:
            L.m.bias_quantizer(L.bias)
    done = 0
    dp = torch.distributed.is_available() and torch.distributed.is_initialized() and \
        (torch.distributed.get_world_size() > 1 or bool(os.environ.get("NQ_DP_REHEARSAL")))

    hook_scope = contextlib.nullcontext()
    if dp and device.type == 'cuda':
        import torch.distributed as dist
        pending = []

        def reduce_part(part, last=True):
            pending.append(_mean_all_reduce(part))
            if last:
                for fin in pending:
                    fin()
                pending.clear()

        hook_scope = ops.grad_arena_hook(reduce_part, two_phase=os.environ.get("NQ_DP_OVERLAP", "1") != "0")

    use_graph = (os.environ.get("NQ_GRAPH", "1") != "0" and device.type == 'cuda' and recorder is None
                 and probe is None and hasattr(gt, 'epoch_indices') and hasattr(gt, 'cache'))
    dp_graph = use_graph and dp and os.environ.get("NQ_DP_GRAPH", "0") == "1"
    if dp and not dp_graph:
        use_graph = False
    fused_stack = None
    if dp_graph:
        from ..models._decode import _fused_stack
        fused_stack = _fused_stack(model.model) if hasattr(model, 'model') else None
        if fused_stack is None:
            dp_graph = use_graph = False

    def _capture_staged(run_body):
        graphs, parts = [torch.cuda.CUDAGraph()], []
        pool = torch.cuda.graph_pool_handle()
        cap = torch.cuda.Stream()
        cap.wait_stream(torch.cuda.current_stream())
        torch.cuda.synchronize()
        with torch.cuda.stream(cap):
            graphs[0].capture_begin(pool=pool, capture_error_mode="thread_local")

            def cut(k, part):
                graphs[-1].capture_end()
                parts.append(part)
                graphs.append(torch.cuda.CUDAGraph())
                graphs[-1].capture_begin(pool=pool, capture_error_mode="thread_local")

            run_body(cut)
            graphs[-1].capture_end()
        torch.cuda.current_stream().wait_stream(cap)
        return graphs, parts

    def _replay_staged(staged_graph):
        import torch.distributed as dist
        graphs, parts = staged_graph
        works = []
        for g, part in zip(graphs[:-1], parts):
            g.replay()
            works.append(_mean_all_reduce(part))
        for fin in works:
            fin()
        graphs[-1].replay()

    fuse_had = bool(hadamard) and os.environ.get("NQ_FUSED_FWHT", "1") != "0" and \
        all(ops.fq_fwht_fusable(L.n, L.src.shape[2] * L.src.shape[3]) for L in layers)

    def run(epochs, params, opt_lr, max_count, ada):
        nonlocal done
        opt = ops.FusedAdam(params, lr=opt_lr)
        loss_start = max_count * warmup
        temp = LinearTempDecay(max_count, rel_start_decay=warmup, start_b=b_range[0], end_b=b_range[1])
        count = 0

        def sched(c):
            b = temp(c)
            reg_on = ada and not (c < loss_start)
            return (b if reg_on else 0), reg_on

        def body(get_batch, b, reg_on, dyn, want_log, staged=None):
            img, inputs = get_batch()
            if ada and fuse_had:
                items = []
                for L in layers:
                    (xw, aw, dw_, zw, nlw, sw), (xb, ab, db_, zb, nlb, sb) = L.ada_items()
                    items += [(xw, aw, dw_, zw, nlw, sw, L.n, L.c_in), (xb, ab, db_, zb, nlb, sb, 0, 0)]
                fq = ops.adaround_fwht_multi(items)
                for i, L in enumerate(layers):
                    L._finish(fq[2 * i], fq[2 * i + 1], transformed=True)
            elif ada:
                fq = ops.adaround_forward_multi(
                    [it for L in layers for it in L.ada_items()])
                if hadamard:
                    had = ops.fwht_channels_multi([(fq[2 * i], L.n, L.c_in) for i, L in enumerate(layers)])
                    for i, L in enumerate(layers):
                        L._finish(had[i], fq[2 * i + 1], transformed=True)
                else:
                    for i, L in enumerate(layers):
                        L._finish(fq[2 * i], fq[2 * i + 1])
            else:
                fq = ops.uaq_forward_multi([it for L in layers for it in L.uaq_items()])
                if hadamard:
                    had = ops.fwht_channels_multi([(fq[2 * i], L.n, L.c_in) for i, L in enumerate(layers)])
                    for i, L in enumerate(layers):
                        L._finish(had[i], fq[2 * i + 1], transformed=True)
                else:
                    for i, L in enumerate(layers):
                        L._finish(fq[2 * i], fq[2 * i + 1])
            node = None
            loss_req = ops.fused_head_loss(cache_u8=img[0], idx=img[1]) if isinstance(img, tuple) else ops.fused_head_loss(tgt=img)
            with loss_req:
                if staged is None:
                    img_out, _, _ = model(inputs)
                else:
                    spec, provs = fused_stack
                    img_out, node = ops.decoder_forward_manual(inputs, spec, [p() for p in provs],
                                                               two_phase=os.environ.get("NQ_DP_OVERLAP", "1") != "0")
            fused = ops.l2_loss_head_grad(img_out, cache_u8=img[0], idx=img[1], node=node) if isinstance(img, tuple) \
                else ops.l2_loss_head_grad(img_out, tgt=img, node=node)
            if fused is None:
                if isinstance(img, tuple):
                    img = ops.gather_frames_u8(img[0], img[1])
                fused = ops.l2_loss_and_grad(img_out, img)
            rec, dimg = fused
            if staged is None:
                img_out.backward(dimg)
            else:
                steps, k = ops.decoder_backward_steps(node, dimg), 0
                while True:
                    try:
                        part, _last = next(steps)
                    except StopIteration as fin:
                        res = fin.value
                        break
                    staged(k, part)
                    k += 1
                for i, L in enumerate(layers):
                    L.W.grad, L.b.grad = res[2 + 2 * i], res[3 + 2 * i]
            if dp and staged is None and not ops.arena_reduced(img_out):
                allreduce_mean_([t.grad for L in layers for t in (L.W, L.b)])
            if want_log:
                rl = torch.zeros((), device=device)
                if reg_on:
                    for L in layers:
                        ops.round_loss(L.m.weight_quantizer.alpha.data, b, weight, out=rl, accumulate=True)
                total, rl_f = float(rec) + float(rl), float(rl)
                if recorder is not None:
                    recorder.append((total, rl_f, float(b), count))
                if count % 500 == 0:
                    logging.info('Total loss:\t{:.4f} (rec:{:.4f}, round:{:.4f})\tb={:.2f}\tcount={}'.format(
                        total, float(rec), rl_f, b, count))
            grads = []
            if ada and fuse_had and probe is None and os.environ.get("NQ_FUSED_ADAM", "1") != "0":
                items = []
                for L in layers:
                    wq, bq = L.m.weight_quantizer, L.m.bias_quantizer
                    items.append((L.src, L.W.grad, wq.alpha.data, wq.delta.data, wq.zero_point, wq.n_levels,
                                  weight if (reg_on or dyn is not None) else 0.0, L.n, L.c_in))
                    items.append((L.bias, L.b.grad, bq.alpha.data, bq.delta.data, bq.zero_point, bq.n_levels, 0.0, 0, 0))
                ops.fwht_adaround_adam_multi(items, opt, b, dyn=dyn)
                grads = None
            elif ada:
                items = []
                gWs = ops.fwht_channels_multi([(L.W.grad, L.n, L.n) for L in layers]) if hadamard else None
                for i, L in enumerate(layers):
                    gW, gb = (gWs[i], L.b.grad) if hadamard else L.grads()
                    wq, bq = L.m.weight_quantizer, L.m.bias_quantizer
                    items.append((L.src, gW, wq.alpha.data, wq.delta.data, wq.zero_point, wq.n_levels,
                                  weight if (reg_on or dyn is not None) else 0.0))
                    items.append((L.bias, gb, bq.alpha.data, bq.delta.data, bq.zero_point, bq.n_levels, 0.0))
                if probe is None and os.environ.get("NQ_FUSED_ADAM", "1") != "0":
                    ops.adaround_adam_multi(items, opt, b, dyn=dyn)
                    grads = None
                else:
                    grads = ops.adaround_backward_multi(items, b, dyn=dyn)
            else:
                gWs = ops.fwht_channels_multi([(L.W.grad, L.n, L.n) for L in layers]) if hadamard else None
                items = []
                for i, L in enumerate(layers):
                    gW, gb = (gWs[i], L.b.grad) if hadamard else L.grads()
                    wq, bq = L.m.weight_quantizer, L.m.bias_quantizer
                    items.append((L.src, gW, wq.delta.data, wq.zero_point, wq.n_levels))
                    items.append((L.bias, gb, bq.delta.data, bq.zero_point, bq.n_levels))
                grads = ops.uaq_backward_multi(items)
            if probe is not None:
                probe('ada' if ada else 'uaq', layers, grads)
            if grads is not None:
                opt.step(grads, dyn=dyn)
            for L in layers:
                L.release()

        if not use_graph:
            for _ in range(epochs):
                model.train()
                for sample in gt:
                    if step_hook is not None:
                        step_hook(done)
                    if max_steps is not None and done >= max_steps:
                        return
                    count += 1
                    b, reg_on = sched(count)
                    img = sample['img'].to(device, non_blocking=True)
                    inputs = cali_data[sample['idx'].to(device, non_blocking=True)]
                    body(lambda: (img, inputs), b, reg_on, None, recorder is not None or count % 500 == 0)
                    done += 1
            return

        st = None
        graph, warm = None, 0
        for _ in range(epochs):
            model.train()
            idx_tab = gt.epoch_indices()
            nb, per = idx_tab.shape
            if st is None or st['order'].shape[0] < nb or st['cur_idx'].numel() != per:
                st = dict(order=torch.zeros((nb, per), device=device, dtype=torch.int64),
                          scal=torch.zeros((nb, 4), device=device, dtype=torch.float32),
                          step=torch.zeros(2, device=device, dtype=torch.int32),
                          emb=torch.zeros((per,) + tuple(cali_data.shape[1:]), device=device, dtype=torch.float32),
                          cur_idx=torch.zeros(per, device=device, dtype=torch.int64),
                          cur_scal=torch.zeros(4, device=device, dtype=torch.float32))
                graph, warm = None, 0
            rows = []
            for c in range(count + 1, count + nb + 1):
                b, reg_on = sched(c)
                rows.append((float(b), 1.0 if reg_on else 0.0) + opt.scalars(opt.t + (c - count)))
            st['scal'][:nb].copy_(torch.tensor(rows, dtype=torch.float32), non_blocking=True)
            st['order'][:nb].copy_(idx_tab)
            st['step'].zero_()

            def static_batch():
                ops.step_prologue_gather(st['order'], st['scal'], st['step'], st['cur_idx'], st['cur_scal'], cali_data, st['emb'])
                return (gt.cache.frames, st['cur_idx']), st['emb']

            for i in range(nb):
                if step_hook is not None:
                    step_hook(done)
                if max_steps is not None and done >= max_steps:
                    return
                count += 1
                b, reg_on = sched(count)
                want_log = count % 500 == 0
                if want_log or warm < 3 or ops.profiling_active():
                    body(static_batch, b, reg_on, st['cur_scal'], want_log)
                    warm += 1
                elif graph is None and dp_graph:
                    graph = _capture_staged(lambda cut: body(static_batch, b, reg_on, st['cur_scal'], False, staged=cut))
                    _replay_staged(graph)
                elif graph is None:
                    graph = torch.cuda.CUDAGraph()
                    with torch.cuda.graph(graph):
                        body(static_batch, b, reg_on, st['cur_scal'], False)
                    graph.replay()
                elif dp_graph:
                    _replay_staged(graph)
                    opt.t += 1
                else:
                    graph.replay()
                    opt.t += 1
                done += 1

    with hook_scope:
        params = []
        for L in layers:
            params += [L.m.weight_quantizer.delta, L.m.bias_quantizer.delta]
        epochs1 = int(0.05 * iters / len(gt))
        run(epochs1, params, 0.001, 2100, ada=False)
        torch.cuda.empty_cache()

        params = []
        for L in layers:
            m = L.m
            m.weight_quantizer = AdaRoundQuantizer(uaq=m.weight_quantizer, round_mode='learned_hard_sigmoid',
                                                   weight_tensor=(m.hadamard_weight if hadamard else m.org_weight).data)
            m.bias_quantizer = AdaRoundQuantizer(uaq=m.bias_quantizer, round_mode='learned_hard_sigmoid',
                                                 weight_tensor=m.bias.data)
            m.weight_quantizer.soft_targets = True
            m.bias_quantizer.soft_targets = True
            params += [m.weight_quantizer.alpha, m.bias_quantizer.alpha]
        run(int(iters / len(gt)) - epochs1, params, lr, iters, ada=True)
        torch.cuda.empty_cache()

    for L in layers:
        L.m.weight_quantizer.soft_targets = False
```

Baseline: 475.2 it/s (B=2 frames per iteration-equivalent, summed over GPUs).

## Fold wgrad slab reductions into AdaRound Adam and fuse fake-quant into layouts

Defers the pending weight-gradient split-K reduction so the fused AdaRound+Adam kernel sums the slabs directly while it updates alpha, m and v. This removes a separate reduction launch and the round trip of the reduced gradient through memory. It also adds an optional lazy fake-quant path where the weight layout kernel applies AdaRound quantisation while reformatting. That path is gated behind NQ_FOLD_LAYOUTS=1, which is off by default. The reduction folding adds bookkeeping about when a pending reduction may be deferred and taken.

After: 475.2 it/s (B=2 frames per iteration-equivalent, summed over GPUs). About the same (-0.0%).

```diff
diff --git a/include/nq_hip.h b/include/nq_hip.h
--- a/include/nq_hip.h
+++ b/include/nq_hip.h
@@ -163,6 +163,28 @@
 } nq_wl3_seg;
 NQ_API int nq_weight_layout3_multi(const nq_wl3_seg* segs, int nseg, nq_stream_t stream);
 NQ_API int nq_weight_layouts_all(const nq_wl3_seg* segs3, int n3, const nq_wl_seg* segsf, int nf, nq_stream_t stream);
+typedef struct nq_fq_par {
+  const float* alpha;
+  const float* delta;
+  const float* zp;
+  int per_row, n_levels, soft;
+} nq_fq_par;
+typedef struct nq_qwl3_seg {
+  nq_wl3_seg l;
+  nq_fq_par q;
+} nq_qwl3_seg;
+typedef struct nq_qwl_seg {
+  nq_wl_seg l;
+  nq_fq_par q;
+} nq_qwl_seg;
+typedef struct nq_qel_seg {
+  const float* x;
+  float* out;
+  int64_t rows, row_len;
+  nq_fq_par q;
+} nq_qel_seg;
+NQ_API int nq_quant_layouts_all(const nq_qwl3_seg* segs3, int n3, const nq_qwl_seg* segsf, int nf, const nq_qel_seg* segse, int ne,
+                         nq_stream_t stream);
 NQ_API int nq_conv_forward3(const float* x, const void* wt3, const float* bias, float* y, float* z, const float* zprev, float* ws, int B,
                      int Cin, int H, int W, int Cout, int k, int r, int epilogue, nq_stream_t stream);
 
@@ -199,6 +221,9 @@
 NQ_API int nq_conv_wgrad_slabs(const float* x, const float* dy, float* dw, float* db, float* ws, int B, int Cin, int H, int W, int Cout,
                         int k, int x_gelu, nq_wgr_seg* seg, nq_stream_t stream);
 NQ_API int nq_wgrad_reduce_multi(const nq_wgr_seg* segs, int nseg, nq_stream_t stream);
+NQ_API int nq_adaround_adam_slabs_multi(const nq_ada_adam_seg* segs, int nseg, const nq_wgr_seg* wgr, int nwgr, float reg_b,
+                                 float step_size, float beta1, float beta2, float eps, float bc2_sqrt, const float* dyn,
+                                 nq_stream_t stream);
 
 NQ_API int nq_ps_gelu_backward(const float* da, const float* z, float* dconv, int B, int C, int H, int W, int r,
                         nq_stream_t stream);
diff --git a/neuroquant_amd/_lib.py b/neuroquant_amd/_lib.py
--- a/neuroquant_amd/_lib.py
+++ b/neuroquant_amd/_lib.py
@@ -27,6 +27,23 @@
 class WLSeg(Structure):
     _fields_ = [("w", c_void_p), ("wt_fwd", c_void_p), ("wt_bwd", c_void_p), ("Cout", c_int), ("Cin", c_int), ("k", c_int),
                 ("krows_fwd", c_int), ("ld_fwd", c_int), ("krows_bwd", c_int), ("ld_bwd", c_int)]
+
+
+class FqPar(Structure):
+    _fields_ = [("alpha", c_void_p), ("delta", c_void_p), ("zp", c_void_p), ("per_row", c_int), ("n_levels", c_int),
+                ("soft", c_int)]
+
+
+class QWL3Seg(Structure):
+    _fields_ = [("l", WL3Seg), ("q", FqPar)]
+
+
+class QWLSeg(Structure):
+    _fields_ = [("l", WLSeg), ("q", FqPar)]
+
+
+class QElSeg(Structure):
+    _fields_ = [("x", c_void_p), ("out", c_void_p), ("rows", c_int64), ("row_len", c_int64), ("q", FqPar)]
 
 
 class FwhtSeg(Structure):
@@ -113,6 +130,7 @@
     sig("nq_weight_layout3_multi", I, POINTER(WL3Seg), I, P)
     sig("nq_weight_layouts_multi", I, POINTER(WLSeg), I, P)
     sig("nq_weight_layouts_all", I, POINTER(WL3Seg), I, POINTER(WLSeg), I, P)
+    sig("nq_quant_layouts_all", I, POINTER(QWL3Seg), I, POINTER(QWLSeg), I, POINTER(QElSeg), I, P)
     sig("nq_conv_forward3_ws_floats", L, I, I, I, I, I, I)
     sig("nq_conv_forward3", I, P, P, P, P, P, P, P, I, I, I, I, I, I, I, I, P)
     sig("nq_conv_wgrad3_supported", I, I, I, I, I, I, I)
@@ -124,6 +142,7 @@
     sig("nq_conv_wgrad3_swapped_slabs", I, P, P, P, P, I, I, I, I, I, I, POINTER(WgrSeg), P)
     sig("nq_conv_wgrad_slabs", I, P, P, P, P, P, I, I, I, I, I, I, I, POINTER(WgrSeg), P)
     sig("nq_wgrad_reduce_multi", I, POINTER(WgrSeg), I, P)
+    sig("nq_adaround_adam_slabs_multi", I, POINTER(AdaAdamSeg), I, POINTER(WgrSeg), I, F, F, F, F, F, F, P, P)
     sig("nq_conv_wgrad_ws_floats", L, I, I, I, I, I, I)
     sig("nq_conv_wgrad", I, P, P, P, P, P, I, I, I, I, I, I, I, P)
     sig("nq_ps_gelu_backward", I, P, P, P, I, I, I, I, I, P)
@@ -157,6 +176,7 @@
     "nq_act_dd", "nq_pixel_shuffle", "nq_bias_add", "nq_conv3_split_io", "nq_conv_split_out", "nq_split_words",
     "nq_conv_wgrad3_split_io", "nq_conv_wgrad3_fmt", "nq_conv_wgrad3_slabs_fmt", "nq_head_forward_loss_ws_floats", "nq_head_forward_loss",
     "nq_adaround_fwht_multi", "nq_fwht_adaround_adam_multi", "nq_weight_layouts_all",
+    "nq_adaround_adam_slabs_multi", "nq_quant_layouts_all",
 )
 
 _lib = None
diff --git a/neuroquant_amd/csrc/conv3.hip b/neuroquant_amd/csrc/conv3.hip
--- a/neuroquant_amd/csrc/conv3.hip
+++ b/neuroquant_amd/csrc/conv3.hip
@@ -1,6 +1,7 @@
 #include <cstdlib>
 #include "nq_common.h"
 #include "conv3_layout.h"
+#include "quant_elem.h"
 
 extern "C" {
 int nq_conv_igemm3_k3(const float*, const void*, const float*, float*, float*, const float*, int, int, int, int, int, int, int,
@@ -60,9 +61,26 @@
   int64_t slots;
 };
 
+struct WLQ {
+  const float* alpha;
+  const float* delta;
+  const float* zp;
+  float qmax;
+  int soft, per_row;
+};
+template <bool Q>
+__device__ __forceinline__ float wl_load(const float* __restrict__ w, const WLQ* q, int64_t idx, int row) {
+  const float t = w[idx];
+  if (!Q) return t;
+  const int r = q->per_row ? row : 0;
+  float xq;
+  return ada_fwd_elem(t, q->alpha[idx], q->delta[r], q->zp[r], q->qmax, q->soft, xq);
+}
+
 constexpr int WL3_KKMAX = 25;
-template <int KK>
-__device__ __forceinline__ void wl3_tile(const WL3& p, int c, int g16, float* __restrict__ T ) {
+template <int KK, bool Q = false>
+__device__ __forceinline__ void wl3_tile(const WL3& p, int c, int g16, float* __restrict__ T ,
+                                         const WLQ* q = nullptr) {
   constexpr int RS = 16 * KK + 1;
   const int tid = threadIdx.x;
   const int nfull = p.nchunk - (p.tail ? 1 : 0);
@@ -80,7 +98,7 @@
       const int a = e / (16 * KK), rem = e - a * (16 * KK);
       const int bb = rem / KK;
       const bool ok = a0 + a < Ra && b0 + bb < Cb;
-      const float t = p.w[ok ? ((int64_t)(a0 + a) * Cb + b0) * KK + rem : 0];
+      const float t = wl_load<Q>(p.w, q, ok ? ((int64_t)(a0 + a) * Cb + b0) * KK + rem : 0, ok ? a0 + a : 0);
       v[j] = ok ? t : 0.f;
     }
 #pragma unroll
@@ -155,32 +173,68 @@
   int blkf[WL3_MAXSEG + 1];
   int nf;
 };
-__global__ __launch_bounds__(256) void weight_layouts_all_kernel(WLAll t) {
-  __shared__ float T[16 * (16 * WL3_KKMAX + 1)];
+template <bool Q>
+__device__ __forceinline__ void wl_all_block(const WLAll& t, int blkx, float* __restrict__ T, const WLQ* q, const int* q3,
+                                             const int* qf) {
   const int nb3 = t.blk3[t.n3];
-  if ((int)blockIdx.x < nb3) {
+  if (blkx < nb3) {
     int k = 0;
-    while (k + 1 < t.n3 && (int)blockIdx.x >= t.blk3[k + 1]) ++k;
-    const int blk = (int)blockIdx.x - t.blk3[k];
-    if (t.s3[k].KK == 25) wl3_tile<25>(t.s3[k], blk / t.s3[k].co16, blk % t.s3[k].co16, T);
-    else wl3_tile<9>(t.s3[k], blk / t.s3[k].co16, blk % t.s3[k].co16, T);
+    while (k + 1 < t.n3 && blkx >= t.blk3[k + 1]) ++k;
+    const int blk = blkx - t.blk3[k];
+    const WLQ* qk = Q ? q + q3[k] : nullptr;
+    if (t.s3[k].KK == 25) wl3_tile<25, Q>(t.s3[k], blk / t.s3[k].co16, blk % t.s3[k].co16, T, qk);
+    else wl3_tile<9, Q>(t.s3[k], blk / t.s3[k].co16, blk % t.s3[k].co16, T, qk);
     return;
   }
-  const int bf = (int)blockIdx.x - nb3;
+  const int bf = blkx - nb3;
   int k = 0;
   while (k + 1 < t.nf && bf >= t.blkf[k + 1]) ++k;
   const WLF& g = t.sf[k];
+  const WLQ* qk = Q ? q + qf[k] : nullptr;
   const int64_t i = (int64_t)(bf - t.blkf[k]) * 256 + threadIdx.x;
   if (i >= (int64_t)g.krows * g.ld) return;
   const int row = (int)(i / g.ld), col = (int)(i - (int64_t)row * g.ld);
   float v = 0.f;
   if (g.bwd) {
     const int co = row / g.KK, tap = row - co * g.KK;
-    if (co < g.Cout && col < g.Cin) v = g.w[((int64_t)co * g.Cin + col) * g.KK + (g.KK - 1 - tap)];
+    if (co < g.Cout && col < g.Cin) v = wl_load<Q>(g.w, qk, ((int64_t)co * g.Cin + col) * g.KK + (g.KK - 1 - tap), co);
   } else {
-    if (col < g.Cout && row < g.Cin * g.KK) v = g.w[(int64_t)col * (g.Cin * g.KK) + row];
+    if (col < g.Cout && row < g.Cin * g.KK) v = wl_load<Q>(g.w, qk, (int64_t)col * (g.Cin * g.KK) + row, col);
   }
   g.wt[i] = v;
+}
+__global__ __launch_bounds__(256) void weight_layouts_all_kernel(WLAll t) {
+  __shared__ float T[16 * (16 * WL3_KKMAX + 1)];
+  wl_all_block<false>(t, (int)blockIdx.x, T, nullptr, nullptr, nullptr);
+}
+
+struct WLE {
+  const float* x;
+  float* out;
+  int n, q, row_len;
+};
+struct WLQAll {
+  WLAll l;
+  WLQ q[WL3_MAXSEG];
+  int q3[WL3_MAXSEG], qf[WL3_MAXSEG];
+  WLE e[WL3_MAXSEG];
+  int blke[WL3_MAXSEG + 1];
+  int ne;
+};
+static_assert(sizeof(WLQAll) <= 4096, "the table must fit one kernel-argument block");
+__global__ __launch_bounds__(256) void quant_layouts_all_kernel(WLQAll t) {
+  __shared__ float T[16 * (16 * WL3_KKMAX + 1)];
+  const int nbl = t.l.blk3[t.l.n3] + t.l.blkf[t.l.nf];
+  if ((int)blockIdx.x < nbl) {
+    wl_all_block<true>(t.l, (int)blockIdx.x, T, t.q, t.q3, t.qf);
+    return;
+  }
+  const int be = (int)blockIdx.x - nbl;
+  int k = 0;
+  while (k + 1 < t.ne && be >= t.blke[k + 1]) ++k;
+  const WLE& g = t.e[k];
+  const int i = (be - t.blke[k]) * 256 + (int)threadIdx.x;
+  if (i < g.n) g.out[i] = wl_load<true>(g.x, t.q + g.q, i, i / g.row_len);
 }
 
 struct Fwd3Plan {
@@ -500,6 +554,67 @@
   }
   t.blkf[t.nf] = bf;
   hipLaunchKernelGGL(weight_layouts_all_kernel, dim3((unsigned)(blocks + bf)), dim3(256), 0, nq_s(stream), t);
+  return nq_launch_status();
+}
+
+int nq_quant_layouts_all(const nq_qwl3_seg* segs3, int n3, const nq_qwl_seg* segsf, int nf, const nq_qel_seg* segse, int ne,
+                         nq_stream_t stream) {
+  if (n3 < 0 || nf < 0 || ne < 0 || n3 > WL3_MAXSEG || nf > WL3_MAXSEG || ne > WL3_MAXSEG || (n3 > 0 && !segs3) ||
+      (nf > 0 && !segsf) || (ne > 0 && !segse) || n3 + nf + ne == 0)
+    return NQ_ERR_INVALID;
+  WLQAll t;
+  int nq = 0;
+  auto quant_of = [&](const nq_fq_par& h) -> int {
+    if (!h.alpha || !h.delta || !h.zp || h.n_levels < 2) return -1;
+    for (int i = 0; i < nq; ++i)
+      if (t.q[i].alpha == h.alpha) return i;
+    if (nq == WL3_MAXSEG) return -1;
+    t.q[nq] = WLQ{h.alpha, h.delta, h.zp, (float)(h.n_levels - 1), h.soft, h.per_row};
+    return nq++;
+  };
+  t.l.n3 = n3;
+  int blocks = 0;
+  for (int i = 0; i < n3; ++i) {
+    const nq_wl3_seg& h = segs3[i].l;
+    if (!wl3_fill(t.l.s3[i], h.w, h.wt3, h.Cin, h.Cout, h.k, h.transposed) || (t.q3[i] = quant_of(segs3[i].q)) < 0)
+      return NQ_ERR_INVALID;
+    t.l.blk3[i] = blocks;
+    blocks += t.l.s3[i].nchunk * t.l.s3[i].co16;
+  }
+  t.l.blk3[n3] = blocks;
+  t.l.nf = 0;
+  int bf = 0;
+  for (int i = 0; i < nf; ++i) {
+    const nq_wl_seg& h = segsf[i].l;
+    if (!h.w || h.Cout <= 0 || h.Cin <= 0 || h.k <= 0) return NQ_ERR_INVALID;
+    const int KK = h.k * h.k, qi = quant_of(segsf[i].q);
+    if (qi < 0) return NQ_ERR_INVALID;
+    for (int bwd = 0; bwd < 2; ++bwd) {
+      float* wt = bwd ? h.wt_bwd : h.wt_fwd;
+      if (!wt) continue;
+      const int krows = bwd ? h.krows_bwd : h.krows_fwd, ld = bwd ? h.ld_bwd : h.ld_fwd;
+      if (bwd ? (krows < h.Cout * KK || ld < h.Cin) : (krows < h.Cin * KK || ld < h.Cout)) return NQ_ERR_INVALID;
+      if (t.l.nf == WL3_MAXSEG) return NQ_ERR_INVALID;
+      t.l.sf[t.l.nf] = WLF{h.w, wt, h.Cout, h.Cin, KK, krows, ld, bwd};
+      t.qf[t.l.nf] = qi;
+      t.l.blkf[t.l.nf] = bf;
+      bf += (int)(((int64_t)krows * ld + 255) / 256);
+      ++t.l.nf;
+    }
+  }
+  t.l.blkf[t.l.nf] = bf;
+  t.ne = ne;
+  int be = 0;
+  for (int i = 0; i < ne; ++i) {
+    const nq_qel_seg& h = segse[i];
+    const int qi = quant_of(h.q);
+    if (!h.x || !h.out || h.rows <= 0 || h.row_len <= 0 || h.rows * h.row_len > 0x7fffffffLL || qi < 0) return NQ_ERR_INVALID;
+    t.e[i] = WLE{h.x, h.out, (int)(h.rows * h.row_len), qi, (int)h.row_len};
+    t.blke[i] = be;
+    be += (t.e[i].n + 255) / 256;
+  }
+  t.blke[ne] = be;
+  hipLaunchKernelGGL(quant_layouts_all_kernel, dim3((unsigned)(blocks + bf + be)), dim3(256), 0, nq_s(stream), t);
   return nq_launch_status();
 }
 
diff --git a/neuroquant_amd/csrc/quant.hip b/neuroquant_amd/csrc/quant.hip
--- a/neuroquant_amd/csrc/quant.hip
+++ b/neuroquant_amd/csrc/quant.hip
@@ -409,6 +409,177 @@
   }
 }
 
+struct AdaAdamSlabSegD {
+  AdaAdamSegD a;
+  const float* slab;
+  int64_t stride;
+  int Cout, N, n_pad, nsplit, swap_kk, sg, kind;
+};
+struct AdaAdamSlabMulti {
+  AdaAdamSlabSegD s[MAXSEG];
+  int blk0[MAXSEG + 1];
+  int nseg;
+};
+static_assert(sizeof(AdaAdamSlabMulti) + 64 <= 4096, "segment table + scalars must fit one kernel-argument block");
+
+__device__ __forceinline__ void ada_adam_quad(const AdaAdamSegD& sg, int64_t i0, int cnt, const float* gv, float reg_b, float rw,
+                                              float step_size, float beta1, float beta2, float eps, float bc2_sqrt) {
+  const bool vec = sg.vec && cnt == 4 && (i0 & 3) == 0;
+  float xv[4], av[4], mv[4], vv[4];
+  if (vec) {
+    const float4 x4 = *reinterpret_cast<const float4*>(sg.x + i0), a4 = *reinterpret_cast<const float4*>(sg.alpha + i0);
+    const float4 m4 = *reinterpret_cast<const float4*>(sg.m + i0), v4 = *reinterpret_cast<const float4*>(sg.v + i0);
+    xv[0] = x4.x; xv[1] = x4.y; xv[2] = x4.z; xv[3] = x4.w;
+    av[0] = a4.x; av[1] = a4.y; av[2] = a4.z; av[3] = a4.w;
+    mv[0] = m4.x; mv[1] = m4.y; mv[2] = m4.z; mv[3] = m4.w;
+    vv[0] = v4.x; vv[1] = v4.y; vv[2] = v4.z; vv[3] = v4.w;
+  } else {
+#pragma unroll
+    for (int j = 0; j < 4; ++j) {
+      const bool in = j < cnt;
+      xv[j] = in ? sg.x[i0 + j] : 0.f;
+      av[j] = in ? sg.alpha[i0 + j] : 0.f;
+      mv[j] = in ? sg.m[i0 + j] : 0.f;
+      vv[j] = in ? sg.v[i0 + j] : 0.f;
+    }
+  }
+  const int64_t row0 = sg.per_row ? i0 / sg.row_len : 0;
+  const int rem0 = sg.per_row ? (int)(i0 - row0 * sg.row_len) : 0;
+#pragma unroll
+  for (int j = 0; j < 4; ++j) {
+    if (j >= cnt) break;
+    int64_t row = 0;
+    if (sg.per_row) row = (sg.row_len >= 4) ? row0 + ((rem0 + j >= sg.row_len) ? 1 : 0) : (i0 + j) / sg.row_len;
+    const float g = ada_bwd_elem(xv[j], gv[j], av[j], sg.delta[row], sg.zp[row], sg.qmax, rw, reg_b);
+    mv[j] = mv[j] + (1.f - beta1) * (g - mv[j]);
+    vv[j] = vv[j] * beta2 + (1.f - beta2) * (g * g);
+    const float denom = sqrtf(vv[j]) / bc2_sqrt + eps;
+    av[j] = av[j] - step_size * (mv[j] / denom);
+  }
+  if (vec) {
+    *reinterpret_cast<float4*>(sg.m + i0) = make_float4(mv[0], mv[1], mv[2], mv[3]);
+    *reinterpret_cast<float4*>(sg.v + i0) = make_float4(vv[0], vv[1], vv[2], vv[3]);
+    *reinterpret_cast<float4*>(sg.alpha + i0) = make_float4(av[0], av[1], av[2], av[3]);
+  } else {
+#pragma unroll
+    for (int j = 0; j < 4; ++j)
+      if (j < cnt) {
+        sg.m[i0 + j] = mv[j];
+        sg.v[i0 + j] = vv[j];
+        sg.alpha[i0 + j] = av[j];
+      }
+  }
+}
+
+__global__ __launch_bounds__(TPB) void adaround_adam_slabs_multi_kernel(AdaAdamSlabMulti t, float reg_b, float step_size,
+                                                                        float beta1, float beta2, float eps, float bc2_sqrt,
+                                                                        const float* __restrict__ dyn) {
+  __shared__ float4 part[TPB];
+  float gate = 1.f;
+  if (dyn) {
+    reg_b = dyn[0];
+    gate = dyn[1];
+    step_size = dyn[2];
+    bc2_sqrt = dyn[3];
+  }
+  const int k = find_seg(t, blockIdx.x);
+  const AdaAdamSlabSegD& q = t.s[k];
+  const AdaAdamSegD& a = q.a;
+  const float rw = dyn ? a.reg_weight * gate : a.reg_weight;
+  const int blk = blockIdx.x - t.blk0[k];
+  if (q.kind == 0) {
+    const int64_t i0 = (int64_t)blk * (TPB * EPT) + 4 * threadIdx.x;
+    if (i0 >= a.n) return;
+    const int cnt = a.n - i0 < 4 ? (int)(a.n - i0) : 4;
+    float gv[4];
+    if (a.vec && cnt == 4) {
+      const float4 g4 = *reinterpret_cast<const float4*>(a.gy + i0);
+      gv[0] = g4.x; gv[1] = g4.y; gv[2] = g4.z; gv[3] = g4.w;
+    } else {
+#pragma unroll
+      for (int j = 0; j < 4; ++j) gv[j] = j < cnt ? a.gy[i0 + j] : 0.f;
+    }
+    ada_adam_quad(a, i0, cnt, gv, reg_b, rw, step_size, beta1, beta2, eps, bc2_sqrt);
+    return;
+  }
+  const int N = q.N, Cout = q.Cout, nsplit = q.nsplit;
+  const int NQ = (N + 3) >> 2;
+  if (q.kind == 3) {
+    const int64_t i = (int64_t)blk * TPB + threadIdx.x;
+    if (i >= (int64_t)Cout * NQ) return;
+    const int co = (int)(i / NQ), n = 4 * (int)(i - (int64_t)co * NQ);
+    const float* p = q.slab + (int64_t)co * q.n_pad + n;
+    float4 acc[4];
+#pragma unroll
+    for (int g = 0; g < 4; ++g) acc[g] = make_float4(0.f, 0.f, 0.f, 0.f);
+    int j = 0;
+    for (; j + 4 <= nsplit; j += 4) {
+#pragma unroll
+      for (int g = 0; g < 4; ++g) {
+        const float4 v = *reinterpret_cast<const float4*>(p + (j + g) * q.stride);
+        acc[g].x += v.x; acc[g].y += v.y; acc[g].z += v.z; acc[g].w += v.w;
+      }
+    }
+#pragma unroll
+    for (int g = 0; g < 3; ++g) {
+      if (j + g < nsplit) {
+        const float4 v = *reinterpret_cast<const float4*>(p + (j + g) * q.stride);
+        acc[g].x += v.x; acc[g].y += v.y; acc[g].z += v.z; acc[g].w += v.w;
+      }
+    }
+    float4 s = acc[0];
+#pragma unroll
+    for (int g = 1; g < 4; ++g) { s.x += acc[g].x; s.y += acc[g].y; s.z += acc[g].z; s.w += acc[g].w; }
+    const float sv[4] = {s.x, s.y, s.z, s.w};
+    ada_adam_quad(a, (int64_t)co * N + n, N - n < 4 ? N - n : 4, sv, reg_b, rw, step_size, beta1, beta2, eps, bc2_sqrt);
+    return;
+  }
+  const int SG = q.sg, OG = TPB / SG;
+  const int o = threadIdx.x % OG, g = threadIdx.x / OG;
+  const int64_t i = (int64_t)blk * OG + o;
+  const int64_t total = q.kind == 1 ? (int64_t)Cout * NQ : Cout;
+  float4 s = make_float4(0.f, 0.f, 0.f, 0.f);
+  int co = 0, n = 0;
+  if (i < total) {
+    if (q.kind == 1) {
+      co = (int)(i / NQ);
+      n = 4 * (int)(i - (int64_t)co * NQ);
+      const float* p = q.slab + (int64_t)co * q.n_pad + n;
+#pragma unroll 8
+      for (int j = g; j < nsplit; j += SG) {
+        const float4 v = *reinterpret_cast<const float4*>(p + j * q.stride);
+        s.x += v.x; s.y += v.y; s.z += v.z; s.w += v.w;
+      }
+    } else {
+#pragma unroll 8
+      for (int j = g; j < nsplit; j += SG) s.x += q.slab[j * q.stride + i];
+    }
+  }
+  if (SG > 1) {
+    part[g * OG + o] = s;
+    __syncthreads();
+    if (g != 0) return;
+    s = part[o];
+    for (int j = 1; j < SG; ++j) {
+      const float4 v = part[j * OG + o];
+      s.x += v.x; s.y += v.y; s.z += v.z; s.w += v.w;
+    }
+  }
+  if (i >= total) return;
+  const float sv[4] = {s.x, s.y, s.z, s.w};
+  if (q.kind == 2) {
+    ada_adam_quad(a, i, 1, sv, reg_b, rw, step_size, beta1, beta2, eps, bc2_sqrt);
+  } else if (q.swap_kk > 0) {
+    for (int e = 0; e < 4 && n + e < N; ++e) {
+      const int ci = (n + e) / q.swap_kk, tap = (n + e) - ci * q.swap_kk;
+      ada_adam_quad(a, ((int64_t)ci * Cout + co) * q.swap_kk + (q.swap_kk - 1 - tap), 1, sv + e, reg_b, rw, step_size, beta1,
+                    beta2, eps, bc2_sqrt);
+    }
+  } else {
+    ada_adam_quad(a, (int64_t)co * N + n, N - n < 4 ? N - n : 4, sv, reg_b, rw, step_size, beta1, beta2, eps, bc2_sqrt);
+  }
+}
+
 struct UaqSegD {
   const float* x;
   const float* gy;
@@ -732,6 +903,58 @@
   return nq_launch_status();
 }
 
+int nq_adaround_adam_slabs_multi(const nq_ada_adam_seg* segs, int nseg, const nq_wgr_seg* wgr, int nwgr, float reg_b,
+                                 float step_size, float beta1, float beta2, float eps, float bc2_sqrt, const float* dyn,
+                                 nq_stream_t stream) {
+  if (!segs || nseg <= 0 || nseg > MAXSEG || nwgr < 0 || nwgr > MAXSEG || (nwgr > 0 && !wgr)) return NQ_ERR_INVALID;
+  AdaAdamSlabMulti t;
+  t.nseg = nseg;
+  int64_t blocks = 0;
+  for (int k = 0; k < nseg; ++k) {
+    const nq_ada_adam_seg& h = segs[k];
+    if (!h.x || !h.gy || !h.alpha || !h.delta || !h.zp || !h.m || !h.v || h.rows <= 0 || h.row_len <= 0 ||
+        h.row_len > 0x7fffffffLL)
+      return NQ_ERR_INVALID;
+    AdaAdamSlabSegD& q = t.s[k];
+    AdaAdamSegD& d = q.a;
+    d.x = h.x; d.gy = h.gy; d.alpha = h.alpha; d.delta = h.delta; d.zp = h.zp; d.m = h.m; d.v = h.v;
+    d.n = h.rows * h.row_len; d.row_len = (int)h.row_len; d.per_row = h.per_row;
+    d.qmax = (float)(h.n_levels - 1); d.reg_weight = h.reg_weight;
+    d.vec = (((uintptr_t)h.x | (uintptr_t)h.alpha | (uintptr_t)h.m | (uintptr_t)h.v) & 15) == 0;
+    q.slab = nullptr; q.stride = 0; q.Cout = q.N = q.n_pad = q.nsplit = q.swap_kk = 0; q.sg = 1; q.kind = 0;
+    for (int j = 0; j < nwgr; ++j) {
+      const nq_wgr_seg& w = wgr[j];
+      if (w.nsplit == 0 || (h.gy != w.dw && h.gy != w.db)) continue;
+      const bool bias = h.gy != w.dw;
+      if (!w.slab || w.Cout <= 0 || w.N <= 0 || w.nsplit < 0 || !(w.sg == 1 || w.sg == 4 || w.sg == 16) || w.co_pad < w.Cout ||
+          w.n_pad < ((w.N + 3) & ~3) || (w.n_pad & 3) || ((uintptr_t)w.slab & 15) || (bias && !w.slab_db) ||
+          d.n != (bias ? (int64_t)w.Cout : (int64_t)w.Cout * w.N) || (!bias && w.swap_kk > 0 && w.N % w.swap_kk))
+        return NQ_ERR_INVALID;
+      q.slab = bias ? w.slab_db : w.slab;
+      q.stride = bias ? (int64_t)w.co_pad : (int64_t)w.co_pad * w.n_pad;
+      q.Cout = w.Cout; q.N = w.N; q.n_pad = w.n_pad; q.nsplit = w.nsplit; q.swap_kk = w.swap_kk; q.sg = w.sg;
+      q.kind = bias ? 2 : 1;
+      if (!bias && w.sg == 4 && w.swap_kk == 0 && (int64_t)w.Cout * ((w.N + 3) / 4) >= 64 * TPB) q.kind = 3;
+      break;
+    }
+    t.blk0[k] = (int)blocks;
+    if (q.kind == 0) {
+      d.vec = d.vec && ((uintptr_t)h.gy & 15) == 0;
+      blocks += (d.n + TPB * EPT - 1) / (TPB * EPT);
+    } else if (q.kind == 3) {
+      blocks += ((int64_t)q.Cout * ((q.N + 3) / 4) + TPB - 1) / TPB;
+    } else {
+      const int og = TPB / q.sg;
+      blocks += ((q.kind == 1 ? (int64_t)q.Cout * ((q.N + 3) / 4) : (int64_t)q.Cout) + og - 1) / og;
+    }
+    if (blocks > 0x7fffffffLL) return NQ_ERR_INVALID;
+  }
+  t.blk0[nseg] = (int)blocks;
+  hipLaunchKernelGGL(adaround_adam_slabs_multi_kernel, dim3((unsigned)blocks), dim3(TPB), 0, nq_s(stream), t, reg_b, step_size,
+                     beta1, beta2, eps, bc2_sqrt, dyn);
+  return nq_launch_status();
+}
+
 int nq_adam_step_multi(const nq_adam_seg* segs, int nseg, float step_size, float beta1, float beta2, float eps,
                        float bc2_sqrt, nq_stream_t stream) {
   return adam_multi(segs, nseg, step_size, beta1, beta2, eps, bc2_sqrt, nullptr, stream);
diff --git a/neuroquant_amd/ops.py b/neuroquant_amd/ops.py
--- a/neuroquant_amd/ops.py
+++ b/neuroquant_amd/ops.py
@@ -230,13 +230,24 @@
     return outs
 
 
-def adaround_adam_multi(items, opt, reg_b=0.0, dyn=None, beta1=0.9, beta2=0.999, eps=1e-8):
+def adaround_adam_multi(items, opt, reg_b=0.0, dyn=None, beta1=0.9, beta2=0.999, eps=1e-8, pending=None):
     assert len(items) == len(opt.params)
+    if pending is not None and (len(items) > 16 or len(pending.segs) > 16):
+        pending.flush()
     opt.t += 1
     segs, _, keep = _ada_segs([tuple(it) + (1,) for it in items], opt=opt)
     if any(t["alpha"].data_ptr() != p.data_ptr() for t, p in zip(keep, opt.params)):
         raise RuntimeError("adaround_adam_multi: items must be in the optimiser's parameter order")
     step_size, bc2_sqrt = opt.scalars(opt.t, beta1, beta2)
+    if pending is not None and pending.segs:
+        wgr = (L.WgrSeg * len(pending.segs))(*pending.segs)
+        have = {t["gy"].data_ptr() for t in keep}
+        if any(s.nsplit and (s.dw not in have or (s.db and s.db not in have)) for s in pending.segs):
+            raise RuntimeError("adaround_adam_multi: a pending reduction's output is not among the gradients handed over")
+        L.check(L.lib().nq_adaround_adam_slabs_multi(segs, len(items), wgr, len(pending.segs), float(reg_b), step_size, beta1,
+                                                     beta2, eps, bc2_sqrt, _p(dyn), _stream()), "adaround_adam_slabs_multi")
+        pending.segs, pending.keep = [], []
+        return
     L.check(L.lib().nq_adaround_adam_multi(segs, len(items), float(reg_b), step_size, beta1, beta2, eps, bc2_sqrt, _p(dyn),
                                            _stream()), "adaround_adam_multi")
 
@@ -508,6 +519,42 @@
     return outs3, outsf
 
 
+class LazyFakeQuant:
+    __slots__ = ("x", "alpha", "delta", "zp", "n_levels", "soft")
+
+    def __init__(self, x, alpha, delta, zp, n_levels, soft):
+        self.x, self.alpha, self.delta, self.zp = (_dev(t) for t in (x, alpha, delta, zp))
+        self.n_levels, self.soft = int(n_levels), bool(soft)
+
+    def par(self, q):
+        q.alpha, q.delta, q.zp = _p(self.alpha), _p(self.delta), _p(self.zp)
+        _, _, q.per_row = _rows(self.x, self.delta)
+        q.n_levels, q.soft = self.n_levels, int(self.soft)
+
+
+def lazy_fake_quant(x, alpha, delta, zp, n_levels, soft):
+    t = torch.empty_like(_dev(x)).requires_grad_(True)
+    t.nq_fq = LazyFakeQuant(x, alpha, delta, zp, n_levels, soft)
+    return t
+
+
+def quant_layouts_all(items3, items_f, items_e):
+    segs3, outs3, keep3 = _wl3_segs([(fq.x, t) for fq, t in items3])
+    segsf, outsf, keepf = _wl_segs([(fq.x, f, b) for fq, f, b in items_f])
+    q3, qf, qe = (L.QWL3Seg * len(items3))(), (L.QWLSeg * len(items_f))(), (L.QElSeg * len(items_e))()
+    for q, sg, it in list(zip(q3, segs3, items3)) + list(zip(qf, segsf, items_f)):
+        q.l = sg
+        it[0].par(q.q)
+    for q, (fq, out) in zip(qe, items_e):
+        if out.shape != fq.x.shape or not out.is_contiguous():
+            raise RuntimeError("quant_layouts_all: out must be a contiguous tensor shaped like x")
+        q.x, q.out = _p(fq.x), _p(out)
+        q.rows, q.row_len, _ = _rows(fq.x, fq.delta)
+        fq.par(q.q)
+    L.check(L.lib().nq_quant_layouts_all(q3, len(items3), qf, len(items_f), qe, len(items_e), _stream()), "quant_layouts_all")
+    return outs3, outsf
+
+
 def _conv_outputs(x, cout, epilogue, r):
     B, _, H, W = x.shape
     y = z = None
@@ -952,6 +999,8 @@
 
 
 def conv2d_fused(x, w, b, epilogue=EPI_PLAIN, r=1):
+    if hasattr(w, "nq_fq") or hasattr(b, "nq_fq"):
+        raise RuntimeError("neuroquant_amd: a lazy_fake_quant stand-in holds no values outside ops.decoder_stack")
     if not torch.is_grad_enabled() or not (x.requires_grad or w.requires_grad or (b is not None and b.requires_grad)):
         x, w = _dev(x, "x"), _dev(w, "weight")
         b = _dev(b, "bias") if b is not None else None
@@ -1007,6 +1056,41 @@
         yield
     finally:
         _ARENA_TLS.state = prev
+
+
+_FOLD_TLS = threading.local()
+
+
+class _FoldSlot:
+    def __init__(self):
+        self.pending = None
+
+    def put(self, pending):
+        self.flush()
+        pending.keep = [k[:1] for k in pending.keep]
+        self.pending = pending
+
+    def take(self):
+        pending, self.pending = self.pending, None
+        return pending
+
+    def flush(self):
+        pending = self.take()
+        if pending is not None:
+            pending.flush()
+
+
+@contextlib.contextmanager
+def fold_reductions(enable=True):
+    slot = _FoldSlot() if enable and os.environ.get("NQ_FOLD", "1") != "0" else None
+    prev = getattr(_FOLD_TLS, "slot", None)
+    _FOLD_TLS.slot = slot
+    try:
+        yield slot
+    finally:
+        _FOLD_TLS.slot = prev
+        if slot is not None:
+            slot.flush()
 
 
 def arena_reduced(img):
@@ -1136,8 +1220,16 @@
                             x.shape[3], ctx.needs_input_grad[0])
         keys3 = [(l, t) for l, p in enumerate(plan) for t, route in ((False, p.fwd), (True, p.dgrad)) if route == "bf16x3"]
         keys32 = [l for l, p in enumerate(plan) if "fp32" in (p.fwd, p.dgrad)]
-        ops3, ops32 = weight_layouts_all([(Ws[l], t) for l, t in keys3],
-                                         [(Ws[l], plan[l].fwd == "fp32", plan[l].dgrad == "fp32") for l in keys32])
+        lazy = [getattr(t, "nq_fq", None) for t in wb]
+        if any(q is not None for q in lazy):
+            if any(q is None for q, t in zip(lazy, wb) if t is not None):
+                raise RuntimeError("decoder_stack: lazy_fake_quant stand-ins and ordinary tensors cannot be mixed")
+            ops3, ops32 = quant_layouts_all([(lazy[2 * l], t) for l, t in keys3],
+                                            [(lazy[2 * l], plan[l].fwd == "fp32", plan[l].dgrad == "fp32") for l in keys32],
+                                            [(lazy[2 * l + 1], bs[l].detach()) for l in range(n) if bs[l] is not None])
+        else:
+            ops3, ops32 = weight_layouts_all([(Ws[l], t) for l, t in keys3],
+                                             [(Ws[l], plan[l].fwd == "fp32", plan[l].dgrad == "fp32") for l in keys32])
         ops3, ops32 = dict(zip(keys3, ops3)), dict(zip(keys32, ops32))
         saved_in, saved_z = [], []
         ctx.wbk, ctx.dims_b, ctx.w3t = [None] * n, [None] * n, [None] * n
@@ -1164,7 +1256,8 @@
         ctx.spec, ctx.plan, ctx.n = spec, plan, n
         ctx.save_for_backward(x, *saved_in, *saved_z)
         ctx.nq_arena, ctx.nq_arena_reduced = _arena_state(), False
-        ctx.nq_head = _HeadHandoff() if spec.tanh_out else None
+        ctx.nq_fold = getattr(_FOLD_TLS, "slot", None)
+        ctx.nq_head =_HeadHandoff() if spec.tanh_out else None
         if fused_loss is not None:
             ctx.nq_head.loss, ctx.nq_head.dconv, ctx.nq_head.db = fused_loss[1], fused_loss[2], fused_loss[3]
             ctx.nq_head.version = fused_loss[2]._version
@@ -1310,7 +1403,11 @@
         main.wait_stream(side)
         keep.clear()
     if pending is not None:
-        pending.flush()
+        fold = getattr(ctx, "nq_fold", None)
+        if fold is not None and arena is None:
+            fold.put(pending)
+        else:
+            pending.flush()
     if arena is not None:
         yield arena, None
         ctx.nq_arena_reduced = True
diff --git a/neuroquant_amd/quantization/calib_model.py b/neuroquant_amd/quantization/calib_model.py
--- a/neuroquant_amd/quantization/calib_model.py
+++ b/neuroquant_amd/quantization/calib_model.py
@@ -181,6 +181,9 @@
     dp_graph = use_graph and dp and os.environ.get("NQ_DP_GRAPH", "0") == "1"
     if dp and not dp_graph:
         use_graph = False
+    from ..models._decode import _fused_stack as _fusable
+    lazy_ok = device.type == 'cuda' and hasattr(model, 'model') and _fusable(model.model) is not None \
+        and os.environ.get("NQ_FOLD_LAYOUTS", "0") == "1"
     fused_stack = None
     if dp_graph:
         from ..models._decode import _fused_stack
@@ -235,6 +238,11 @@
             return (b if reg_on else 0), reg_on
 
         def body(get_batch, b, reg_on, dyn, want_log, staged=None):
+            fold = ada and not hadamard and not dp and probe is None and os.environ.get("NQ_FUSED_ADAM", "1") != "0"
+            with ops.fold_reductions(fold) as slot:
+                _body(get_batch, b, reg_on, dyn, want_log, staged, slot)
+
+        def _body(get_batch, b, reg_on, dyn, want_log, staged, slot):
             img, inputs = get_batch()
             if ada and fuse_had:
                 items = []
@@ -244,6 +252,10 @@
                 fq = ops.adaround_fwht_multi(items)
                 for i, L in enumerate(layers):
                     L._finish(fq[2 * i], fq[2 * i + 1], transformed=True)
+            elif ada and slot is not None and lazy_ok:
+                for L in layers:
+                    w_it, b_it = L.ada_items()
+                    L._finish(ops.lazy_fake_quant(*w_it), ops.lazy_fake_quant(*b_it))
             elif ada:
                 fq = ops.adaround_forward_multi(
                     [it for L in layers for it in L.ada_items()])
@@ -326,7 +338,7 @@
                                   weight if (reg_on or dyn is not None) else 0.0))
                     items.append((L.bias, gb, bq.alpha.data, bq.delta.data, bq.zero_point, bq.n_levels, 0.0))
                 if probe is None and os.environ.get("NQ_FUSED_ADAM", "1") != "0":
-                    ops.adaround_adam_multi(items, opt, b, dyn=dyn)
+                    ops.adaround_adam_multi(items, opt, b, dyn=dyn, pending=slot.take() if slot is not None else None)
                     grads = None
                 else:
                     grads = ops.adaround_backward_multi(items, b, dyn=dyn)
```
